# qiskit-community/aqc-research

Measured on AMD Instinct MI355X. Metric: objective+gradient evals/sec, higher is better.
Workload: dtype f64; 1 GPU; 16-qubit, 40-block cx spin ansatz, state-vector objective+gradient; n_qubits=16, num_thetas=208, gate_groups=56, batch_per_gpu=1024, columns=1, transport=none, records_gathered=1024, launcher=none

## Files before the change

### aqc_research_amd/csrc/aqc_kernels3.hip

```cpp
#include <hip/hip_runtime.h>

#include <cstring>

#include <type_traits>

#include "aqc_device.h"
#include "aqc_launch.h"
#include "aqc_math.h"

namespace aqc {

typedef double double4_t __attribute__((ext_vector_type(4)));

__host__ __device__ __forceinline__ unsigned swz3(unsigned l) { return l ^ ((l >> 4) & 15u) ^ ((l >> 8) & 15u); }

__device__ __forceinline__ double4_t mfma(double a, double b, double4_t c) {
    return __builtin_amdgcn_mfma_f64_16x16x4f64(a, b, c, 0, 0, 0);
}

struct Acc3 { double4_t k1, k2, k3; };
__device__ __forceinline__ void u_mfma(const cplx (&v)[4], const double (&u0)[4], const double (&u1)[4], const double (&u2)[4], Acc3& t) {
    t.k1 = double4_t{0.0, 0.0, 0.0, 0.0}; t.k2 = t.k1; t.k3 = t.k1;
#pragma unroll
    for (int s = 0; s < 4; ++s) {
        t.k1 = mfma(v[s].x + v[s].y, u0[s], t.k1);
        t.k2 = mfma(v[s].x, u1[s], t.k2);
        t.k3 = mfma(v[s].y, u2[s], t.k3);
    }
}
__device__ __forceinline__ void u_combine(const Acc3& t, cplx (&o)[4]) {
#pragma unroll
    for (int r = 0; r < 4; ++r) {
        o[r].x = t.k1[r] - t.k3[r];
        o[r].y = t.k1[r] + t.k2[r];
    }
}

#ifdef AQC_TUNING
#define AQC_STAMP(slot) do { if (a.stamps && threadIdx.x == 0 && (slot) < kStampSlots) \
    a.stamps[((size_t)blockIdx.y * gridDim.x + blockIdx.x) * kStampSlots + (slot)] = __builtin_amdgcn_s_memtime(); } while (0)
#ifdef AQC_TUNING_NODBG
#define AQC_DBG_AND(x)
#define AQC_DBG_TEST(x) false
#else
#define AQC_DBG_AND(x) && (x)
#define AQC_DBG_TEST(x) (x)
#endif
#else
#define AQC_STAMP(slot) do { } while (0)
#define AQC_DBG_AND(x)
#define AQC_DBG_TEST(x) false
#endif

__host__ __device__ constexpr bool sweep_scratch_double(int k) { return k >= 12 || k <= 9; }
#ifndef AQC_SWEEP_SPREAD
#define AQC_SWEEP_SPREAD 1
#endif
#ifndef AQC_APPLY_SPREAD
#define AQC_APPLY_SPREAD 1
#endif
#ifndef AQC_EXP_APPLY_SKIP
#define AQC_EXP_APPLY_SKIP 0
#endif
constexpr int kApplySkip = AQC_EXP_APPLY_SKIP;
#ifndef AQC_EXP_SWEEP_SKIP
#define AQC_EXP_SWEEP_SKIP 0
#endif
constexpr int kSweepSkip = AQC_EXP_SWEEP_SKIP;
#ifndef AQC_EXP_UBUILD_SKIP
#define AQC_EXP_UBUILD_SKIP 0
#endif
constexpr int kUbuildSkip = AQC_EXP_UBUILD_SKIP;

constexpr int kSweepSpread = AQC_SWEEP_SPREAD, kApplySpread = AQC_APPLY_SPREAD;
template <int K, bool SWEEP = false> struct TileShape {
    static constexpr int kSweepWaves12 = 4;
    static constexpr int kWaves = (SWEEP && K == 12) ? kSweepWaves12 : (K >= 10 ? 4 : (1 << (K - 8)));
    static constexpr int kGroups = 1 << (K - 8);
    static constexpr int kGpw = kGroups / kWaves;
    static constexpr int kLoads = (1 << (K - 6)) / kWaves;
};

struct SubRegs {
    double u0[4], u1[4], u2[4];
    unsigned lane12;
};

template <int GPW>
__device__ __forceinline__ void fetch_sub(SubRegs& x, const DevSub3* subs, const double* umat, int sub_index, int lane, int wave,
                                          int nwaves) {
    const DevSub3* sub = subs + sub_index;
    const double* up = umat + (size_t)sub_index * 12 * 64;
#pragma unroll
    for (int s = 0; s < 4; ++s) {
        x.u0[s] = up[(0 * 4 + s) * 64 + lane];
        x.u1[s] = up[(1 * 4 + s) * 64 + lane];
        x.u2[s] = up[(2 * 4 + s) * 64 + lane];
    }
    x.lane12 = sub->lane12[lane];
}

template <int GPW>
struct SubAddr {
    unsigned a1, a2;
    unsigned k1[GPW][4], k2[GPW][4];
};
typedef unsigned uint8v_t __attribute__((ext_vector_type(8)));
template <int GPW>
__device__ __forceinline__ void fetch_k(SubAddr<GPW>& x, const DevSub3* subs, int sub_index, int wave, int nwaves) {
#pragma unroll
    for (int j = 0; j < GPW; ++j) {
        const uint8v_t kv = *reinterpret_cast<const __attribute__((address_space(4))) uint8v_t*>(
            (const __attribute__((address_space(4))) void*)(const void*)&subs[sub_index].kk[wave + j * nwaves][0]);
#pragma unroll
        for (int s = 0; s < 4; ++s) { x.k1[j][s] = kv[s]; x.k2[j][s] = kv[4 + s]; }
    }
}
template <int GPW>
__device__ __forceinline__ void sub_addr(SubAddr<GPW>& x, const SubRegs& c, unsigned lds_base) {
    x.a1 = ((c.lane12 & 0xffffu) << 4) + lds_base;
    x.a2 = ((c.lane12 >> 16) << 4) + lds_base;
}
typedef double dbl2_t __attribute__((ext_vector_type(2)));
typedef __attribute__((address_space(3))) dbl2_t* lds_cplx_ptr;
__device__ __forceinline__ cplx lds_get(unsigned addr) {
    const dbl2_t v = *reinterpret_cast<lds_cplx_ptr>(addr);
    return make_double2(v.x, v.y);
}
__device__ __forceinline__ void lds_put(unsigned addr, cplx v) { *reinterpret_cast<lds_cplx_ptr>(addr) = dbl2_t{v.x, v.y}; }
__device__ __forceinline__ unsigned lds_address(const void* p) {
    return (unsigned)reinterpret_cast<size_t>((__attribute__((address_space(3))) const char*)p);
}

__device__ __forceinline__ const void* uniform_ptr(const void* p) {
    const unsigned long long v = (unsigned long long)p;
    const unsigned lo = __builtin_amdgcn_readfirstlane((unsigned)v), hi = __builtin_amdgcn_readfirstlane((unsigned)(v >> 32));
    return (const void*)(((unsigned long long)hi << 32) | lo);
}

template <int K, int NV>
__device__ __forceinline__ void load_tiles3(cplx* t0, cplx* t1, const cplx* s0, const cplx* s1, const DevStage& st, unsigned lo, int wave) {
    constexpr int NL = TileShape<K, NV == 2>::kLoads, NW = TileShape<K, NV == 2>::kWaves;
    cplx v0[NL], v1[NL];
#pragma unroll
    for (int i = 0; i < NL; ++i) {
        const unsigned off = lo + st.dhi[wave + i * NW];
        v0[i] = s0[off];
        if (NV == 2) v1[i] = s1[off];
    }
#pragma unroll
    for (int i = 0; i < NL; ++i) {
        const unsigned slot = swz3((unsigned)((wave + i * NW) << 6) | (threadIdx.x & 63u));
        t0[slot] = v0[i];
        if (NV == 2) t1[slot] = v1[i];
    }
}
template <int K, bool SWEEP>
__device__ __forceinline__ void store_tile3(const cplx* tile, cplx* dst, const DevStage& st, unsigned lo, int wave) {
    constexpr int NL = TileShape<K, SWEEP>::kLoads, NW = TileShape<K, SWEEP>::kWaves;
#pragma unroll
    for (int i = 0; i < NL; ++i) {
        const unsigned slot = swz3((unsigned)((wave + i * NW) << 6) | (threadIdx.x & 63u));
        dst[lo + st.dhi[wave + i * NW]] = tile[slot];
    }
}
__device__ __forceinline__ size_t tile_base3(const DevStage& st, unsigned tile) {
    size_t base = 0;
    for (int i0 = 0; i0 < st.nub; i0 += 4) {
        int ub[4];
#pragma unroll
        for (int u = 0; u < 4; ++u) ub[u] = st.ubits[i0 + u];
#pragma unroll
        for (int u = 0; u < 4; ++u)
            if (i0 + u < st.nub) base |= (size_t)((tile >> (i0 + u)) & 1u) << ub[u];
    }
    return base;
}

__device__ __forceinline__ int uniform_load(const int* p) { return __builtin_amdgcn_readfirstlane(*p); }
struct ItemAt { int bl, tile, slot; };
template <bool LIST>
__device__ __forceinline__ ItemAt item_at(const Stage3Args& a, int wi) {
    if (LIST) {
        const TileItem* it = a.items + wi;
        return ItemAt{uniform_load(&it->lane), uniform_load(&it->tile), uniform_load(&it->slot)};
    }
    const int bl = wi / a.ntiles;
    return ItemAt{bl, wi - bl * a.ntiles, 0};
}
template <int K, bool LIST, bool PAIR = false>
__device__ __forceinline__ void apply_mfma_body(const Stage3Args& a0, const Stage3Args& b0, const int wg, const int nwg) {
    using TS = TileShape<K>;
    static_assert(!PAIR || (LIST && K >= 12), "the pair form walks two lists with persistent workgroups");
    extern __shared__ __attribute__((aligned(16))) char smem[];
    const Stage3Args* ca = &a0;
#define a (*ca)
#define st (ca->stage)
    cplx* tw = reinterpret_cast<cplx*>(smem);
    const unsigned lds_base = lds_address(smem);
    if (lds_base & ((16u << K) - 1)) __builtin_trap();
    const int lane = threadIdx.x & 63;
    const int wave = __builtin_amdgcn_readfirstlane((int)(threadIdx.x >> 6));
    constexpr int NL = TS::kLoads, NW = TS::kWaves;
    constexpr bool kPersist = K >= 12;
    int nwork = LIST ? uniform_load(a.nitems) : a.ntiles * a.batch;
    bool second = false;
    if (PAIR && wg >= nwork) { ca = &b0; second = true; nwork = uniform_load(b0.nitems); }
    unsigned lo = st.dlo[lane];
    unsigned lo16 = lo << 4;
    (void)lo16;
    SubRegs cur, nxt;
    SubAddr<TS::kGpw> ad;
    dbl2_t pw[NL];
    int wi = wg + ((kPersist || LIST) ? 0 : (int)blockIdx.y * a.ntiles);
    if (LIST && wi >= nwork) return;
    ItemAt it = item_at<LIST>(a, wi);
    {
        const int bl = it.bl;
        if (st.nsubs > 0) {
            fetch_sub<TS::kGpw>(cur, a.subs, a.umat + (size_t)bl * a.nsubs_total * 12 * 64, st.sub_begin, lane, wave, NW);
            fetch_k<TS::kGpw>(ad, a.subs, st.sub_begin, wave, NW);
        }
        AQC_STAMP(0);
        if (!(kApplySkip & 64)) load_tiles3<K, 1>(tw, nullptr, a.in0 + (size_t)bl * a.lane_stride + tile_base3(st, it.tile), nullptr, st, lo, wave);
    }
    __builtin_amdgcn_s_waitcnt(0x0F70);
    AQC_STAMP(1);
    for (;;) {
    const int bl = it.bl;
    const size_t lane_off = (size_t)bl * a.lane_stride + tile_base3(st, it.tile);
    const double* umat = a.umat + (size_t)bl * a.nsubs_total * 12 * 64;
    int nwi = wi + nwg;
    bool more = kPersist && st.nsubs > 0 && nwi < nwork;
    const Stage3Args* na = ca;
    int nnwork = nwork;
    if (PAIR && !more && !second) {
        na = &b0; nwi = wg; nnwork = uniform_load(b0.nitems);
        more = nwi < nnwork;
    }
    const bool change = PAIR && na != ca;
    const ItemAt nit = more ? item_at<LIST>(*na, nwi) : ItemAt{0, 0, 0};
    const int nbl = nit.bl;
    const size_t next_off = more ? (size_t)nbl * na->lane_stride + tile_base3(na->stage, nit.tile) : 0;
    const unsigned nlo = change ? na->stage.dlo[lane] : lo;
    const unsigned nlo16 = nlo << 4;
    for (int si = 0; si < st.nsubs; ++si) {
        AQC_STAMP(4 + si);
        if (!(kApplySkip & 512)) __syncthreads();
        if (si + 1 < st.nsubs) fetch_sub<TS::kGpw>(nxt, a.subs, umat, st.sub_begin + si + 1, lane, wave, NW);
        else if (more) fetch_sub<TS::kGpw>(nxt, na->subs, na->umat + (size_t)nbl * na->nsubs_total * 12 * 64, na->stage.sub_begin, lane, wave, NW);
        if (kPersist && more && !(kApplySkip & 64)) {
#pragma unroll
            for (int c = 0; c < 4; ++c) {
                if (si == (c < st.nsubs ? c : st.nsubs - 1)) {
#pragma unroll
                    for (int i = c * (NL / 4); i < (c + 1) * (NL / 4); ++i) {
                        const size_t ub = next_off + na->stage.dhi[wave + i * NW];
                        asm volatile("s_nop 4\n\tglobal_load_dwordx4 %0, %1, %2" : "=a"(pw[i]) : "v"(nlo16), "s"(uniform_ptr(na->in0 + ub)) : "memory");
                    }
                }
            }
        }
        sub_addr(ad, cur, lds_base);
        cplx v[2][4];
        Acc3 acc;
#pragma unroll
        for (int s = 0; s < 4; ++s) v[0][s] = lds_get(ad.a1 ^ ad.k1[0][s]);
#pragma unroll
        for (int j = 0; j <= TS::kGpw; ++j) {
            if (j + 1 < TS::kGpw && !(kApplySkip & 2)) {
#pragma unroll
                for (int s = 0; s < 4; ++s) v[(j + 1) & 1][s] = lds_get((kApplySkip & 32) ? ad.a1 : (ad.a1 ^ ad.k1[j + 1][s]));
            }
            __builtin_amdgcn_sched_barrier(0);
            double sv[4];
            cplx o[4];
            if (j < TS::kGpw) {
#pragma unroll
                for (int s = 0; s < 4; ++s) sv[s] = (kApplySkip & (16 | 128)) ? v[j & 1][s].x : v[j & 1][s].x + v[j & 1][s].y;
            }
            if (j > 0) {
                if (kApplySkip & (16 | 256)) {
#pragma unroll
                    for (int r = 0; r < 4; ++r) o[r] = make_double2(acc.k1[r], acc.k2[r]);
                } else u_combine(acc, o);
            }
            unsigned wa[4];
            if (j < TS::kGpw) {
#pragma unroll
                for (int s = 0; s < 4; ++s) asm volatile("" : "+v"(sv[s]));
            }
            if (j > 0) {
#pragma unroll
                for (int r = 0; r < 4; ++r) { wa[r] = (kApplySkip & 32) ? ad.a2 : (ad.a2 ^ ad.k2[j - 1][r]); asm volatile("" : "+v"(wa[r])); }
            }
            __builtin_amdgcn_sched_barrier(0);
            if (j < TS::kGpw) {
                acc.k1 = double4_t{0.0, 0.0, 0.0, 0.0}; acc.k2 = acc.k1; acc.k3 = acc.k1;
#pragma unroll
                for (int s = 0; s < 4; ++s) {
                    if (kApplySkip & 8) continue;
                    acc.k1 = mfma(sv[s], cur.u0[s], acc.k1);
                    acc.k2 = mfma(v[j & 1][s].x, cur.u1[s], acc.k2);
                    acc.k3 = mfma(v[j & 1][s].y, cur.u2[s], acc.k3);
                }
            }
            if (j > 0 && !(kApplySkip & 1)) {
#pragma unroll
                for (int r = 0; r < 4; ++r) lds_put(wa[r], o[r]);
                if (j < TS::kGpw) {
#pragma unroll
                    for (int i = 0; i < 4; ++i) {
                        __builtin_amdgcn_sched_group_barrier(0x008, kApplySpread, 0);
                        __builtin_amdgcn_sched_group_barrier(0x200, 1, 0);
                    }
                }
            }
            __builtin_amdgcn_sched_barrier(0);
        }
        if (si + 1 < st.nsubs || more) {
            cur = nxt;
            if (si + 1 < st.nsubs) fetch_k<TS::kGpw>(ad, a.subs, st.sub_begin + si + 1, wave, NW);
            else fetch_k<TS::kGpw>(ad, na->subs, na->stage.sub_begin, wave, NW);
        }
    }
    AQC_STAMP(4 + st.nsubs);
    __syncthreads();
    AQC_STAMP(2);
    if (!(kApplySkip & 64)) store_tile3<K, false>(tw, a.out0 + lane_off, st, lo, wave);
    AQC_STAMP(3);
    if (!more) break;
    __syncthreads();
    __builtin_amdgcn_s_waitcnt(0x0F70);
#pragma unroll
    for (int i = 0; i < NL; ++i) {
        const unsigned slot = swz3((unsigned)((wave + i * NW) << 6) | (threadIdx.x & 63u));
        asm volatile("ds_write_b128 %0, %1" : : "v"(lds_base + (slot << 4)), "a"(pw[i]) : "memory");
    }
    __builtin_amdgcn_s_waitcnt(0xC07F);
    wi = nwi;
    it = nit;
    if (PAIR) { ca = na; second = second || change; nwork = nnwork; lo = nlo; lo16 = nlo16; }
    }
#undef a
#undef st
}
template <int K, bool LIST = false>
__global__ __launch_bounds__(TileShape<K>::kWaves * 64, 2) void apply_mfma_kernel(const Stage3Args a) {
    apply_mfma_body<K, LIST>(a, a, (int)blockIdx.x, (int)gridDim.x);
}
#ifndef AQC_PAIR_PLAIN_BOUNDARY
#define AQC_PAIR_PLAIN_BOUNDARY 0
#endif
template <int K>
__global__ __launch_bounds__(TileShape<K>::kWaves * 64, 2) void apply_pair_kernel(const Stage3Args a, const Stage3Args b, const int grid_a) {
    if constexpr (K >= 12 && !AQC_PAIR_PLAIN_BOUNDARY) {
        static_assert(sizeof(Stage3Args) % 8 == 0 && alignof(Stage3Args) == 8, "b follows a in the kernel-argument segment without padding");
        const __attribute__((address_space(4))) char* kp = (const __attribute__((address_space(4))) char*)__builtin_amdgcn_kernarg_segment_ptr();
        const Stage3Args* pa = (const Stage3Args*)(const void*)kp;
        const Stage3Args* pb = (const Stage3Args*)(const void*)(kp + sizeof(Stage3Args));
        apply_mfma_body<K, true, true>(*pa, *pb, (int)blockIdx.x, (int)gridDim.x);
    } else if (K >= 12) {
        apply_mfma_body<K, true>(a, a, (int)blockIdx.x, (int)gridDim.x);
        __syncthreads();
        apply_mfma_body<K, true>(b, b, (int)blockIdx.x, (int)gridDim.x);
    } else if ((int)blockIdx.x < grid_a) {
        apply_mfma_body<K, true>(a, a, (int)blockIdx.x, grid_a);
    } else {
        apply_mfma_body<K, true>(b, b, (int)blockIdx.x - grid_a, (int)gridDim.x - grid_a);
    }
}

template <int N>
__device__ __forceinline__ void wait_prefetched(dbl2_t (&pw)[N], dbl2_t (&pz)[N]) {
    asm volatile("s_waitcnt vmcnt(0)" : : : "memory");
#pragma unroll
    for (int i = 0; i < N; ++i) asm volatile("" : "+a"(pw[i]), "+a"(pz[i]));
}
__device__ __forceinline__ unsigned tile_offset3(const DevStage& st, unsigned local) { return st.dlo[local & 63u] | st.dhi[local >> 6]; }
template <int K> struct SweepShape : TileShape<K, true> {};
__device__ __forceinline__ unsigned elem_bit(const DevStage& st, long long e, unsigned local_pos) {
    const unsigned m = local_pos < 6 ? st.dlo[1u << local_pos] : st.dhi[1u << (local_pos - 6)];
    return ((unsigned long long)e & m) ? 1u : 0u;
}
template <int GPW, int NW>
__device__ __forceinline__ void skip_masks(const DevStage& st, unsigned info, long long e0, long long e1, int wave, unsigned& nzmask, unsigned& kneed) {
    nzmask = 0; kneed = 0;
    const unsigned gfresh = info & 15u, kfresh = (info >> 6) & 3u;
#pragma unroll
    for (int k = 0; k < 2; ++k) {
        const long long e = k ? e1 : e0;
        if (e < 0) continue;
        unsigned gb = 0;
#pragma unroll
        for (int i = 0; i < 4; ++i)
            if (gfresh >> i & 1) gb |= elem_bit(st, e, (info >> (8 + 4 * i)) & 15u) << i;
        unsigned kb = 0;
        if (kfresh & 1) kb |= elem_bit(st, e, (info >> 24) & 15u);
        if (kfresh & 2) kb |= elem_bit(st, e, (info >> 28) & 15u) << 1;
#pragma unroll
        for (int j = 0; j < GPW; ++j)
            if ((((unsigned)(wave + j * NW) ^ gb) & gfresh) == 0) nzmask |= 1u << j;
#pragma unroll
        for (unsigned s2 = 0; s2 < 4; ++s2)
            if (((s2 ^ kb) & kfresh) == 0) kneed |= 1u << s2;
    }
}
template <int K, bool LIST, bool SKIPW, bool RLAST>
__device__ __forceinline__ void sweep_mfma_body(const Stage3Args& a, const int wg, const int nwg) {
    using TS = TileShape<K, true>;
    constexpr int kSlots = TS::kWaves > 4 ? 4 : TS::kWaves;
    constexpr unsigned tsize = 1u << K;
    extern __shared__ __attribute__((aligned(16))) char smem[];
    const DevStage& st = a.stage;
    cplx* tw = reinterpret_cast<cplx*>(smem);
    cplx* tz = tw + tsize;
    cplx* scratch = tz + tsize;
    constexpr bool kDouble = sweep_scratch_double(K);
    const unsigned lds_base = lds_address(smem);
    if (lds_base & ((32u << K) - 1)) __builtin_trap();
    const int lane = threadIdx.x & 63;
    const int wave = __builtin_amdgcn_readfirstlane((int)(threadIdx.x >> 6));
    constexpr bool kPersist = K >= 12;
    constexpr int NL = TS::kLoads, NW = TS::kWaves;
    const int nwork = LIST ? uniform_load(a.nitems) : a.ntiles * a.batch;
    const unsigned lo = st.dlo[lane];
    SubRegs cur, nxt;
    SubAddr<TS::kGpw> ad;
    dbl2_t pw[NL], pz[NL];
    unsigned parity = 0;
    AQC_STAMP(0);
    const int chunk = kPersist ? (LIST ? (nwork + nwg - 1) / nwg : a.chunk) : 0;
    const int wi_first = kPersist ? wg * chunk : wg;
    const int wi_end = kPersist ? (wi_first + chunk < nwork ? wi_first + chunk : nwork) : wi_first + 1;
    int wi = wi_first;
    if (wi >= nwork) return;
    const unsigned e16 = threadIdx.x << 4;
    dbl2_t racc;
    static_assert(!kPersist || NL == 4 * TS::kGpw, "the prefetch registers are the first sub-stage's operands");
    const bool reg_first = kPersist && st.nsubs > 0;
    unsigned flo16 = 0;
    ItemAt it = item_at<LIST>(a, wi);
    size_t item_off = (size_t)it.bl * a.lane_stride + tile_base3(st, it.tile);
    {
        const size_t off0 = item_off;
        if (st.nsubs > 0) {
            fetch_sub<TS::kGpw>(cur, a.subs, a.umat + (size_t)it.bl * a.nsubs_total * 12 * 64, st.sub_begin, lane, wave, NW);
            fetch_k<TS::kGpw>(ad, a.subs, st.sub_begin, wave, NW);
        }
        if (reg_first) {
            flo16 = tile_offset3(st, swz3(cur.lane12 & 0xffffu)) << 4;
#pragma unroll
            for (int i = 0; i < ((kSweepSkip & 64) ? 0 : NL); ++i) {
                const size_t ub = off0 + a.first_hi[wave + (i / 4) * NW][i % 4];
                asm volatile("s_nop 4\n\tglobal_load_dwordx4 %0, %1, %2" : "=a"(pw[i]) : "v"(flo16), "s"(uniform_ptr(a.in0 + ub)) : "memory");
                asm volatile("s_nop 4\n\tglobal_load_dwordx4 %0, %1, %2" : "=a"(pz[i]) : "v"(flo16), "s"(uniform_ptr(a.in1 + ub)) : "memory");
            }
        } else {
            load_tiles3<K, 2>(tw, tz, a.in0 + off0, a.in1 + off0, st, lo, wave);
        }
    }
    __builtin_amdgcn_s_waitcnt(0x0F70);
    if (reg_first) wait_prefetched<NL>(pw, pz);
    __syncthreads();
    AQC_STAMP(1);
    for (;;) {
    const int bl = it.bl, tile = it.tile;
    const size_t lane_off = item_off;
    long long se0 = -1, se1 = -1;
    if (SKIPW) {
        const unsigned long long toff = (unsigned long long)tile_base3(st, tile);
        const long long c0 = a.supp[2 * (size_t)bl], c1 = a.supp[2 * (size_t)bl + 1];
        const unsigned lo0 = __builtin_amdgcn_readfirstlane((unsigned)c0), hi0 = __builtin_amdgcn_readfirstlane((unsigned)(c0 >> 32));
        const unsigned lo1 = __builtin_amdgcn_readfirstlane((unsigned)c1), hi1 = __builtin_amdgcn_readfirstlane((unsigned)(c1 >> 32));
        const long long u0 = (long long)(((unsigned long long)hi0 << 32) | lo0), u1 = (long long)(((unsigned long long)hi1 << 32) | lo1);
        if (u0 >= 0 && (((unsigned long long)u0 ^ toff) & st.fresh_nonlocal) == 0) se0 = u0;
        if (u1 >= 0 && (((unsigned long long)u1 ^ toff) & st.fresh_nonlocal) == 0) se1 = u1;
    }
    const double* umat = a.umat + (size_t)bl * a.nsubs_total * 12 * 64;
    const int part = LIST ? it.slot : (kPersist ? wg - (bl * a.ntiles) / chunk : tile);
    const bool seg_first = LIST || !kPersist || wi == wi_first || tile == 0;
    cplx* rpart = a.rpart + (((size_t)bl * a.nsubs_total + st.sub_begin) * a.nparts + part) * 256;
    const int nwi = wi + 1;
    const bool more = reg_first && nwi < wi_end;
    const ItemAt nit = more ? item_at<LIST>(a, nwi) : ItemAt{0, 0, 0};
    const int nbl = nit.bl;
    const size_t next_off = more ? (size_t)nbl * a.lane_stride + tile_base3(st, nit.tile) : 0;
    constexpr unsigned ZOFF = tsize * 16;
    cplx vw[2][4], vz[2][4];
    constexpr bool kEarly = K >= 11;
    if (reg_first) {
        sub_addr(ad, cur, lds_base);
#pragma unroll
        for (int s = 0; s < 4; ++s) { vw[0][s] = make_double2(pw[s].x, pw[s].y); vz[0][s] = make_double2(pz[s].x, pz[s].y); }
    } else if (kEarly && st.nsubs > 0) {
        sub_addr(ad, cur, lds_base);
#pragma unroll
        for (int s = 0; s < 4; ++s) { vw[0][s] = lds_get(ad.a1 ^ ad.k1[0][s]); vz[0][s] = lds_get((ad.a1 | ZOFF) ^ ad.k1[0][s]); }
    }
    auto prefetch = [&](int c) __attribute__((always_inline)) {
#pragma unroll
        for (int i = 0; i < ((kSweepSkip & 64) ? 0 : NL); ++i)
            if (i / (NL / 4) == c) {
                const size_t ub = next_off + a.first_hi[wave + (i / 4) * NW][i % 4];
                asm volatile("s_nop 4\n\tglobal_load_dwordx4 %0, %1, %2" : "=a"(pw[i]) : "v"(flo16), "s"(uniform_ptr(a.in0 + ub)) : "memory");
                asm volatile("s_nop 4\n\tglobal_load_dwordx4 %0, %1, %2" : "=a"(pz[i]) : "v"(flo16), "s"(uniform_ptr(a.in1 + ub)) : "memory");
            }
    };
    const int nmain = RLAST && a.r_only_last && st.nsubs >= 1 && !(kPersist && st.nsubs == 1) ? st.nsubs - 1 : st.nsubs;
    if (!RLAST) {
        for (int si = 0; si < st.nsubs; ++si) {
#define AQC_SS_FROM_REGS (reg_first && si == 0)
#define AQC_SS_RONLY false
#include "aqc_sweep_substage.inc"
#undef AQC_SS_FROM_REGS
#undef AQC_SS_RONLY
        }
    } else {
        if (nmain > 0) {
            const int si = 0;
#define AQC_SS_FROM_REGS reg_first
#define AQC_SS_RONLY false
#include "aqc_sweep_substage.inc"
#undef AQC_SS_FROM_REGS
#undef AQC_SS_RONLY
        }
        for (int si = 1; si < nmain; ++si) {
#define AQC_SS_FROM_REGS false
#define AQC_SS_RONLY false
#include "aqc_sweep_substage.inc"
#undef AQC_SS_FROM_REGS
#undef AQC_SS_RONLY
        }
        if (nmain < st.nsubs) {
            const int si = nmain;
#define AQC_SS_FROM_REGS false
#define AQC_SS_RONLY true
#include "aqc_sweep_substage.inc"
#undef AQC_SS_FROM_REGS
#undef AQC_SS_RONLY
        }
    }
    AQC_STAMP(kStampSlots - 2);
    if (more) wait_prefetched<NL>(pw, pz);
    if (!(kSweepSkip & 64)) {
        if (a.store_out & 1) store_tile3<K, true>(tw, a.out0 + lane_off, st, lo, wave);
        if (a.store_out & 2) store_tile3<K, true>(tz, a.out1 + lane_off, st, lo, wave);
    }
    AQC_STAMP(kStampSlots - 1);
    if (!more) break;
    AQC_STAMP(kStampSlots - 6);
    __syncthreads();
    AQC_STAMP(kStampSlots - 5);
    wi = nwi;
    it = nit;
    item_off = next_off;
    }
    AQC_STAMP(kStampSlots - 4);
}
template <int K, bool LIST = false, bool SKIPW = false, bool RLAST = false>
__global__ __launch_bounds__(SweepShape<K>::kWaves * 64, K >= 12 ? 1 : 2) void sweep_mfma_kernel(const Stage3Args a) {
    sweep_mfma_body<K, LIST, SKIPW, RLAST>(a, (int)blockIdx.x, (int)gridDim.x);
}
template <int K, bool RLAST_A, bool RLAST_B>
__global__ __launch_bounds__(SweepShape<K>::kWaves * 64, K >= 12 ? 1 : 2) void sweep_pair_kernel(const Stage3Args a, const Stage3Args b, const int grid_a) {
    if (K >= 12) {
        sweep_mfma_body<K, true, false, RLAST_A>(a, (int)blockIdx.x, (int)gridDim.x);
        __syncthreads();
        sweep_mfma_body<K, true, false, RLAST_B>(b, (int)blockIdx.x, (int)gridDim.x);
    } else if ((int)blockIdx.x < grid_a) {
        sweep_mfma_body<K, true, false, RLAST_A>(a, (int)blockIdx.x, grid_a);
    } else {
        sweep_mfma_body<K, true, false, RLAST_B>(b, (int)blockIdx.x - grid_a, (int)gridDim.x - grid_a);
    }
}

constexpr int kGrpChunk = 16;
struct Gm {
    cplx c[4], t[4];
    double ec, es;
    double rc[4], rs[4];
    int type, pc, pt, flags, slot0, jblock, o0, o1;
};
__device__ __forceinline__ void m2_mul(const cplx (&a)[4], const cplx (&b)[4], cplx (&o)[4]) {
#pragma unroll
    for (int i = 0; i < 2; ++i)
#pragma unroll
        for (int j = 0; j < 2; ++j) {
            const cplx x = a[2 * i], y = b[j], u = a[2 * i + 1], v = b[2 + j];
            o[2 * i + j] = make_double2(x.x * y.x - x.y * y.y + u.x * v.x - u.y * v.y, x.x * y.y + x.y * y.x + u.x * v.y + u.y * v.x);
        }
}
__device__ __forceinline__ void m2_ry(double c, double s, cplx (&o)[4]) {
    o[0] = make_double2(c, 0.0); o[1] = make_double2(-s, 0.0); o[2] = make_double2(s, 0.0); o[3] = make_double2(c, 0.0);
}
__device__ __forceinline__ void m2_rz(double c, double s, cplx (&o)[4]) {
    o[0] = make_double2(c, -s); o[1] = make_double2(0.0, 0.0); o[2] = make_double2(0.0, 0.0); o[3] = make_double2(c, s);
}
__device__ __forceinline__ void m2_rx(double c, double s, cplx (&o)[4]) {
    o[0] = make_double2(c, 0.0); o[1] = make_double2(0.0, -s); o[2] = make_double2(0.0, -s); o[3] = make_double2(c, 0.0);
}
template <bool DAG, bool TR>
__device__ __forceinline__ void m2_apply(const cplx (&m)[4], cplx& a0, cplx& a1) {
    const cplx m00 = m[0], m01 = (DAG || TR) ? m[2] : m[1], m10 = (DAG || TR) ? m[1] : m[2], m11 = m[3];
    const double sg = DAG ? -1.0 : 1.0;
    const cplx x = a0, y = a1;
    a0 = make_double2(m00.x * x.x - sg * m00.y * x.y + m01.x * y.x - sg * m01.y * y.y, m00.x * x.y + sg * m00.y * x.x + m01.x * y.y + sg * m01.y * y.x);
    a1 = make_double2(m10.x * x.x - sg * m10.y * x.y + m11.x * y.x - sg * m11.y * y.y, m10.x * x.y + sg * m10.y * x.x + m11.x * y.y + sg * m11.y * y.x);
}
__device__ __forceinline__ void stage_groups(Gm* gm, const DevGrp* grps, int begin, int count, const double* th, int ent, int lane) {
    {
        const int gi = lane >> 2, k = lane & 3;
        if (gi < count) {
            const DevGrp d = grps[begin + gi];
            double c = 1.0, s = 0.0;
            if (k < (d.type == 0 ? 3 : 4)) sincos(0.5 * th[d.theta0 + k], &s, &c);
            gm[gi].rc[k] = c; gm[gi].rs[k] = s;
            if (k == 0) {
                double ec = 1.0, es = 0.0;
                if (ent == 2 && d.type != 0) sincos(th[d.theta0 + 4], &es, &ec);
                gm[gi].ec = ec; gm[gi].es = es;
            }
        }
    }
    __builtin_amdgcn_fence(__ATOMIC_SEQ_CST, "wavefront");
    __builtin_amdgcn_wave_barrier();
    if (lane >= count) return;
    const DevGrp d = grps[begin + lane];
    Gm g;
    g.type = d.type; g.pc = d.pc; g.pt = d.pt; g.flags = d.flags; g.slot0 = d.slot0; g.jblock = d.jblock;
    const int mask = 0xF & ~(1 << d.pc) & ~(1 << d.pt);
    g.o0 = __ffs(mask) - 1; g.o1 = __ffs(mask & (mask - 1)) - 1;
    g.ec = gm[lane].ec; g.es = gm[lane].es;
#pragma unroll
    for (int k = 0; k < 4; ++k) { g.rc[k] = gm[lane].rc[k]; g.rs[k] = gm[lane].rs[k]; }
    cplx a[4], b[4], m[4];
    if (d.type == 0) {
        m2_rz(g.rc[0], g.rs[0], a); m2_ry(g.rc[1], g.rs[1], b); m2_mul(a, b, m);
        m2_rz(g.rc[2], g.rs[2], b); m2_mul(m, b, g.c);
        g.t[0] = make_double2(1.0, 0.0); g.t[1] = make_double2(0.0, 0.0); g.t[2] = g.t[1]; g.t[3] = g.t[0];
    } else {
        m2_rz(g.rc[1], g.rs[1], a); m2_ry(g.rc[0], g.rs[0], b); m2_mul(a, b, g.c);
        if (d.flags & 1) { m2_rz(kR, -kR, b); m2_mul(g.c, b, m); g.c[0] = m[0]; g.c[1] = m[1]; g.c[2] = m[2]; g.c[3] = m[3]; }
        if (ent == 0) m2_rx(g.rc[3], g.rs[3], a); else m2_rz(g.rc[3], g.rs[3], a);
        m2_ry(g.rc[2], g.rs[2], b); m2_mul(a, b, g.t);
        if (d.flags & 2) { m2_rz(kR, kR, a); m2_mul(a, g.t, m); g.t[0] = m[0]; g.t[1] = m[1]; g.t[2] = m[2]; g.t[3] = m[3]; }
    }
    gm[lane] = g;
}
__device__ __forceinline__ int grp_index(const Gm& g, int l, int rest) {
    return ((l >> 1) << g.pc) | ((l & 1) << g.pt) | ((rest & 1) << g.o0) | ((rest >> 1) << g.o1);
}
template <int MODE>
__device__ __forceinline__ void grp_apply(const Gm& g, int ent, cplx (&x)[4]) {
    auto entangle = [&](double es) {
        if (g.type == 0) return;
        if (ent == 0) { const cplx t = x[2]; x[2] = x[3]; x[3] = t; }
        else if (ent == 1) x[3] = make_double2(-x[3].x, -x[3].y);
        else x[3] = cmul(x[3], g.ec, es);
    };
    if (MODE == 0) {
        entangle(g.es);
        m2_apply<false, false>(g.t, x[0], x[1]); m2_apply<false, false>(g.t, x[2], x[3]);
        m2_apply<false, false>(g.c, x[0], x[2]); m2_apply<false, false>(g.c, x[1], x[3]);
    } else {
        m2_apply<MODE == 1, MODE == 2>(g.c, x[0], x[2]); m2_apply<MODE == 1, MODE == 2>(g.c, x[1], x[3]);
        m2_apply<MODE == 1, MODE == 2>(g.t, x[0], x[1]); m2_apply<MODE == 1, MODE == 2>(g.t, x[2], x[3]);
        entangle(MODE == 1 ? -g.es : g.es);
    }
}

__global__ __launch_bounds__(64) void ubuild_kernel(const UJob* jobs, const double* thetas, int T, double* thetas_copy) {
    __shared__ cplx u[256];
    __shared__ Gm gm[kGrpChunk];
    const int lane = threadIdx.x, b = blockIdx.y;
    const UJob job = jobs[blockIdx.x];
    const DevSub3 sub = *job.sub;
    const double* th = thetas + (size_t)b * T;
    if (thetas_copy && blockIdx.x == 0)
        for (int i = lane; i < T; i += 64) thetas_copy[(size_t)b * T + i] = th[i];
#pragma unroll
    for (int m = 0; m < 4; ++m) {
        const int e = lane + 64 * m;
        u[e] = make_double2((e >> 4) == (e & 15) ? 1.0 : 0.0, 0.0);
    }
    const int col = lane & 15, rest = lane >> 4;
    for (int base = 0; base < sub.ngrp; base += kGrpChunk) {
        const int count = min(kGrpChunk, sub.ngrp - base);
        __syncthreads();
        stage_groups(gm, job.grps, sub.grp_begin + base, count, th, job.entangler, lane);
        __syncthreads();
        for (int i = 0; i < count; ++i) {
            const Gm& g = gm[i];
            cplx x[4];
            int idx[4];
#pragma unroll
            for (int l = 0; l < 4; ++l) { idx[l] = grp_index(g, l, rest) * 16 + col; x[l] = u[idx[l]]; }
            if (job.inverse) grp_apply<1>(g, job.entangler, x); else grp_apply<0>(g, job.entangler, x);
#pragma unroll
            for (int l = 0; l < 4; ++l) u[idx[l]] = x[l];
            __syncthreads();
        }
    }
    __syncthreads();
    double* out = job.umat + ((size_t)b * job.nsubs + job.index) * 12 * 64;
    if (kUbuildSkip) {
        double acc = 0.0;
        for (int m = 0; m < 4; ++m) acc += u[lane + 64 * m].x * u[lane + 64 * m].y;
        if (acc == 1.0e300) out[lane] = acc;
    }
    if (kUbuildSkip & 1) return;
#pragma unroll
    for (int s = 0; s < 4; ++s) {
        const cplx v = u[(lane & 15) * 16 + 4 * s + (lane >> 4)];
        out[(0 * 4 + s) * 64 + lane] = v.x;
        out[(1 * 4 + s) * 64 + lane] = v.y - v.x;
        out[(2 * 4 + s) * 64 + lane] = v.x + v.y;
    }
    if (job.umat_mirror && !(kUbuildSkip & 2)) {
        double* om = job.umat_mirror + ((size_t)b * job.mirror_nsubs + job.mirror_index) * 12 * 64;
#pragma unroll
        for (int s = 0; s < 4; ++s) {
            const cplx t = u[(4 * s + (lane >> 4)) * 16 + (lane & 15)];
            const double re = t.x, im = -t.y;
            om[(0 * 4 + s) * 64 + lane] = re;
            om[(1 * 4 + s) * 64 + lane] = im - re;
            om[(2 * 4 + s) * 64 + lane] = re + im;
        }
    }
}

template <int LB>
__device__ __forceinline__ void rho_unapply(cplx (&rho)[16], int kind, double c, double s) {
    constexpr int st = LB == 0 ? 1 : 2, other = LB == 0 ? 2 : 1;
#pragma unroll
    for (int q = 0; q < 2; ++q)
#pragma unroll
        for (int b = 0; b < 4; ++b) {
            const int a0 = q * other;
            if (kind == MOP_RY) ry2(rho[a0 * 4 + b], rho[(a0 + st) * 4 + b], c, -s);
            else if (kind == MOP_RZ) rz2(rho[a0 * 4 + b], rho[(a0 + st) * 4 + b], c, -s);
            else rx2(rho[a0 * 4 + b], rho[(a0 + st) * 4 + b], c, -s);
        }
#pragma unroll
    for (int q = 0; q < 2; ++q)
#pragma unroll
        for (int a = 0; a < 4; ++a) {
            const int b0 = q * other;
            if (kind == MOP_RY) ry2(rho[a * 4 + b0], rho[a * 4 + b0 + st], c, -s);
            else if (kind == MOP_RZ) rz2(rho[a * 4 + b0], rho[a * 4 + b0 + st], c, s);
            else rx2(rho[a * 4 + b0], rho[a * 4 + b0 + st], c, s);
        }
}
template <int LB>
__device__ __forceinline__ cplx rho_dot(const cplx (&rho)[16], int kind) {
    constexpr int st = LB == 0 ? 1 : 2, other = LB == 0 ? 2 : 1;
    double re = 0.0, im = 0.0;
#pragma unroll
    for (int q = 0; q < 2; ++q) {
        const int i0 = q * other, i1 = i0 + st;
        if (kind == MOP_RY) { re += rho[i1 * 4 + i0].x - rho[i0 * 4 + i1].x; im += rho[i1 * 4 + i0].y - rho[i0 * 4 + i1].y; }
        else if (kind == MOP_RZ) { re += rho[i0 * 4 + i0].x - rho[i1 * 4 + i1].x; im += rho[i0 * 4 + i0].y - rho[i1 * 4 + i1].y; }
        else { re += rho[i0 * 4 + i1].x + rho[i1 * 4 + i0].x; im += rho[i0 * 4 + i1].y + rho[i1 * 4 + i0].y; }
    }
    return kind == MOP_RY ? make_double2(0.5 * re, 0.5 * im) : make_double2(-0.5 * im, 0.5 * re);
}

#ifdef AQC_TUNING
__device__ unsigned long long g_rgrad_stamps[32 * 8];
#define RG_STAMP(slot) do { if (blockIdx.y == 0 && blockIdx.x < 32 && threadIdx.x == 0) g_rgrad_stamps[blockIdx.x * 8 + (slot)] = __builtin_amdgcn_s_memtime(); } while (0)
#else
#define RG_STAMP(slot) do { } while (0)
#endif
template <int WAVES>
__global__ __launch_bounds__(64 * WAVES) void rgrad_kernel(const DevSub3* subs, const DevGrp* grps, int ent, const double* thetas, int T,
                                                           const cplx* rpart, int ntiles, int nsubs_total, cplx* partial, int nslots,
                                                           int from, int to, int front, const int* slot_theta, cplx* grads, cplx* mirror,
                                                           const GatherJob gj, int tiles_per_lane, int chunk, int sparse_subs,
                                                           const int* lane_parts, int conj_sub, const double* umat, int nsubs_run,
                                                           const RgradSecond second) {
    if ((int)blockIdx.x == nsubs_run + second.count) {
        const cplx* src = static_cast<const cplx*>(gj.buf) + (size_t)blockIdx.y * gj.lane_stride;
        for (int i = threadIdx.x; i < gj.count; i += 64 * WAVES) {
            const cplx v = src[(size_t)gj.elem[i]];
            static_cast<cplx*>(gj.out)[(size_t)blockIdx.y * gj.count + i] = v;
            if (gj.mirror) static_cast<cplx*>(gj.mirror)[(size_t)blockIdx.y * gj.count + i] = v;
        }
        return;
    }
    __shared__ cplx R[16 * 17];
    __shared__ Gm gm[kGrpChunk];
    __shared__ cplx rho_s[kGrpChunk][16];
    __shared__ cplx psum[WAVES > 1 ? WAVES - 1 : 1][WAVES > 1 ? 256 : 1];
    const int lane = threadIdx.x & 63, wave = threadIdx.x >> 6, b = blockIdx.y;
    int si = blockIdx.x;
    if (si >= nsubs_run) {
        si -= nsubs_run;
        subs = second.subs; grps = second.grps; rpart = second.rpart; ntiles = second.nparts; nsubs_total = second.nsubs_total;
        tiles_per_lane = second.nparts; chunk = 0; sparse_subs = second.nsubs_total; lane_parts = second.lane_parts; conj_sub = -1; umat = second.umat;
    }
    RG_STAMP(0);
    const DevSub3 sub = subs[si];
    const double* th = thetas + (size_t)b * T;
    const int nparts_stride = ntiles;
    if (chunk > 0) ntiles = ((b + 1) * tiles_per_lane - 1) / chunk - (b * tiles_per_lane) / chunk + 1;
    if (si < sparse_subs) ntiles = lane_parts[b];
    const cplx* rp = rpart + ((size_t)b * nsubs_total + si) * nparts_stride * 256;
    {
        cplx acc[4] = {make_double2(0.0, 0.0), make_double2(0.0, 0.0), make_double2(0.0, 0.0), make_double2(0.0, 0.0)};
        constexpr int TB = 8;
        for (int t0 = wave; t0 < ntiles; t0 += TB * WAVES) {
            cplx v[TB][4];
#pragma unroll
            for (int u = 0; u < TB; ++u)
#pragma unroll
                for (int r = 0; r < 4; ++r)
                    v[u][r] = t0 + u * WAVES < ntiles ? rp[(size_t)(t0 + u * WAVES) * 256 + 64 * r + lane] : make_double2(0.0, 0.0);
            if (WAVES > 1 && t0 == wave && wave == 0 && sub.ngrp > 0)
                stage_groups(gm, grps, sub.grp_begin + max(0, sub.ngrp - kGrpChunk), min(sub.ngrp, kGrpChunk), th, ent, lane);
#pragma unroll
            for (int u = 0; u < TB; ++u)
#pragma unroll
                for (int r = 0; r < 4; ++r) { acc[r].x += v[u][r].x; acc[r].y += v[u][r].y; }
        }
        if (WAVES > 1) {
            if (wave > 0) {
#pragma unroll
                for (int r = 0; r < 4; ++r) psum[wave - 1][64 * r + lane] = acc[r];
            }
            __syncthreads();
            if (wave > 0) return;
#pragma unroll
            for (int w = 0; w < WAVES - 1; ++w)
#pragma unroll
                for (int r = 0; r < 4; ++r) { const cplx p = psum[w][64 * r + lane]; acc[r].x += p.x; acc[r].y += p.y; }
        }
#pragma unroll
        for (int r = 0; r < 4; ++r)
            R[(4 * r + (lane >> 4)) * 17 + (lane & 15)] = acc[r];
    }
    if (si == conj_sub) {
        cplx* const Us = &rho_s[0][0];
        const double* up = umat + ((size_t)b * nsubs_total + si) * 12 * 64;
        __syncthreads();
#pragma unroll
        for (int s2 = 0; s2 < 4; ++s2) {
            const double re = up[(0 * 4 + s2) * 64 + lane], im = up[(1 * 4 + s2) * 64 + lane] + re;
            Us[(lane & 15) * 16 + 4 * s2 + (lane >> 4)] = make_double2(re, im);
        }
        __syncthreads();
        const int i0 = lane & 15, j0 = lane >> 4;
        cplx acc[4];
#pragma unroll
        for (int m = 0; m < 4; ++m) {
            const int j = j0 + 4 * m;
            double re = 0.0, im = 0.0;
            for (int k = 0; k < 16; ++k) {
                const cplx u = Us[j * 16 + k], r = R[k * 17 + i0];
                re += u.x * r.x - u.y * r.y; im += u.x * r.y + u.y * r.x;
            }
            acc[m] = make_double2(re, im);
        }
        __syncthreads();
#pragma unroll
        for (int m = 0; m < 4; ++m) R[(j0 + 4 * m) * 17 + i0] = acc[m];
        __syncthreads();
#pragma unroll
        for (int m = 0; m < 4; ++m) {
            const int j = j0 + 4 * m;
            double re = 0.0, im = 0.0;
            for (int k = 0; k < 16; ++k) {
                const cplx t = R[j * 17 + k], u = Us[i0 * 16 + k];
                re += t.x * u.x + t.y * u.y; im += t.y * u.x - t.x * u.y;
            }
            acc[m] = make_double2(re, im);
        }
        __syncthreads();
#pragma unroll
        for (int m = 0; m < 4; ++m) R[(j0 + 4 * m) * 17 + i0] = acc[m];
        __syncthreads();
    }
    RG_STAMP(1);
    cplx* out = partial + (size_t)b * nslots;
    auto put = [&](int slot, cplx v) {
        out[slot] = v;
        if (slot_theta) {
            const int t = slot_theta[slot];
            if (t >= 0) {
                grads[(size_t)b * T + t] = v;
                if (mirror) mirror[(size_t)b * T + t] = v;
            }
        }
    };
    const int lo = lane & 15, hi = lane >> 4;
    for (int top = sub.ngrp; top > 0; top -= kGrpChunk) {
        const int base = max(0, top - kGrpChunk), count = top - base;
        __syncthreads();
        if (WAVES == 1 || top != sub.ngrp) stage_groups(gm, grps, sub.grp_begin + base, count, th, ent, lane);
        __syncthreads();
        RG_STAMP(2);
        for (int i = count - 1; i >= 0; --i) {
            const Gm& g = gm[i];
            {
                const int a = lane >> 4, bb = (lane >> 2) & 3, o = lane & 3;
                cplx v = R[grp_index(g, a, o) * 17 + grp_index(g, bb, o)];
                v.x += dpp_mov<0xB1, 0xf>(v.x); v.y += dpp_mov<0xB1, 0xf>(v.y);
                v.x += dpp_mov<0x4E, 0xf>(v.x); v.y += dpp_mov<0x4E, 0xf>(v.y);
                if (o == 0) rho_s[i][a * 4 + bb] = v;
            }
            cplx x[4];
            int idx[4];
#pragma unroll
            for (int l = 0; l < 4; ++l) { idx[l] = grp_index(g, l, hi) * 17 + lo; x[l] = R[idx[l]]; }
            grp_apply<1>(g, ent, x);
#pragma unroll
            for (int l = 0; l < 4; ++l) R[idx[l]] = x[l];
            __syncthreads();
#pragma unroll
            for (int l = 0; l < 4; ++l) { idx[l] = lo * 17 + grp_index(g, l, hi); x[l] = R[idx[l]]; }
            grp_apply<2>(g, ent, x);
#pragma unroll
            for (int l = 0; l < 4; ++l) R[idx[l]] = x[l];
            __syncthreads();
        }
        RG_STAMP(3);
        if (lane < count) {
            const Gm& g = gm[lane];
            const bool on = g.jblock < 0 ? (front != 0) : (g.jblock >= from && g.jblock < to);
            if (on && g.slot0 >= 0) {
                cplx rho[16];
#pragma unroll
                for (int e = 0; e < 16; ++e) rho[e] = rho_s[lane][e];
                if (g.type == 0) {
                    put(g.slot0 + 2, rho_dot<1>(rho, MOP_RZ));
                    rho_unapply<1>(rho, MOP_RZ, g.rc[0], g.rs[0]);
                    put(g.slot0 + 1, rho_dot<1>(rho, MOP_RY));
                    rho_unapply<1>(rho, MOP_RY, g.rc[1], g.rs[1]);
                    put(g.slot0 + 0, rho_dot<1>(rho, MOP_RZ));
                } else {
                    const int ks = ent == 0 ? MOP_RX : MOP_RZ;
                    if (g.flags & 2) rho_unapply<0>(rho, MOP_RZ, kR, kR);
                    put(g.slot0 + 3, rho_dot<0>(rho, ks));
                    rho_unapply<0>(rho, ks, g.rc[3], g.rs[3]);
                    put(g.slot0 + 2, rho_dot<0>(rho, MOP_RY));
                    put(g.slot0 + 1, rho_dot<1>(rho, MOP_RZ));
                    rho_unapply<1>(rho, MOP_RZ, g.rc[1], g.rs[1]);
                    put(g.slot0 + 0, rho_dot<1>(rho, MOP_RY));
                    if (ent == 2) {
                        rho_unapply<0>(rho, MOP_RY, g.rc[2], g.rs[2]);
                        rho_unapply<1>(rho, MOP_RY, g.rc[0], g.rs[0]);
                        put(g.slot0 + 4, make_double2(rho[15].y, -rho[15].x));
                    }
                }
            } else if (slot_theta && g.slot0 >= 0) {
                for (int k = 0; k < 5; ++k) put(g.slot0 + k, make_double2(0.0, 0.0));
            }
        }
        RG_STAMP(4);
    }
}
#ifdef AQC_TUNING
void rgrad_print_stamps(int nsubs) {
    unsigned long long h[32 * 8];
    if (hipMemcpyFromSymbol(h, HIP_SYMBOL(g_rgrad_stamps), sizeof h) != hipSuccess) return;
    double a = 0, b = 0, c = 0, d = 0;
    const int n = nsubs < 32 ? nsubs : 32;
    for (int i = 0; i < n; ++i) { a += h[i * 8 + 1] - h[i * 8]; b += h[i * 8 + 2] - h[i * 8 + 1]; c += h[i * 8 + 3] - h[i * 8 + 2]; d += h[i * 8 + 4] - h[i * 8 + 3]; }
    fprintf(stderr, "aqc_hip stamps: gradient walk (lane 0, %d sub-stages): tile sum %.0f + group decode %.0f + R walk %.0f + rho walk %.0f cycles\n", n, a / n, b / n, c / n, d / n);
}
#endif

void stage3_first_offsets(Stage3Args& a, const DevSub3& first_sub) {
    for (int g = 0; g < 16; ++g)
        for (int s = 0; s < 4; ++s) {
            const unsigned local = swz3(first_sub.kk[g][s] >> 4);
            a.first_hi[g][s] = a.stage.dlo[local & 63u] | a.stage.dhi[local >> 6];
        }
}

int mfma_threads(int k, bool sweep) { return (sweep && k == 12) ? 64 * SweepShape<12>::kWaves : 64 * std::min(4, 1 << std::max(0, k - 8)); }
size_t apply3_lds_bytes(int k) { return (size_t)16 << k; }
size_t sweep3_lds_bytes(int k) {
    return ((size_t)32 << k) + (size_t)(sweep_scratch_double(k) ? 2 : 1) * std::min(4, mfma_threads(k, true) / 64) * 256 * sizeof(cplx);
}

template <typename F>
static hipError_t with_tile_size(int k, F&& f) {
    switch (k) {
        case 8: return f(std::integral_constant<int, 8>{});
        case 9: return f(std::integral_constant<int, 9>{});
        case 10: return f(std::integral_constant<int, 10>{});
        case 11: return f(std::integral_constant<int, 11>{});
        case 12: return f(std::integral_constant<int, 12>{});
        default: return hipErrorInvalidValue;
    }
}
using Stage3Kernel = void (*)(Stage3Args);
using Pair3Kernel = void (*)(Stage3Args, Stage3Args, int);
template <int K> static Stage3Kernel apply_variant(bool list) { return list ? apply_mfma_kernel<K, true> : apply_mfma_kernel<K, false>; }
template <int K> static Stage3Kernel sweep_variant(bool list, bool skipw, bool rlast) {
    if (list) return rlast ? sweep_mfma_kernel<K, true, false, true> : sweep_mfma_kernel<K, true, false, false>;
    if (skipw) return sweep_mfma_kernel<K, false, true, false>;
    return rlast ? sweep_mfma_kernel<K, false, false, true> : sweep_mfma_kernel<K, false, false, false>;
}
template <int K> static Pair3Kernel apply_pair_variant() { return apply_pair_kernel<K>; }
template <int K> static Pair3Kernel sweep_pair_variant(bool rlast_a) { return rlast_a ? sweep_pair_kernel<K, true, false> : sweep_pair_kernel<K, false, false>; }

template <typename F>
static hipError_t big_lds(F kernel) {
    return hipFuncSetAttribute(reinterpret_cast<const void*>(kernel), hipFuncAttributeMaxDynamicSharedMemorySize, 160 * 1024);
}
hipError_t init_kernels3() {
    hipError_t e = hipSuccess;
    for (int k = 8; k <= 12 && e == hipSuccess; ++k)
        e = with_tile_size(k, [](auto kk) {
            constexpr int K = decltype(kk)::value;
            hipError_t e = big_lds(apply_pair_variant<K>());
            for (int f = 0; f < 2 && e == hipSuccess; ++f) e = big_lds(apply_variant<K>(f));
            for (int f = 0; f < 2 && e == hipSuccess; ++f) e = big_lds(sweep_pair_variant<K>(f));
            for (int f = 0; f < 8 && e == hipSuccess; ++f) e = big_lds(sweep_variant<K>(f & 1, f & 2, f & 4));
            return e;
        });
    return e;
}
template <typename... Args>
static hipError_t launch3(void (*kernel)(Args...), dim3 grid, int k, bool sweep, hipStream_t s, const Args&... args) {
    kernel<<<grid, mfma_threads(k, sweep), sweep ? sweep3_lds_bytes(k) : apply3_lds_bytes(k), s>>>(args...);
    return hipGetLastError();
}
int mfma_occupancy(int k, bool sweep) {
    int n = 0;
    const hipError_t e = with_tile_size(k, [&](auto kk) {
        constexpr int K = decltype(kk)::value;
        return sweep ? hipOccupancyMaxActiveBlocksPerMultiprocessor(&n, sweep_variant<K>(false, false, false), mfma_threads(k, true), sweep3_lds_bytes(k))
                     : hipOccupancyMaxActiveBlocksPerMultiprocessor(&n, apply_variant<K>(false), mfma_threads(k, false), apply3_lds_bytes(k));
    });
    return e == hipSuccess ? n : -1;
}
static long persistent_sweep_grid(long sweep_grid) {
    if (sweep_grid > 0) return sweep_grid;
    static int cus[64] = {0};
    int dev = 0;
    if (hipGetDevice(&dev) != hipSuccess || dev < 0 || dev >= 64) return 256;
    if (cus[dev] == 0) {
        int n = 0;
        cus[dev] = (hipDeviceGetAttribute(&n, hipDeviceAttributeMultiprocessorCount, dev) == hipSuccess && n > 0) ? n : 256;
    }
    return cus[dev];
}
static bool stage3_launchable(int k, const Stage3Args& a, bool need_list, bool need_subs) {
    if (a.items ? (!a.nitems || a.max_items < 1) : need_list) return false;
    if (k < 12) return true;
    if (need_subs && a.stage.nsubs <= 0) return false;
    for (int l = 0; l < 64; ++l)
        if (a.stage.dlo[l] >= (1u << 28)) return false;
    return true;
}
hipError_t launch_apply3(int k, hipStream_t s, const Stage3Args& a, const Switches& sw) {
    const bool list = a.items != nullptr;
    const long persist = sw.apply_persist;
    if (!stage3_launchable(k, a, false, list) || (list && k >= 12 && persist <= 0)) return hipErrorInvalidValue;
    const long nwork = list ? (long)a.max_items : (long)a.ntiles * a.batch;
    const dim3 grid = (k >= 12 && persist > 0 && a.stage.nsubs > 0) ? dim3((unsigned)std::min<long>(nwork, persist * persistent_sweep_grid(sw.sweep_grid)))
                                                                     : ((k >= 12 || list) ? dim3((unsigned)nwork) : dim3(a.ntiles, a.batch));
    return with_tile_size(k, [&](auto kk) { return launch3(apply_variant<decltype(kk)::value>(list), grid, k, false, s, a); });
}
static_assert(2 * sizeof(Stage3Args) + 16 <= 3840, "two argument blocks must fit the kernel-argument segment");
hipError_t launch_apply3_pair(int k, hipStream_t s, const Stage3Args& a, const Stage3Args& b, const Switches& sw) {
    const long persist = sw.apply_persist;
    if (!stage3_launchable(k, a, true, true) || !stage3_launchable(k, b, true, true) || (k >= 12 && persist <= 0)) return hipErrorInvalidValue;
    const long longer = std::max(a.max_items, b.max_items);
    const dim3 grid((unsigned)(k >= 12 ? std::min<long>(longer, persist * persistent_sweep_grid(sw.sweep_grid)) : (long)a.max_items + b.max_items));
    return with_tile_size(k, [&](auto kk) { return launch3(apply_pair_variant<decltype(kk)::value>(), grid, k, false, s, a, b, a.max_items); });
}
int sweep3_chunk(int ntiles, int batch, int k, long sweep_grid) {
    if (k < 12) return 0;
    const long nwork = (long)ntiles * batch, g = std::min<long>(nwork, persistent_sweep_grid(sweep_grid));
    return (int)((nwork + g - 1) / g);
}
int sweep3_nparts(int ntiles, int batch, int k, long sweep_grid) {
    const int chunk = sweep3_chunk(ntiles, batch, k, sweep_grid);
    return chunk > 0 ? std::min(ntiles, (ntiles + chunk - 1) / chunk + 1) : ntiles;
}
hipError_t launch_sweep3(int k, hipStream_t s, const Stage3Args& a, const Switches& sw) {
    const bool list = a.items != nullptr;
    if (!stage3_launchable(k, a, false, true)) return hipErrorInvalidValue;
    if (a.nparts < 1 || (!list && (a.nparts != sweep3_nparts(a.ntiles, a.batch, k, sw.sweep_grid) || a.chunk != sweep3_chunk(a.ntiles, a.batch, k, sw.sweep_grid)))) return hipErrorInvalidValue;
    const long nwork = list ? (long)a.max_items : (long)a.ntiles * a.batch;
    const dim3 grid((unsigned)(k >= 12 ? (list ? std::min<long>(nwork, persistent_sweep_grid(sw.sweep_grid)) : (nwork + a.chunk - 1) / a.chunk) : nwork));
    const bool skipw = !list && a.supp != nullptr;
    const bool rlast = !skipw && a.r_only_last != 0;
    return with_tile_size(k, [&](auto kk) { return launch3(sweep_variant<decltype(kk)::value>(list, skipw, rlast), grid, k, true, s, a); });
}

hipError_t launch_sweep3_pair(int k, hipStream_t s, const Stage3Args& a, const Stage3Args& b, const Switches& sw) {
    if (!stage3_launchable(k, a, true, true) || !stage3_launchable(k, b, true, true)) return hipErrorInvalidValue;
    if (a.nparts < 1 || b.nparts < 1 || a.supp || b.supp || b.r_only_last) return hipErrorInvalidValue;
    const long longer = std::max(a.max_items, b.max_items);
    const dim3 grid((unsigned)(k >= 12 ? std::min<long>(longer, persistent_sweep_grid(sw.sweep_grid)) : (long)a.max_items + b.max_items));
    return with_tile_size(k, [&](auto kk) { return launch3(sweep_pair_variant<decltype(kk)::value>(a.r_only_last != 0), grid, k, true, s, a, b, a.max_items); });
}

__device__ __forceinline__ int tile_of_elem(const DevStage& st, long long e) {
    int t = 0;
    for (int i = 0; i < st.nub; ++i) t |= (int)((e >> st.ubits[i]) & 1) << i;
    return t;
}
__device__ __forceinline__ int lane_tiles(const DevStage& st, const long long* supp, int per_lane, const long long* extra, int nextra, int b,
                                          int (&tiles)[kMaxTileCands]) {
    int n = 0;
    auto add = [&](long long e) {
        if (e < 0) return;
        const int t = tile_of_elem(st, e);
        for (int i = 0; i < n; ++i)
            if (tiles[i] == t) return;
        tiles[n++] = t;
    };
    for (int k = 0; supp && k < per_lane; ++k) add(supp[(size_t)b * per_lane + k]);
    for (int k = 0; extra && k < nextra; ++k) add(extra[k]);
    return n;
}
__global__ __launch_bounds__(1024) void tile_items_kernel(const DevStage st, const long long* supp, int per_lane, const long long* extra, int nextra,
                                                          int batch, TileItem* items, int* nitems, int* lane_parts, int* prev_tiles,
                                                          TileItem* clear_items, int* nclear) {
    __shared__ int scan_a[1024], scan_b[1024];
    const int tid = threadIdx.x, per = (batch + 1023) / 1024;
    const int b0 = tid * per, b1 = min(batch, b0 + per);
    int tiles[kMaxTileCands];
    int mine = 0, mine_clear = 0;
    for (int b = b0; b < b1; ++b) {
        const int n = lane_tiles(st, supp, per_lane, extra, nextra, b, tiles);
        mine += n;
        if (prev_tiles)
            for (int k = 0; k < 2; ++k) {
                const int pt = prev_tiles[2 * b + k];
                bool stale = pt >= 0;
                for (int i = 0; i < n; ++i) stale = stale && tiles[i] != pt;
                mine_clear += stale ? 1 : 0;
            }
    }
    scan_a[tid] = mine; scan_b[tid] = mine_clear;
    __syncthreads();
    for (int d = 1; d < 1024; d <<= 1) {
        const int va = tid >= d ? scan_a[tid - d] : 0, vb = tid >= d ? scan_b[tid - d] : 0;
        __syncthreads();
        scan_a[tid] += va; scan_b[tid] += vb;
        __syncthreads();
    }
    int at = scan_a[tid] - mine, at_clear = scan_b[tid] - mine_clear;
    if (tid == 1023) { *nitems = scan_a[tid]; if (nclear) *nclear = scan_b[tid]; }
    for (int b = b0; b < b1; ++b) {
        const int n = lane_tiles(st, supp, per_lane, extra, nextra, b, tiles);
        if (lane_parts) lane_parts[b] = n;
        if (prev_tiles) {
            for (int k = 0; k < 2; ++k) {
                const int pt = prev_tiles[2 * b + k];
                bool stale = pt >= 0;
                for (int i = 0; i < n; ++i) stale = stale && tiles[i] != pt;
                if (stale) clear_items[at_clear++] = TileItem{b, pt, 0, 0};
            }
            prev_tiles[2 * b] = n > 0 ? tiles[0] : -1;
            prev_tiles[2 * b + 1] = n > 1 ? tiles[1] : -1;
        }
        for (int i = 0; i < n; ++i) items[at++] = TileItem{b, tiles[i], i, 0};
    }
}
hipError_t launch_tile_items(const DevStage& stage, const long long* supp, int per_lane, const long long* extra, int nextra, int batch,
                             TileItem* items, int* nitems, int* lane_parts, int* prev_tiles, TileItem* clear_items, int* nclear, hipStream_t s) {
    if ((supp ? per_lane : 0) + (extra ? nextra : 0) > kMaxTileCands || batch < 1) return hipErrorInvalidValue;
    if (prev_tiles && ((supp ? per_lane : 0) > 2 || (extra && nextra > 0) || !clear_items || !nclear)) return hipErrorInvalidValue;
    tile_items_kernel<<<1, 1024, 0, s>>>(stage, supp, per_lane, extra, nextra, batch, items, nitems, lane_parts, prev_tiles, clear_items, nclear);
    return hipGetLastError();
}
__global__ __launch_bounds__(256) void clear_tiles_kernel(const DevStage st, cplx* buf, size_t lane_stride, const TileItem* clear_items, const int* nclear) {
    if ((int)blockIdx.x >= *nclear) return;
    const TileItem it = clear_items[blockIdx.x];
    cplx* dst = buf + (size_t)it.lane * lane_stride + tile_base3(st, (unsigned)it.tile);
    for (unsigned l = threadIdx.x; l < (1u << st.k); l += 256) dst[tile_offset3(st, l)] = make_double2(0.0, 0.0);
}
hipError_t launch_clear_tiles(const DevStage& stage, void* buf, size_t lane_stride, const TileItem* clear_items, const int* nclear, int max_items,
                              hipStream_t s) {
    if (max_items < 1) return hipSuccess;
    clear_tiles_kernel<<<max_items, 256, 0, s>>>(stage, static_cast<cplx*>(buf), lane_stride, clear_items, nclear);
    return hipGetLastError();
}
hipError_t launch_ubuild(const UJob* jobs, int njobs, const double* thetas, int T, int batch, hipStream_t s, double* thetas_copy) {
    if (njobs < 1) return hipSuccess;
    ubuild_kernel<<<dim3(njobs, batch), 64, 0, s>>>(jobs, thetas, T, thetas_copy);
    return hipGetLastError();
}
hipError_t launch_rgrad(const DevSub3* subs, const DevGrp* grps, int entangler, const double* thetas, int T, const void* rpart,
                        int ntiles, int nsubs_total, void* partial, int nslots, int from, int to, int front, int batch, hipStream_t s,
                        const int* slot_theta, void* grads, void* mirror, GatherJob gather, int nparts, int chunk, int sparse_subs,
                        const int* lane_parts, int conj_sub, const double* umat, int nsubs_run, const RgradSecond* second_plan) {
    if (nsubs_total < 1) return hipSuccess;
    if (nsubs_run < 0 || nsubs_run > nsubs_total) nsubs_run = nsubs_total;
    RgradSecond second;
    memset(&second, 0, sizeof second);
    if (second_plan) second = *second_plan;
    const int extra = (gather.count > 0 && gather.buf ? 1 : 0) + second.count;
    if (nsubs_run + extra < 1) return hipSuccess;
    const int tiles_per_lane = ntiles;
    if (nparts <= 0) nparts = ntiles;
    ntiles = nparts;
    if (nparts >= 32 && second.count == 0)
        rgrad_kernel<4><<<dim3(nsubs_run + extra, batch), 256, 0, s>>>(subs, grps, entangler, thetas, T, static_cast<const cplx*>(rpart), ntiles,
                                                                  nsubs_total, static_cast<cplx*>(partial), nslots, from, to, front, slot_theta,
                                                                  static_cast<cplx*>(grads), static_cast<cplx*>(mirror), gather, tiles_per_lane, chunk, sparse_subs, lane_parts, conj_sub, umat, nsubs_run, second);
    else
        rgrad_kernel<1><<<dim3(nsubs_run + extra, batch), 64, 0, s>>>(subs, grps, entangler, thetas, T, static_cast<const cplx*>(rpart), ntiles,
                                                                 nsubs_total, static_cast<cplx*>(partial), nslots, from, to, front, slot_theta,
                                                                 static_cast<cplx*>(grads), static_cast<cplx*>(mirror), gather, tiles_per_lane, chunk, sparse_subs, lane_parts, conj_sub, umat, nsubs_run, second);
    return hipGetLastError();
}

}
```

### aqc_research_amd/csrc/aqc_launch.h

```cpp
#pragma once
#include <string>
#include <hip/hip_runtime.h>

#include <algorithm>
#include <cstddef>

#include "aqc_device.h"
#include "aqc_mps_walk.h"
#include "aqc_switches.h"

namespace aqc {

struct StageArgs {
    const DevStage* stage;
    const DevOp* ops;
    const DevSub* subs;
    const DevMop* mops;
    const double* coef;
    int ncoef;
    const double2* in0;
    const double2* in1;
    double2* out0;
    double2* out1;
    size_t lane_stride;
    double2* partial;
    int nslots, ntiles_max;
    int from, to, front;
    int final_stage;
    int debug;
};

size_t apply_lds_bytes(int k);
size_t sweep_lds_bytes(int k, int threads);
hipError_t init_kernels();
hipError_t launch_apply(int ent, bool inverse, int ntiles, int batch, int threads, int k, hipStream_t s, const StageArgs& a);
hipError_t launch_sweep(int ent, int ntiles, int batch, int threads, int k, hipStream_t s, const StageArgs& a);
hipError_t launch_coef(const double* thetas, double* coef, int n, int nblocks, int tpb, int tail, int batch, hipStream_t s);
hipError_t launch_finalize(const void* partial, const int* theta_slots, const int* slot_ntiles, void* grads, int T,
                           int nslots, int ntiles_max, int n, int tpb, int from, int to, int front, int batch,
                           hipStream_t s, void* mirror = nullptr);
hipError_t launch_scatter_one(void* buf, size_t lane_stride, int batch, const long long* elem, hipStream_t s);
hipError_t launch_scatter_two(void* buf, size_t lane_stride, int batch, const long long* elem, const void* coef, long long* prev, hipStream_t s);
hipError_t launch_set_identity(void* buf, size_t lane_stride, int dim, int pitch, int batch, hipStream_t s);
hipError_t launch_gather(const void* buf, size_t lane_stride, const long long* elem, int count, int batch, void* out,
                         hipStream_t s, void* mirror = nullptr);
hipError_t launch_vdot(const void* a, const void* b, size_t lane_stride, size_t count, int batch, void* part, int nparts,
                       void* out, hipStream_t s);

hipError_t init_kernels2();
hipError_t launch_apply2(int ent, int ntiles, int batch, int k, hipStream_t s, const StageArgs& a);
hipError_t launch_sweep2(int ent, int ntiles, int batch, int k, int reg_bits, hipStream_t s, const StageArgs& a);

struct TileItem { int lane, tile, slot, pad; };
struct Stage3Args {
    DevStage stage;
    const DevSub3* subs;
    const double* umat;
    int nsubs_total;
    const double2* in0;
    const double2* in1;
    double2* out0;
    double2* out1;
    size_t lane_stride;
    double2* rpart;
    int ntiles;
    int batch;
    int chunk, nparts;
    int store_out;
    int r_only_last;
    const long long* supp;
    const TileItem* items;
    const int* nitems;
    int max_items;
    unsigned first_hi[16][4];
    int debug;
    unsigned long long* stamps;
};
constexpr int kStampSlots = 40;
void stage3_first_offsets(Stage3Args& a, const DevSub3& first_sub);
hipError_t init_kernels3();
int mfma_threads(int k, bool sweep);
int mfma_occupancy(int k, bool sweep);
hipError_t launch_apply3(int k, hipStream_t s, const Stage3Args& a, const Switches& sw);
hipError_t launch_sweep3(int k, hipStream_t s, const Stage3Args& a, const Switches& sw);
hipError_t launch_apply3_pair(int k, hipStream_t s, const Stage3Args& a, const Stage3Args& b, const Switches& sw);
hipError_t launch_sweep3_pair(int k, hipStream_t s, const Stage3Args& a, const Stage3Args& b, const Switches& sw);
void rgrad_print_stamps(int nsubs);
int sweep3_chunk(int ntiles, int batch, int k, long sweep_grid);
int sweep3_nparts(int ntiles, int batch, int k, long sweep_grid);
struct ProjMap { const unsigned* tab; int shift; };
struct ProjArgs {
    const double2* y;
    const double2* s;
    double2* out;
    int s_virtual, out_virtual;
    int staged;
    int keep_bits, k_bits, cb;
    ProjMap y_keep, y_k, s_k, s_c, o_keep, o_c;
    size_t lane_stride;
    const TileItem* items;
    const int* nitems;
    const int* lane_parts;
    int nub0, ubits0[32];
    unsigned ff_mask, cb_mask, tf_mask;
    int nvp;
    const unsigned* off_t;
    const unsigned* off_cb;
    const unsigned* it_of_c;
    const unsigned* off_us;
    int us_bits;
    size_t part_stride;
    double2* cpart;
    int cpart_shares;
    int t, ntiles_v;
    double2* vm;
    TileItem* vitems;
    int* vcount;
    int* vlane_parts;
    int batch;
};
hipError_t launch_project_init(const ProjArgs& a, hipStream_t s);
hipError_t launch_project_fused(const ProjArgs& a, const void* mend, void* ctile, void* yout, hipStream_t s, int qb);
hipError_t launch_project_amps(const ProjArgs& a, const long long* gather, int ngather, const long long* supp, void* small, const void* vy, const void* z,
                               hipStream_t s);
hipError_t launch_project(const ProjArgs& a, hipStream_t s);
struct UJob {
    const DevSub3* sub;
    const DevGrp* grps;
    double* umat;
    int index, nsubs;
    int inverse, entangler;
    double* umat_mirror;
    int mirror_index, mirror_nsubs;
};
hipError_t launch_ubuild(const UJob* jobs, int njobs, const double* thetas, int T, int batch, hipStream_t s, double* thetas_copy = nullptr);
struct GatherJob {
    const void* buf; size_t lane_stride; const long long* elem; int count; void* out; void* mirror;
};
struct RgradSecond {
    const DevSub3* subs;
    const DevGrp* grps;
    const double2* rpart;
    const int* lane_parts;
    const double* umat;
    int nparts, nsubs_total, count;
};
hipError_t launch_rgrad(const DevSub3* subs, const DevGrp* grps, int entangler, const double* thetas, int T, const void* rpart,
                        int ntiles, int nsubs_total, void* partial, int nslots, int from, int to, int front, int batch, hipStream_t s,
                        const int* slot_theta = nullptr, void* grads = nullptr, void* mirror = nullptr,
                        GatherJob gather = GatherJob{nullptr, 0, nullptr, 0, nullptr, nullptr},
                        int nparts = 0, int chunk = 0,
                        int sparse_subs = 0, const int* lane_parts = nullptr,
                        int conj_sub = -1, const double* umat = nullptr,
                        int nsubs_run = -1,
                        const RgradSecond* second_plan = nullptr);
constexpr int kMaxTileCands = 72;
hipError_t launch_tile_items(const DevStage& stage, const long long* supp, int per_lane, const long long* extra, int nextra, int batch,
                             TileItem* items, int* nitems, int* lane_parts, int* prev_tiles, TileItem* clear_items, int* nclear, hipStream_t s);
hipError_t launch_clear_tiles(const DevStage& stage, void* buf, size_t lane_stride, const TileItem* clear_items, const int* nclear, int max_items,
                              hipStream_t s);

struct LbState {
    int B, T, S, memory;
    double *x, *g, *f;
    double *d, *slope, *step;
    double *x_new;
    double *Smem, *Ymem, *rho;
    int *active, *done;
    long long* nit;
    double *weight, *fidelity;
    int* max_no;
    double2 *cur_hs, *cur_g0;
    double2 *acc_hs, *acc_g0;
};
hipError_t lb_prepare(const LbState& st, const void* hs, int update, double* f_out, void* raw_hs, void* x2, size_t lane_stride,
                      const long long* index, long long* prev, hipStream_t s);
hipError_t lb_take(const LbState& st, const void* grads, double* g_out, void* raw_g, hipStream_t s);
hipError_t lb_probe(const LbState& st, const void* hs, int* flags, hipStream_t s);
hipError_t lb_commit0(const LbState& st, const void* hs, const void* raw_g, double* f_out, double* g_out, hipStream_t s);
hipError_t lb_active(const LbState& st, double gtol, double fid_thr, int* flags, hipStream_t s);
hipError_t lb_direction(const LbState& st, int count, hipStream_t s);
hipError_t lb_trial(const LbState& st, double* thetas, hipStream_t s);
hipError_t lb_armijo(const LbState& st, double c1, const double* thetas, const double* ft, const void* raw_hs_t, const void* raw_g0_t,
                     int* flags, hipStream_t s);
hipError_t lb_copy_raw(const LbState& st, hipStream_t s);
hipError_t lb_history(const LbState& st, int count, double ftol, const double* f_acc, const double* g_acc, hipStream_t s);
struct LbMat {
    int k;
    double gtol, fobj_thr, fid_thr;
    double *gmax;
    double *ft, *gt, *gmax_t, *fid_t;
    double *f_acc, *g_acc, *gmax_acc, *fid_acc;
    int* status;
    int* flags;
};
enum { kLbNotDone = 1, kLbAnyActive = 2 };
enum { kLbNonFinite = 1 };
hipError_t lb_mat_value(const LbState& st, const LbMat& m, const void* trace, const void* grads, int init, hipStream_t s);
hipError_t lb_mat_direction(const LbState& st, const LbMat& m, int count, hipStream_t s);
hipError_t lb_mat_armijo(const LbState& st, const LbMat& m, double c1, const double* thetas, hipStream_t s);
hipError_t lb_mat_history(const LbState& st, const LbMat& m, int count, double ftol, int last, hipStream_t s);

hipError_t launch_mps_scale(void* g, const double* lam, int rows, int cols, hipStream_t s);
hipError_t launch_zgemm(bool conj_t, bool accum, int M, int N, int K, const void* A, int lda, const void* B, int ldb,
                        void* C, int ldc, hipStream_t s);
hipError_t launch_zgemm_bh(bool conj_t, bool accum, int M, int N, int K, const void* A, int lda, const void* B, int ldb,
                           void* C, int ldc, hipStream_t s);
hipError_t launch_mps_env_dot(const void* e, const void* rc, size_t count, void* out, hipStream_t s);
hipError_t launch_zgemm_batched(bool conj_t, bool accum, int M, int N, int K, const void* A, int lda, const void* B, int ldb,
                                void* C, int ldc, size_t stride_a, size_t stride_b, size_t stride_c, int nbatch, hipStream_t s);
hipError_t launch_zgemm_tables(int M, int N, int K, const void* const* a_tab, int lda, const void* const* b_tab, int ldb, void* const* c_tab, int ldc,
                               size_t stride_a, size_t stride_b, size_t stride_c, int outer, int inner, hipStream_t s, int b_transposed = 0);
hipError_t launch_zgemm_tables_op(bool conj_t, bool accum, int M, int N, int K, const void* const* a_tab, int lda, const void* const* b_tab, int ldb,
                                  void* const* c_tab, int ldc, size_t stride_a, size_t stride_b, size_t stride_c, int outer, int inner, hipStream_t s);
hipError_t launch_mps_product(const void* const* t_tab, void* const* out_tab, int n, int count, hipStream_t s);
struct MpsSites {
    int n;
    size_t total;
    size_t offset[65];
    int lam_offset[64];
    int cols[64];
};
hipError_t launch_mps_scale_all(void* t, const double* lam, const MpsSites& sites, hipStream_t s);

struct CdSegHost { int32_t ha, hb, ent, nrot, kind[4], on_b[4], tindex[4]; };
size_t cd_persistent_lds_bytes(int nbits, int T);
struct CdRule {
    int* status;
    int* nit;
    double* best_f;
    double* best_thetas;
    double* profile;
    double fobj_thr, dtheta_thr;
    int maxiter;
};
hipError_t launch_cd_persistent(const void* prog, int nsegs, int nbits, int col_bits, const void* target, size_t lane_stride, double* thetas,
                                int T, double* fobj, int nsweeps, int max_steps, int batch, hipStream_t s, const CdRule* rule = nullptr);
struct CdWide {
    void* w; void* z;
    size_t lane_stride;
    int ngroups, nparts;
    int ha, hb, ent;
    int kind, on_b, tindex;
    int next_kind, next_on_b;
    int T;
    const double* theta_in;
    double* theta_out;
    double* dmax;
    const int* status;
    const double* part_in;
    double* part_out;
    double inv_d2n;
};
int cd_wide_parts(size_t lane_elems);
hipError_t launch_cd_wide_open(const CdWide& a, int batch, hipStream_t s);
hipError_t launch_cd_wide_step(const CdWide& a, int batch, hipStream_t s);
struct CdClose {
    CdRule rule;
    const double2* trace;
    double* dmax;
    double* theta_own;
    const double* theta_cur;
    int T;
    double inv_d2n;
};
hipError_t launch_cd_close(const CdClose& a, int batch, hipStream_t s);
hipError_t launch_cd_count(int* status, int batch, int mark, int* running, hipStream_t s);


hipError_t launch_gate1q(const void* src, void* dst, int n, size_t ncols, int q, const double* g, hipStream_t s);
hipError_t launch_gate2q(const void* src, void* dst, int n, size_t ncols, int qc, int qt, const double* g, hipStream_t s);
int gate_dot_parts(int n, size_t ncols, int kind);
hipError_t launch_gate_dot(const void* w, const void* z, int n, size_t ncols, int kind, int q0, int q1, void* partial, void* out,
                           hipStream_t s);

constexpr int kXxzThreads = 256, kXxzTileBits = 11;
struct XxzArgs {
    int n, tile_bits, lanes;
    double delta;
    const double2* cur;
    size_t cur_stride;
    const double2* prev;
    size_t prev_stride;
    double2* next;
    double2* out;
    const double2* coef;
    const double2* coef0;
    double scale;
    int first;
    double* partial;
};
int xxz_tile_bits(int n);
hipError_t launch_xxz_mul(const XxzArgs& a, hipStream_t s);
hipError_t launch_xxz_step(const XxzArgs& a, hipStream_t s);
hipError_t launch_xxz_energy(const XxzArgs& a, double* energy , hipStream_t s);

constexpr int kObsThreads = 256, kObsSubsetCap = 16, kObsGridCap = 512;
struct ObsArgs {
    int n, tile_bits, lanes, nsub;
    int ksplit;
    uint32_t bits;
    uint16_t subsets[kObsSubsetCap];
    const double2* src;
    double* partial;
};
int obs_ksplit(int nsub);
unsigned obs_grid_x(int n, int tile_bits);
hipError_t launch_obs_pass(const ObsArgs& a, hipStream_t s);
hipError_t launch_obs_final(const double* partial, unsigned nblocks, int nsub, int lanes, double2* rho, size_t lane_stride, hipStream_t s);

struct MpsObsFusedArgs {
    int n;
    const double2* const* sites;
    const int* dims;
    const size_t* env_off;
    double2* env_l;
    double2* env_r;
    const int* chain_start;
    const int* chain_last;
    const int* emit_of;
    double2* sums;
};
hipError_t launch_mps_obs_env(const MpsObsFusedArgs& a, hipStream_t s);
hipError_t launch_mps_obs_fused(const MpsObsFusedArgs& a, int nchains, hipStream_t s);
hipError_t launch_mps_obs_sums(const void* e_base, const int* slots, const int* emits, int count, size_t slot_stride, const void* k_base, size_t k_stride,
                               int chi, void* sums, hipStream_t s);

int set_error(const std::string& msg);

hipError_t launch_svd_identity(void* V, int cols, hipStream_t s);
hipError_t launch_jacobi_round(void* W, int rows, void* V, int cols, const void* pairs, int npairs, double tol, const double* fro2, int* rotations,
                               hipStream_t s);
hipError_t launch_svd_fro2(const void* W, size_t n, double* out, hipStream_t s);
hipError_t launch_svd_load(const void* a, int m, int n, int mode, void* work, hipStream_t s);
hipError_t launch_svd_assemble(const void* W, const void* V, const int* ord, const double* sigma, int m, int n, int k, int mode, void* u, void* vh,
                               double* s_sorted, hipStream_t s);
bool svd_fits_small(int rows, int cols);
hipError_t launch_jacobi_small(void* W, int rows, void* V, int cols, double tol, int max_sweeps, int* sweeps_out, double* sigma_out,
                               hipStream_t s);
bool svd_fits_block(int rows, int cols);
int svd_block_size();
hipError_t launch_jacobi_block(void* W, int rows, void* V, int cols, const void* bpairs, int rounds, int per_round, double tol, int max_sweeps,
                               const double* fro2, int* rot, unsigned* bar, int* status, hipStream_t s, int debug = 0);
hipError_t launch_svd_norms(const void* W, int rows, int cols, double* sigma, hipStream_t s);
hipError_t launch_mps_theta(const void* theta0, const double* lam_left, int chil, int chir, const double* g16, int mode, void* work, hipStream_t s);
size_t svd_batch_work_elems(int count, int m, int n);
size_t svd_batch_v_elems(int count, int m, int n);
hipError_t launch_svd_batch(int count, int m, int n, const int* d_rows, const int* d_cols, const void* d_a, void* d_u, double* d_s, void* d_vh,
                            int* d_sweeps, int* d_status, void* work, void* vmat, hipStream_t s);
constexpr int kLaneCap = 32;
constexpr int kLaneSite = 2 * kLaneCap * kLaneCap;
constexpr int kLaneEnv = kLaneCap * kLaneCap;
constexpr int kLaneNoConv = 1, kLaneOverflow = 2, kLaneZero = 4, kLaneLdsShort = 8;
struct LaneMps { void* T; double* lam; int* dims; double* discarded; int n, pad; };
hipError_t launch_lanes_gate1(const LaneMps& a, const LaneMps* b, const LaneOp1* ops, int nops, const LaneOp1& one, const double* thetas, int T, int lanes,
                              int bond_hint, hipStream_t s);
hipError_t launch_lanes_gate2(const LaneMps& m, const LaneMps* m2, const LaneOp2* ops, int nops, const LaneOp2& one, const double* thetas, int T,
                              double trunc_thr, int max_bond, int* status, int* peak, int lanes, int bond_hint, hipStream_t s,
                              unsigned long long* jstats = nullptr);
hipError_t launch_lanes_env_left(const LaneMps& w, const LaneMps& z, int p, const void* in, size_t in_stride, void* out, size_t out_stride,
                                 const double* gh8, int lanes, hipStream_t s);
hipError_t launch_lanes_env_right(const LaneMps& w, const LaneMps& z, int p, const void* in, size_t in_stride, void* out, size_t out_stride, int lanes,
                                  hipStream_t s);
hipError_t launch_lanes_env_dot(const LaneMps& w, const LaneMps& z, int hi, const void* e, size_t e_stride, const void* rc, size_t rc_stride, void* vals,
                                int nvals, int slot, int lanes, hipStream_t s);
struct LaneSteps { LaneGate1 g[3]; double gh[3][8]; int count, pad; };
hipError_t launch_lanes_grad_step(const LaneMps& w, const LaneMps& z, int q, const LaneSteps& steps, const double* thetas, int T, const void* env_l,
                                  size_t l_stride, const void* env_r, size_t r_stride, void* scratch, void* vals, int nvals, int slot, int lanes, hipStream_t s);
hipError_t launch_lanes_basis(const LaneMps& m, const unsigned char* bits , int lanes, hipStream_t s);
hipError_t launch_lanes_bank_dot(const LaneMps& bank, int count, const LaneMps& vh, int lanes, void* vals, int nvals, int slot0, int* status,
                                 int bond_hint, hipStream_t s);
hipError_t launch_lanes_env_init(void* env_l, size_t l_stride, void* env_r_last, size_t r_stride, int lanes, hipStream_t s);
bool mps_env_fits_small(int xa, int ua, int yb, int vb);
hipError_t launch_mps_env_left(const void* in, const void* A, const void* B, int xa, int ua, int yb, int vb, const double* gh8, void* out, hipStream_t s);
hipError_t launch_mps_env_right(const void* rc, const void* A, const void* B, int xa, int ua, int yb, int vb, void* out, hipStream_t s);
hipError_t launch_mps_theta_fused(const void* tq, const void* tq1, const double* lam_left, int chil, int chim, int chir, const double* g16, int mode,
                                  void* work, hipStream_t s);
hipError_t launch_mps_split(const void* W, const void* V, const int* ord, const double* sigma, const double* lam_left, int chil, int chir,
                            int k, int mode, double rescale, void* tq, void* tq1, const double* lam_new, double* lam_dst, hipStream_t s);
hipError_t launch_mps_colscale(void* t, const double* lam, size_t rows, int cols, int mul, hipStream_t s);

int sk_qr_slabs(int d);
hipError_t launch_sk_qr(void* a, void* scratch, size_t lane_stride, int lda, int d, int k, int batch, double abs_floor, void* partial, void* rinv, int* status,
                        hipStream_t s);
hipError_t launch_sk_alt(void* x, void* y, size_t lane_stride, int pitch, int d, int k, const void* u, size_t u_stride, const int* idx, int batch,
                         hipStream_t s);
hipError_t launch_sk_omega(void* out, size_t lane_stride, int pitch, int d, int k, unsigned long long seed, unsigned long long stream,
                           unsigned long long iteration, int normal, int batch, hipStream_t s);
hipError_t launch_sk_sub(void* a, const void* b, size_t lane_stride, int pitch, int d, int k, int batch, hipStream_t s);
struct SkAdam {
    int B, T, k, profile_stride;
    double* thetas;
    const double2* trace;
    const double2* grads;
    double *m, *v, *best_x;
    double *best_f, *profile;
    const double* lr;
    int *t, *nit, *flag;
    double beta1, beta2, eps, tol;
};
hipError_t launch_sk_adam(const SkAdam& st, int col, int do_update, hipStream_t s);

}
```

### aqc_research_amd/csrc/aqc_sweep_substage.inc

```
{
        constexpr bool kROnly = AQC_SS_RONLY;
        const bool from_regs = AQC_SS_FROM_REGS;
        unsigned nzmask = ~0u, kneed = 15u;
        if (SKIPW) {
            const unsigned info = *reinterpret_cast<const __attribute__((address_space(4))) unsigned*>(
                (const __attribute__((address_space(4))) void*)(const void*)&a.subs[st.sub_begin + si].skipinfo);
            skip_masks<TS::kGpw, NW>(st, info, se0, se1, wave, nzmask, kneed);
        }
        AQC_STAMP(2 + 4 * si);
        if (si + 1 < st.nsubs) fetch_sub<TS::kGpw>(nxt, a.subs, umat, st.sub_begin + si + 1, lane, wave, NW);
        else if (more) fetch_sub<TS::kGpw>(nxt, a.subs, a.umat + (size_t)nbl * a.nsubs_total * 12 * 64, st.sub_begin, lane, wave, NW);
        if (kPersist && more && si > 0) {
#pragma unroll
            for (int c = 0; c < 4; ++c)
                if (si == (1 + c < st.nsubs ? 1 + c : st.nsubs - 1)) prefetch(c);
        }
        if (kPersist && !seg_first)
            asm volatile("s_nop 4\n\tglobal_load_dwordx4 %0, %1, %2 sc0 sc1" : "=a"(racc) : "v"(e16), "s"(uniform_ptr(rpart + (size_t)si * a.nparts * 256)) : "memory");
        double4_t t1 = {0.0, 0.0, 0.0, 0.0}, t2 = t1, t3 = t1;
        if (!kEarly) {
            sub_addr(ad, cur, lds_base);
#pragma unroll
            for (int s = 0; s < 4; ++s) { vw[0][s] = lds_get(ad.a1 ^ ad.k1[0][s]); vz[0][s] = lds_get((ad.a1 | ZOFF) ^ ad.k1[0][s]); }
        }
        const unsigned a1z = ad.a1 | ZOFF, a2z = ad.a2 | ZOFF;
        auto group_loop = [&]() __attribute__((always_inline)) {
        constexpr bool SK = SKIPW;
        const bool from_regs_here = from_regs;
        Acc3 aw, az;
#pragma unroll
        for (int j = 0; j <= TS::kGpw; ++j) {
            if (j + 1 < TS::kGpw AQC_DBG_AND(!(a.debug & 2))) {
                if (kPersist && from_regs_here) {
#pragma unroll
                    for (int s = 0; s < 4; ++s) {
                        vw[(j + 1) & 1][s] = make_double2(pw[4 * (j + 1) + s].x, pw[4 * (j + 1) + s].y);
                        vz[(j + 1) & 1][s] = make_double2(pz[4 * (j + 1) + s].x, pz[4 * (j + 1) + s].y);
                    }
                } else {
#pragma unroll
                    for (int s = 0; s < 4; ++s) {
                        vw[(j + 1) & 1][s] = lds_get(ad.a1 ^ ad.k1[j + 1][s]);
                        vz[(j + 1) & 1][s] = lds_get(a1z ^ ad.k1[j + 1][s]);
                    }
                }
            }
            __builtin_amdgcn_sched_barrier(0);
            double sw[4], sz[4], zs[4], wd[4];
            cplx ow[4], oz[4];
            if (j < TS::kGpw) {
#pragma unroll
                for (int s = 0; s < 4; ++s) { sw[s] = vw[j & 1][s].x + vw[j & 1][s].y; sz[s] = vz[j & 1][s].x + vz[j & 1][s].y; }
            }
            if (j > 0) {
                u_combine(aw, ow);
                u_combine(az, oz);
#pragma unroll
                for (int r = 0; r < 4; ++r) { zs[r] = oz[r].x + oz[r].y; wd[r] = ow[r].x - ow[r].y; }
            }
            if (j < TS::kGpw) {
#pragma unroll
                for (int s = 0; s < 4; ++s) { asm volatile("" : "+v"(sw[s])); asm volatile("" : "+v"(sz[s])); }
            }
            if (j > 0) {
#pragma unroll
                for (int r = 0; r < 4; ++r) { asm volatile("" : "+v"(zs[r])); asm volatile("" : "+v"(wd[r])); }
            }
            unsigned wa[4], za[4];
            if (j > 0) {
#pragma unroll
                for (int r = 0; r < 4; ++r) {
                    wa[r] = ad.a2 ^ ad.k2[j - 1][r]; za[r] = a2z ^ ad.k2[j - 1][r];
                    asm volatile("" : "+v"(wa[r])); asm volatile("" : "+v"(za[r]));
                }
            }
            __builtin_amdgcn_sched_barrier(0);
            if (j < TS::kGpw) {
                aw.k1 = double4_t{0.0, 0.0, 0.0, 0.0}; aw.k2 = aw.k1; aw.k3 = aw.k1; az.k1 = aw.k1; az.k2 = aw.k1; az.k3 = aw.k1;
                if (!SK) {
#pragma unroll
                    for (int s = 0; s < (AQC_DBG_TEST(a.debug & 8) ? 0 : 4); ++s) {
                        aw.k1 = mfma(sw[s], cur.u0[s], aw.k1);
                        aw.k2 = mfma(vw[j & 1][s].x, cur.u1[s], aw.k2);
                        aw.k3 = mfma(vw[j & 1][s].y, cur.u2[s], aw.k3);
                        az.k1 = mfma(sz[s], cur.u0[s], az.k1);
                        az.k2 = mfma(vz[j & 1][s].x, cur.u1[s], az.k2);
                        az.k3 = mfma(vz[j & 1][s].y, cur.u2[s], az.k3);
                    }
                } else {
#pragma unroll
                    for (int s = 0; s < 4; ++s) {
                        az.k1 = mfma(sz[s], cur.u0[s], az.k1);
                        az.k2 = mfma(vz[j & 1][s].x, cur.u1[s], az.k2);
                        az.k3 = mfma(vz[j & 1][s].y, cur.u2[s], az.k3);
                    }
                }
            }
            if (!SK && j > 0 AQC_DBG_AND(!(a.debug & 4))) {
#pragma unroll
                for (int r = 0; r < 4; ++r) {
                    t1 = mfma(oz[r].x, ow[r].x, t1);
                    t2 = mfma(oz[r].y, ow[r].y, t2);
                    t3 = mfma(zs[r], wd[r], t3);
                }
            }
            if (j > 0 && !(SK && j == TS::kGpw) AQC_DBG_AND(!(a.debug & 1))) {
#pragma unroll
                for (int r = 0; r < 4; ++r) { lds_put(wa[r], ow[r]); lds_put(za[r], oz[r]); }
#pragma unroll
                for (int i = 0; i < 8; ++i) {
                    __builtin_amdgcn_sched_group_barrier(0x008, kSweepSpread, 0);
                    __builtin_amdgcn_sched_group_barrier(0x200, 1, 0);
                }
            }
            __builtin_amdgcn_sched_barrier(0);
            if (SK && j == TS::kGpw) {
                if (nzmask >> (j - 1) & 1u) {
#pragma unroll
                    for (int r = 0; r < 4; ++r) {
                        t1 = mfma(oz[r].x, ow[r].x, t1);
                        t2 = mfma(oz[r].y, ow[r].y, t2);
                        t3 = mfma(zs[r], wd[r], t3);
                    }
#pragma unroll
                    for (int r = 0; r < 4; ++r) { lds_put(wa[r], ow[r]); lds_put(za[r], oz[r]); }
#pragma unroll
                    for (int i = 0; i < 8; ++i) {
                        __builtin_amdgcn_sched_group_barrier(0x008, kSweepSpread, 0);
                        __builtin_amdgcn_sched_group_barrier(0x200, 1, 0);
                    }
                } else {
#pragma unroll
                    for (int r = 0; r < 4; ++r) { lds_put(wa[r], ow[r]); lds_put(za[r], oz[r]); }
                }
                __builtin_amdgcn_sched_barrier(0);
            } else
            if (SK) {
                if (j < TS::kGpw && (nzmask >> j & 1u)) {
#pragma unroll
                    for (int s = 0; s < 4; ++s)
                        if (kneed >> s & 1u) {
                            aw.k1 = mfma(sw[s], cur.u0[s], aw.k1);
                            aw.k2 = mfma(vw[j & 1][s].x, cur.u1[s], aw.k2);
                            aw.k3 = mfma(vw[j & 1][s].y, cur.u2[s], aw.k3);
                        }
                }
                if (j > 0 && (nzmask >> (j - 1) & 1u)) {
#pragma unroll
                    for (int r = 0; r < 4; ++r) {
                        t1 = mfma(oz[r].x, ow[r].x, t1);
                        t2 = mfma(oz[r].y, ow[r].y, t2);
                        t3 = mfma(zs[r], wd[r], t3);
                    }
                }
                __builtin_amdgcn_sched_barrier(0);
            }
        }
        };
        if (kROnly) {
            cplx rw[2][4], rz[2][4];
#pragma unroll
            for (int r = 0; r < 4; ++r) { rw[0][r] = lds_get(ad.a2 ^ ad.k2[0][r]); rz[0][r] = lds_get(a2z ^ ad.k2[0][r]); }
#pragma unroll
            for (int j = 0; j < TS::kGpw; ++j) {
                if (j + 1 < TS::kGpw) {
#pragma unroll
                    for (int r = 0; r < 4; ++r) { rw[(j + 1) & 1][r] = lds_get(ad.a2 ^ ad.k2[j + 1][r]); rz[(j + 1) & 1][r] = lds_get(a2z ^ ad.k2[j + 1][r]); }
                }
                __builtin_amdgcn_sched_barrier(0);
                double zs2[4], wd2[4];
#pragma unroll
                for (int r = 0; r < 4; ++r) { zs2[r] = rz[j & 1][r].x + rz[j & 1][r].y; wd2[r] = rw[j & 1][r].x - rw[j & 1][r].y; }
#pragma unroll
                for (int r = 0; r < 4; ++r) { asm volatile("" : "+v"(zs2[r])); asm volatile("" : "+v"(wd2[r])); }
                __builtin_amdgcn_sched_barrier(0);
#pragma unroll
                for (int r = 0; r < 4; ++r) {
                    t1 = mfma(rz[j & 1][r].x, rw[j & 1][r].x, t1);
                    t2 = mfma(rz[j & 1][r].y, rw[j & 1][r].y, t2);
                    t3 = mfma(zs2[r], wd2[r], t3);
                }
                __builtin_amdgcn_sched_barrier(0);
            }
        } else {
            group_loop();
        }
        AQC_STAMP(3 + 4 * si);
        if (kPersist && more && st.nsubs == 1) {
#pragma unroll
            for (int c = 0; c < 4; ++c) prefetch(c);
        }
        if (si + 1 < st.nsubs || more) fetch_k<TS::kGpw>(ad, a.subs, si + 1 < st.nsubs ? st.sub_begin + si + 1 : st.sub_begin, wave, NW);
        cplx rr[4];
#pragma unroll
        for (int r = 0; r < 4; ++r) rr[r] = make_double2(t1[r] + t2[r], t3[r] - t1[r] + t2[r]);
        cplx* scr = scratch + (kDouble ? parity * (kSlots * 256) : 0);
        parity ^= 1u;
        if (TS::kWaves > 4) {
            if (wave >= 4) {
#pragma unroll
                for (int r = 0; r < 4; ++r) scr[((wave - 4) * 4 + r) * 64 + lane] = rr[r];
            }
            __syncthreads();
            if (wave < 4) {
#pragma unroll
                for (int r = 0; r < 4; ++r) {
                    const cplx p = scr[(wave * 4 + r) * 64 + lane];
                    scr[(wave * 4 + r) * 64 + lane] = make_double2(rr[r].x + p.x, rr[r].y + p.y);
                }
            }
        } else {
#pragma unroll
            for (int r = 0; r < 4; ++r) scr[(wave * 4 + r) * 64 + lane] = rr[r];
        }
        __syncthreads();
        AQC_STAMP(4 + 4 * si);
        const bool go_on = si + 1 < st.nsubs;
        if (kEarly) {
            cplx p[kSlots];
#pragma unroll
            for (int w = 0; w < kSlots; ++w) p[w] = scr[w * 256 + threadIdx.x];
            __builtin_amdgcn_sched_barrier(0);
            if (go_on) {
                cur = nxt;
                sub_addr(ad, cur, lds_base);
#pragma unroll
                for (int s = 0; s < 4; ++s) { vw[0][s] = lds_get(ad.a1 ^ ad.k1[0][s]); vz[0][s] = lds_get((ad.a1 | ZOFF) ^ ad.k1[0][s]); }
            }
            __builtin_amdgcn_sched_barrier(0);
            double re = p[0].x, im = p[0].y;
#pragma unroll
            for (int w = 1; w < kSlots; ++w) { re += p[w].x; im += p[w].y; }
            if (kPersist && !seg_first) {
                asm volatile("s_waitcnt vmcnt(0)" : "+a"(racc) : : "memory");
                re += racc.x; im += racc.y;
            }
            rpart[(size_t)si * a.nparts * 256 + threadIdx.x] = make_double2(re, im);
            if (!kDouble) __syncthreads();
        } else {
            for (int e = threadIdx.x; e < 256; e += TS::kWaves * 64) {
                cplx p[kSlots];
#pragma unroll
                for (int w = 0; w < kSlots; ++w) p[w] = scr[w * 256 + e];
                double re = p[0].x, im = p[0].y;
#pragma unroll
                for (int w = 1; w < kSlots; ++w) { re += p[w].x; im += p[w].y; }
                rpart[(size_t)si * a.nparts * 256 + e] = make_double2(re, im);
            }
            if (!kDouble) __syncthreads();
            if (go_on) cur = nxt;
        }
        AQC_STAMP(5 + 4 * si);
        if (!go_on && more) cur = nxt;
}
```

### aqc_research_amd/csrc/aqc_ws.h

```cpp
#pragma once
#include <hip/hip_runtime_api.h>

#include <cmath>
#include <cstdarg>
#include <cstdio>
#include <cstdlib>
#include <cstring>
#include <functional>
#include <initializer_list>
#include <map>
#include <memory>
#include <mutex>
#include <string>
#include <type_traits>
#include <vector>

#include "../../include/aqc_hip.h"
#include "aqc_devbuf.h"
#include "aqc_device.h"
#include "aqc_launch.h"
#include "aqc_plan.h"

namespace aqc {

int fail(const char* fmt, ...) __attribute__((format(printf, 1, 2)));

#define HIP_OK(expr)                                                                              \
    do {                                                                                          \
        hipError_t e_ = (expr);                                                                   \
        if (e_ != hipSuccess) return ::aqc::fail("%s failed: %s (%s:%d)", #expr, hipGetErrorString(e_), __FILE__, __LINE__); \
    } while (0)

inline int ceil_log2(int v) {
    int b = 0;
    while ((1 << b) < v) ++b;
    return b;
}

enum ULevel { kUNone = 0, kURoute = 1, kUAll = 2 };

struct HostPlan {
    Plan plan;
    std::vector<DevStage> h_stages;
    std::vector<DevOp> h_ops;
    std::vector<DevSub> h_subs;
    std::vector<DevMop> h_mops;
    int k = 0, ntiles = 0, reg_bits = 0;
    bool v2 = false;
    bool v3 = false;
    std::vector<DevSub3> h_subs3;
    std::vector<DevGrp> h_grps;
    int family() const { return v3 ? 3 : (v2 ? 2 : 1); }
};
static_assert(std::is_copy_constructible<HostPlan>::value && std::is_copy_assignable<HostPlan>::value,
              "a cached plan is copied out of the cache: it owns no device memory (a buffer member would make it move-only)");

struct DevPlan : HostPlan {
    DevBuf<DevStage> d_stages;
    DevBuf<DevOp> d_ops;
    DevBuf<DevSub> d_subs;
    DevBuf<DevMop> d_mops;
    DevBuf<DevSub3> d_subs3;
    DevBuf<DevGrp> d_grps;
    DevBuf<double> d_umat;
    DevBuf<double2> d_rpart;
    int u_level = kUNone;
    DevPlan& operator=(const HostPlan& host) { HostPlan::operator=(host); return *this; }
};

struct ListKey {
    static constexpr int kUnknown = -2, kGatherOnly = -1;
    int buf = kUnknown;
    unsigned long long supp = 0, gather = 0;
    bool operator==(const ListKey& o) const { return buf != kUnknown && buf == o.buf && supp == o.supp && gather == o.gather; }
};

struct EvalRoute {
    int x_buf = AQC_BUF_X;
    bool vdag = false;
    bool new_thetas = false;
    bool gather = false;
    bool gather_rides = false;
    bool grads = false;
    bool support_in_gather_set = false;
    bool sparse = false;
    enum VdagKind { kStages, kRestricted, kProjected } vdag_kind = kStages;
    bool skip_zero_w = false;
    int key_bits() const {
        static_assert(AQC_NUM_BUFS <= 8, "x_buf takes the low three bits");
        return x_buf | (vdag ? 8 : 0) | (gather ? 16 : 0) | (gather_rides ? 32 : 0) | (grads ? 64 : 0) | (sparse ? 128 : 0) |
               (support_in_gather_set ? 256 : 0) | (skip_zero_w ? 512 : 0) | ((int)vdag_kind << 10);
    }
};

struct ProjRoute {
    bool ok = false;
    int t = 0, cb = 0, us = 0, nv = 0, nvp = 0, kv = 0, ntiles_v = 0;
    int first_subs = 0;
    Program vprog;
    std::vector<int> rest;
    DevPlan vsw;
    DevPlan vinv;
    DevBuf<double2> vm;
    DevBuf<double2> vy;
    DevBuf<double2> vme;
    DevBuf<double2> cpart;
    int cpart_shares = 0;
    int vy_copies = 1;
    unsigned l0_mask = 0;
    DevBuf<unsigned> d_tab;
    std::vector<unsigned> h_tab;
    unsigned ff_mask = 0, cb_mask = 0, tf_mask = 0;
    DevBuf<TileItem> d_items;
    DevBuf<int> d_count;
    DevBuf<int> d_lane_parts;
    ListKey init_key;
};

void lower_plan(const Program& prog, const Plan& plan, HostPlan& out, int reg_bits, bool with_dots, bool mfma = false, bool presplit = false, int beam_width = 64);
int upload_plan(DevPlan& p);
Plan mirror_plan(const Plan& plan);

}

using aqc::DevBuf; using aqc::DevPlan; using aqc::HostPlan; using aqc::PinBuf; using aqc::Program; using aqc::UJob;

struct aqc_ctx {
    Program prog;
    std::recursive_mutex mu;
    std::map<std::vector<int>, HostPlan> plan_cache;
    std::map<int, aqc_ws*> oneshot;
};

struct aqc_ws {
    aqc_ctx* ctx = nullptr;
    aqc::Switches sw;
    int device = 0, batch = 1, ncols = 1, pitch = 1, col_bits = 0, nbits = 0, threads = 256;
    size_t lane_elems = 0;
    hipStream_t stream = nullptr;
    DevPlan fwd, inv, sweep;
    double* d_thetas = nullptr;
    DevBuf<double> d_thetas_own;
    DevBuf<double> d_theta_bank;
    int bank_sets = 0, gather_count = 0;
    DevBuf<double> d_coef;
    DevBuf<double2> bufs[AQC_NUM_BUFS];
    PinBuf<double> h_pin;
    size_t pin_thetas = 0, pin_grads = 0, pin_small = 0;
    DevBuf<double2> d_partial;
    DevBuf<double2> d_grads;
    double* mirror_grads = nullptr;
    double* mirror_small = nullptr;
    DevBuf<double2> d_small;
    DevBuf<double2> d_vdot_part;
    DevBuf<double2> d_vdot_out;
    DevBuf<long long> d_index;
    DevBuf<long long> d_tmp_index;
    DevBuf<double2> d_tmp_small;
    DevBuf<long long> d_basis_index;
    DevBuf<long long> d_combo_prev[AQC_NUM_BUFS];
    bool combo_valid[AQC_NUM_BUFS] = {false, false, false, false, false, false};
    std::vector<long long> combo_last_elem[AQC_NUM_BUFS];
    std::vector<double> combo_last_coef[AQC_NUM_BUFS];
    DevBuf<char> d_sur;
    PinBuf<char> h_sur;
    int sur_states = 0;
    DevBuf<double> d_sur_real;
    DevBuf<long long> d_combo_index;
    DevBuf<double2> d_combo_coef;
    DevBuf<int> d_theta_slots;
    DevBuf<int> d_slot_theta;
    bool grads_direct = false;
    DevBuf<int> d_slot_ntiles;
    int nslots = 0, vdot_parts = 0;
    bool coef_valid = false;
    bool need_coef = false;
    std::map<std::vector<long long>, hipGraphExec_t> graphs;
    bool capturing = false;
    DevBuf<UJob> d_ujobs;
    bool ujobs_mirror = false;
    DevBuf<UJob> d_ujobs_route;
    int n_ujobs_route = 0;
    struct MpsSlot {
        std::vector<int> dims;
        std::vector<size_t> offset;
        DevBuf<double2> d_t;
    } mps[AQC_MPS_SLOTS];
    DevBuf<double> d_mps_lam;
    DevBuf<double2> d_mps_scratch;
    struct MpsTabs { std::vector<const void*> host; DevBuf<const void*> dev; unsigned long long tick = 0; };
    DevBuf<aqc::CdSegHost> d_cd_prog;
    int cd_nsteps = 0;
    DevBuf<double> d_cd_thetas;
    DevBuf<double> d_cd_fobj;
    DevBuf<double> d_cd_best;
    DevBuf<double> d_cd_real;
    DevBuf<int> d_cd_int;
    DevBuf<double> d_cd_profile;
    DevBuf<double> d_cd_part;
    MpsTabs mps_tabs[32];
    unsigned long long mps_tabs_tick = 0;
    hipEvent_t ev0 = nullptr, ev1 = nullptr, pev0 = nullptr, pev1 = nullptr;
    hipStream_t copy_stream = nullptr;
    hipEvent_t ev_ready = nullptr, ev_copied = nullptr;
    hipStream_t mps_stream = nullptr;
    hipEvent_t ev_mps_fork = nullptr, ev_mps_join = nullptr;
    bool copy_pending = false;
    const double* theta_host = nullptr;
    bool inv_mirrored = false;
    bool ckpt_valid = false;
    bool w_clean = true;
    unsigned long long supp_version[AQC_NUM_BUFS] = {0, 0, 0, 0, 0, 0};
    DevBuf<aqc::TileItem> d_sw_items;
    DevBuf<aqc::TileItem> d_sw_clear;
    DevBuf<int> d_sw_counts;
    DevBuf<int> d_sw_lane_parts;
    DevBuf<int> d_sw_prev_tiles;
    int sw_lists_built = 0;
    aqc::ListKey sw_items_key;
    DevBuf<double2> w2;
    DevBuf<double2> zw2;
    bool z_full = true;
    DevBuf<aqc::TileItem> d_vd_items;
    unsigned long long gather_gen = 0;
    aqc::ListKey vd_key;
    aqc::ListKey z_key;
    aqc::ProjRoute proj;
    bool proj_y0_ready = false;
    bool z_from_y = false;
    std::vector<long long> h_gather;
    aqc::ListKey projb_key;
    bool projb_ok = false;
    struct Sketch {
        DevBuf<double2> target;
        bool shared = false;
        DevBuf<double2> qr_part;
        DevBuf<double2> qr_rinv;
        DevBuf<double2> tmp;
        DevBuf<int> status;
        DevBuf<int> idx;
        DevBuf<double> adam;
        DevBuf<int> adam_i;
        DevBuf<double> profile;
        bool adam_started = false;
    } sk;
    bool profile = false;
    int64_t prof_count[AQC_NUM_KINDS] = {};
    double prof_ms[AQC_NUM_KINDS] = {};
    std::vector<std::pair<int, float>> prof_log;
};

namespace aqc {

struct ProfScope {
    aqc_ws* ws;
    int kind;
    ProfScope(aqc_ws* w, int k) : ws(w), kind(k) {
        if (ws->profile) (void)hipEventRecord(ws->pev0, ws->stream);
    }
    ~ProfScope() {
        if (!ws->profile) return;
        float ms = 0.f;
        if (hipEventRecord(ws->pev1, ws->stream) == hipSuccess && hipEventSynchronize(ws->pev1) == hipSuccess &&
            hipEventElapsedTime(&ms, ws->pev0, ws->pev1) == hipSuccess) {
            ws->prof_count[kind] += 1;
            ws->prof_ms[kind] += ms;
            if (ws->prof_log.size() < 100000) ws->prof_log.emplace_back(kind, ms);
        }
    }
};

inline int wait_result_copies(aqc_ws* ws) {
    if (!ws->copy_pending) return 0;
    HIP_OK(hipStreamSynchronize(ws->copy_stream));
    ws->copy_pending = false;
    return 0;
}
struct MirrorScope {
    aqc_ws* w;
    MirrorScope(aqc_ws* w_, double* grads, double* small) : w(w_) { w->mirror_grads = grads; w->mirror_small = small; }
    ~MirrorScope() { w->mirror_grads = nullptr; w->mirror_small = nullptr; w->theta_host = nullptr; }
};
inline bool direct_thetas(const aqc_ws* ws, bool zero_copy) {
    return zero_copy && ws->fwd.v3 && ws->inv.v3 && ws->sweep.v3 && !ws->need_coef;
}

int check_buf(const aqc_ws* ws, int buf);
int check_block_range(const aqc_ws* ws, int block_from, int block_to);
int ensure_coef(aqc_ws* ws);
int copy_in(aqc_ws* ws, double2* dst, const double* src, size_t rows);
int copy_out(aqc_ws* ws, double* dst, const double2* src, size_t rows);
int results_guard(aqc_ws* ws);
int before_read(aqc_ws* ws, int buf);
int before_gather(aqc_ws* ws, int buf);
int before_write(aqc_ws* ws, int buf, bool some_lanes = false);
void lhs_support_changed(aqc_ws* ws, int buf, std::vector<long long> elem = {}, std::vector<double> coef = {});
int run_coef(aqc_ws* ws, double* d_thetas);
void thetas_changed(aqc_ws* ws, double* d_thetas);
ListKey key_of(const aqc_ws* ws, int lhs_buf, bool gather);
bool built_for(const aqc_ws* ws, const ListKey& slot, const ListKey& key);
void record_key(const aqc_ws* ws, ListKey& slot, const ListKey& key);
void replay_state_after(aqc_ws* ws);
int eval_route(aqc_ws* ws, EvalRoute& route);
int enqueue_vdag(aqc_ws* ws, const EvalRoute& route);
int enqueue_gather(aqc_ws* ws, const EvalRoute& route);
void route_state_after(aqc_ws* ws, const EvalRoute& route);
int run_graph(aqc_ws* ws, const EvalRoute& route, std::initializer_list<long long> call, const std::function<int()>& enqueue);
void vdag_projected_state_after(aqc_ws* ws, int x_buf);
int grad_from_impl(aqc_ws* ws, const EvalRoute& route, int block_from, int block_to, int front_layer);
int sweep_r_only_sub(const aqc_ws* ws);
int ensure_umat(aqc_ws* ws, DevPlan& p, int need = kUAll);
int run_apply(aqc_ws* ws, bool inverse, int src_buf, int dst_buf);
Stage3Args stage3_args(aqc_ws* ws, const DevPlan& p, size_t s);
void stage3_first_list(const aqc_ws* ws, Stage3Args& a);
void stage3_sweep_fields(Stage3Args& a, const DevPlan& p, int nparts, int chunk);
void drop_graphs(aqc_ws* ws);
void proj_plan(aqc_ws* ws, int low_bits);
int proj_alloc(aqc_ws* ws);
bool list_launches_allowed(const aqc_ws* ws);
bool sweep_route_projected(const aqc_ws* ws, bool sparse);
bool projected_pairs(const aqc_ws* ws);
Stage3Args virtual_stage3_args(aqc_ws* ws, const DevPlan& v, size_t s);
Stage3Args projected_sweep_stage(aqc_ws* ws, size_t s);
int run_projected_stages(aqc_ws* ws);
aqc::RgradSecond projected_rgrad_plan(aqc_ws* ws);
bool vdag_route_projected(aqc_ws* ws, int x_buf);
int run_vdag_projected(aqc_ws* ws, int x_buf);
int proj_fix_amplitudes(aqc_ws* ws, int x_buf);
int ensure_sweep_items(aqc_ws* ws, int x_buf);

}
```

### aqc_research_amd/csrc/aqc_ws_project.cpp

```cpp
#include "aqc_ws.h"

#include <algorithm>

using namespace aqc;

namespace aqc {

namespace {
int popc(uint64_t v) { return __builtin_popcountll(v); }
unsigned deposit_bits(unsigned v, const std::vector<int>& bits) {
    unsigned o = 0;
    for (size_t j = 0; j < bits.size(); ++j)
        if (v >> j & 1) o |= 1u << bits[j];
    return o;
}
}

void proj_plan(aqc_ws* ws, int low_bits) {
    ProjRoute& pr = ws->proj;
    pr.ok = false;
    const Program& prog = ws->ctx->prog;
    const DevPlan& p = ws->sweep;
    if (!ws->sw.projected || !ws->sw.sparse_sweep || !ws->inv_mirrored || !p.v3 || ws->col_bits != 0 || ws->ncols != 1 ||
        p.plan.stages.size() < 2 || prog.n > 30 || !list_launches_allowed(ws))
        return;
    const int n = prog.n;
    uint64_t L0 = 0, T = 0;
    for (int b : p.plan.stages[0].bits) L0 |= 1ull << b;
    pr.rest.clear();
    for (size_t s = 1; s < p.plan.stages.size(); ++s)
        for (int gi : p.plan.stages[s].ops) {
            const GateGroup& g = prog.groups[gi];
            pr.rest.push_back(gi);
            T |= 1ull << g.q0;
            if (g.q1 >= 0) T |= 1ull << g.q1;
        }
    if (pr.rest.empty()) return;
    const uint64_t all = (1ull << n) - 1, F = all & ~L0, Cb = T & L0, Us = L0 & ~T;
    pr.t = popc(T); pr.cb = popc(Cb); pr.us = popc(Us);
    pr.nv = pr.t + pr.cb;
    if ((Us & 15) != 15 || pr.t < 4 || pr.cb > 6 || pr.nv + 2 > n || pr.nv > 20) return;
    pr.nvp = std::max(pr.nv, 8);
    pr.kv = std::min(pr.nvp, p.k);
    pr.ntiles_v = 1 << (pr.nvp - pr.kv);
    pr.first_subs = p.h_stages[0].nsubs;
    std::vector<int> tbits, cbits, usbits;
    std::vector<int> vq(n, -1);
    for (int b = 0; b < n; ++b) {
        if (T >> b & 1) { vq[b] = (int)tbits.size(); tbits.push_back(b); }
        if (Cb >> b & 1) cbits.push_back(b);
        if (Us >> b & 1) usbits.push_back(b);
    }
    pr.vprog = prog;
    for (int gi : pr.rest) {
        GateGroup& g = pr.vprog.groups[gi];
        g.q0 = vq[g.q0];
        if (g.q1 >= 0) g.q1 = vq[g.q1];
    }
    Plan best;
    for (int lb = std::max(low_bits, 2); lb >= 2; --lb) {
        Plan cand = make_plan(pr.vprog, 0, pr.kv, lb, false, &pr.rest, pr.nvp);
        if (best.stages.empty() || cand.stages.size() < best.stages.size()) best = cand;
    }
    lower_plan(pr.vprog, best, pr.vsw, 4, true, true, false, (int)ws->sw.projected_beam);
    if (!pr.vsw.v3 || !check_plan(pr.vprog, pr.vsw.plan, &pr.rest).empty()) return;
    lower_plan(pr.vprog, mirror_plan(pr.vsw.plan), pr.vinv, 4, false, true, true);
    if (!pr.vinv.v3 || pr.vinv.h_subs3.size() != pr.vsw.h_subs3.size()) return;
    for (DevPlan* q : {&pr.vsw, &pr.vinv})
        for (DevStage& ds : q->h_stages) {
            if (ds.nub >= 32) return;
            ds.ubits[ds.nub++] = pr.nvp;
            ds.ntiles *= 2;
        }
    pr.l0_mask = (unsigned)L0;
    pr.ff_mask = (unsigned)(F & ~T);
    pr.cb_mask = (unsigned)Cb;
    pr.tf_mask = (unsigned)(T & F);
    pr.h_tab.clear();
    for (unsigned i = 0; i < (1u << pr.t); ++i) pr.h_tab.push_back(deposit_bits(i, tbits));
    for (unsigned k = 0; k < (1u << pr.us); ++k) pr.h_tab.push_back(deposit_bits(k, usbits));
    for (unsigned c = 0; c < (1u << pr.cb); ++c) pr.h_tab.push_back(deposit_bits(c, cbits));
    for (unsigned c = 0; c < (1u << pr.cb); ++c) {
        const unsigned addr = deposit_bits(c, cbits);
        unsigned it = 0;
        for (size_t j = 0; j < tbits.size(); ++j)
            if (addr >> tbits[j] & 1) it |= 1u << j;
        pr.h_tab.push_back(it);
    }
    pr.ok = true;
    if (ws->sw.verbose)
        fprintf(stderr, "aqc_hip: projected route: the sweep's stages after the first run on %d virtual qubits (%d touched, %d shared with the first "
                "stage) instead of %d: %zu stage(s) of 2^%d tiles, %zu sub-stages\n", pr.nv, pr.t, pr.cb, n, pr.vsw.h_stages.size(), pr.kv,
                pr.vsw.h_subs3.size());
}

int proj_alloc(aqc_ws* ws) {
    ProjRoute& pr = ws->proj;
    if (!pr.ok) return 0;
    const size_t B = (size_t)ws->batch;
    if (upload_plan(pr.vsw) || upload_plan(pr.vinv)) return 1;
    const size_t nsubs = std::max<size_t>(pr.vsw.h_subs3.size(), 1);
    if (pr.vsw.d_umat.alloc(B * nsubs * 12 * 64) || pr.vinv.d_umat.alloc(B * nsubs * 12 * 64)) return 1;
    if (pr.vsw.d_rpart.alloc(B * nsubs * (2 * (size_t)pr.ntiles_v) * 256)) return 1;
    const size_t velems = B * (2ull << pr.nvp), vbytes = sizeof(double2) * velems;
    pr.vy_copies = pr.us > 8 && pr.us <= 10 && pr.cb <= 4 ? 1 << (pr.us - 8) : 1;
    if (pr.vm.alloc(velems) || pr.vy.alloc(velems * pr.vy_copies)) return 1;
    HIP_OK(hipMemsetAsync(pr.vm, 0, vbytes, ws->stream));
    HIP_OK(hipMemsetAsync(pr.vy, 0, vbytes * pr.vy_copies, ws->stream));
    pr.cpart_shares = 0;
    const long want_wgs = ws->sw.projected_fused_wgs;
    if (pr.us <= 10 && pr.cb <= 4 && (long)B < want_wgs) {
        int shares = 1;
        const long cap = ws->sw.projected_fused_max_shares;
        while ((long)B * pr.vy_copies * shares < want_wgs && 2 * shares <= (1 << (pr.t - 4)) && 2 * shares <= cap) shares *= 2;
        if (shares > 1) {
            if (pr.cpart.alloc((size_t)shares * 2 * B * (16ull << pr.us))) return 1;
            pr.cpart_shares = shares;
        }
    }
    if (pr.vme.alloc(velems)) return 1;
    HIP_OK(hipMemsetAsync(pr.vme, 0, vbytes, ws->stream));
    if (pr.d_tab.upload(pr.h_tab) || pr.d_items.alloc(2 * B * pr.ntiles_v) || pr.d_count.alloc(1) || pr.d_lane_parts.alloc(B)) return 1;
    HIP_OK(hipMemsetAsync(pr.d_count, 0, sizeof(int), ws->stream));
    HIP_OK(hipMemsetAsync(pr.d_lane_parts, 0, sizeof(int) * B, ws->stream));
    return 0;
}

bool list_launches_allowed(const aqc_ws* ws) { return ws->sweep.k < 12 || ws->sw.apply_persist > 0; }
bool sweep_route_projected(const aqc_ws* ws, bool sparse) { return sparse && ws->proj.ok; }

static ProjArgs proj_args(aqc_ws* ws);
static int ensure_pattern(aqc_ws* ws, const ProjArgs& a) {
    ProjRoute& pr = ws->proj;
    if (pr.vsw.h_stages.size() == 1 && built_for(ws, pr.init_key, ws->sw_items_key)) return 0;
    ProfScope ps(ws, AQC_K_MISC);
    HIP_OK(launch_project_init(a, ws->stream));
    record_key(ws, pr.init_key, ws->sw_items_key);
    return 0;
}

static ProjArgs proj_args(aqc_ws* ws) {
    ProjRoute& pr = ws->proj;
    ProjArgs a;
    memset(&a, 0, sizeof a);
    a.lane_stride = ws->lane_elems;
    a.items = ws->d_sw_items;
    a.nitems = ws->d_sw_counts;
    a.lane_parts = ws->d_sw_lane_parts;
    const DevStage& s0 = ws->sweep.h_stages[0];
    a.nub0 = s0.nub;
    for (int i = 0; i < s0.nub; ++i) a.ubits0[i] = s0.ubits[i];
    a.ff_mask = pr.ff_mask; a.cb_mask = pr.cb_mask; a.tf_mask = pr.tf_mask;
    a.nvp = pr.nvp;
    a.off_t = pr.d_tab;
    a.off_cb = pr.d_tab + (1u << pr.t) + (1u << pr.us);
    a.it_of_c = a.off_cb + (1u << pr.cb);
    a.off_us = pr.d_tab + (1u << pr.t);
    a.us_bits = pr.us;
    a.t = pr.t; a.cb = pr.cb; a.ntiles_v = pr.ntiles_v;
    a.vm = pr.vm;
    a.vitems = pr.d_items; a.vcount = pr.d_count; a.vlane_parts = pr.d_lane_parts;
    a.batch = ws->batch;
    return a;
}

static ProjArgs y_product(aqc_ws* ws, ProjArgs a, const double2* y) {
    const ProjRoute& pr = ws->proj;
    a.y = y;
    a.s = ws->bufs[AQC_BUF_W];
    a.out = pr.vy;
    a.s_virtual = 0; a.out_virtual = 1;
    a.staged = 1;
    a.keep_bits = pr.t; a.k_bits = pr.us;
    a.y_keep = ProjMap{a.off_t, 0};
    a.y_k = ProjMap{a.off_us, 0};
    a.s_k = ProjMap{a.off_us, 0};
    a.s_c = ProjMap{a.off_cb, 0};
    a.o_keep = ProjMap{nullptr, 0};
    a.o_c = ProjMap{nullptr, pr.t};
    return a;
}

int run_projected_stages(aqc_ws* ws) {
    ProjRoute& pr = ws->proj;
    if (!ws->proj_y0_ready) {
        const ProjArgs a = proj_args(ws);
        if (ensure_pattern(ws, a)) return 1;
        ProfScope ps(ws, AQC_K_PROJECT);
        HIP_OK(launch_project(y_product(ws, a, ws->bufs[AQC_BUF_ZW]), ws->stream));
    }
    for (size_t s = 0; s < pr.vsw.h_stages.size(); ++s) {
        const Stage3Args a = projected_sweep_stage(ws, s);
        ProfScope ps(ws, AQC_K_SWEEP_VIRTUAL);
        HIP_OK(launch_sweep3(pr.kv, ws->stream, a, ws->sw));
    }
    return 0;
}

Stage3Args virtual_stage3_args(aqc_ws* ws, const DevPlan& v, size_t s) {
    const ProjRoute& pr = ws->proj;
    Stage3Args a = stage3_args(ws, v, s);
    a.lane_stride = 2ull << pr.nvp;
    a.ntiles = 2 * pr.ntiles_v;
    a.items = pr.d_items; a.nitems = pr.d_count; a.max_items = 2 * ws->batch * pr.ntiles_v;
    return a;
}
Stage3Args projected_sweep_stage(aqc_ws* ws, size_t s) {
    const ProjRoute& pr = ws->proj;
    Stage3Args a = virtual_stage3_args(ws, pr.vsw, s);
    a.in0 = pr.vm; a.in1 = pr.vy; a.out0 = pr.vm; a.out1 = pr.vy;
    a.store_out = s + 1 < pr.vsw.h_stages.size() ? 3 : 0;
    stage3_sweep_fields(a, pr.vsw, a.ntiles, 0);
    return a;
}

bool projected_pairs(const aqc_ws* ws) {
    const ProjRoute& pr = ws->proj;
    return pr.ok && ws->sw.projected_pairs && !ws->capturing && pr.vsw.h_stages.size() == 1 && pr.vinv.h_stages.size() == 1 &&
           ws->sweep.k == pr.kv && ws->inv.k == pr.kv;
}

RgradSecond projected_rgrad_plan(aqc_ws* ws) {
    ProjRoute& pr = ws->proj;
    DevPlan& v = pr.vsw;
    RgradSecond r;
    memset(&r, 0, sizeof r);
    r.subs = v.d_subs3; r.grps = v.d_grps; r.rpart = v.d_rpart; r.lane_parts = pr.d_lane_parts; r.umat = v.d_umat;
    r.nparts = 2 * pr.ntiles_v;
    r.nsubs_total = r.count = (int)v.h_subs3.size();
    return r;
}

bool vdag_route_projected(aqc_ws* ws, int x_buf) {
    ProjRoute& pr = ws->proj;
    if (!pr.ok || !ws->sw.projected_vdag || ws->capturing || (long long)ws->lane_elems * ws->batch < ws->sw.projected_vdag_min_elems) return false;
    const ListKey key = key_of(ws, x_buf, true);
    if (ws->projb_key == key) return ws->projb_ok;
    ws->projb_key = key;
    ws->projb_ok = false;
    const std::vector<long long>& el = ws->combo_last_elem[x_buf];
    const std::vector<double>& cf = ws->combo_last_coef[x_buf];
    const size_t B = (size_t)ws->batch;
    if (el.size() != 2 * B || cf.size() != 4 * B || (ws->gather_count > 0 && ws->h_gather.size() != (size_t)ws->gather_count)) return false;
    const unsigned fmask = ~pr.l0_mask & (unsigned)((1ull << ws->ctx->prog.n) - 1);
    for (size_t b = 0; b < B; ++b) {
        if (el[2 * b] < 0 || el[2 * b + 1] >= 0 || cf[4 * b] != 1.0 || cf[4 * b + 1] != 0.0) return false;
        const unsigned e = (unsigned)el[2 * b];
        for (long long gl : ws->h_gather) {
            const unsigned d = e ^ (unsigned)gl;
            if ((d & fmask) == 0) continue;
            if ((d & pr.l0_mask) != 0 || (d & pr.ff_mask) != 0) return false;
        }
    }
    ws->projb_ok = true;
    return true;
}

struct VirtualRun { const DevPlan& plan; const double2* src; double2* dst; };
static Stage3Args virtual_apply_stage(aqc_ws* ws, const VirtualRun& v, size_t s) {
    Stage3Args a = virtual_stage3_args(ws, v.plan, s);
    a.in0 = s == 0 ? v.src : v.dst;
    a.out0 = v.dst;
    return a;
}
static int enqueue_couple(aqc_ws* ws, int k, const Stage3Args* real, const VirtualRun* v) {
    if (real && v) {
        ProfScope ps(ws, AQC_K_APPLY_VIRTUAL);
        HIP_OK(launch_apply3_pair(k, ws->stream, *real, virtual_apply_stage(ws, *v, 0), ws->sw));
    } else if (real) {
        ProfScope ps(ws, AQC_K_APPLY_LIST);
        HIP_OK(launch_apply3(k, ws->stream, *real, ws->sw));
    } else {
        for (size_t s = 0; s < v->plan.h_stages.size(); ++s) {
            ProfScope ps(ws, AQC_K_APPLY_VIRTUAL);
            HIP_OK(launch_apply3(ws->proj.kv, ws->stream, virtual_apply_stage(ws, *v, s), ws->sw));
        }
    }
    return 0;
}

int run_vdag_projected(aqc_ws* ws, int x_buf) {
    ProjRoute& pr = ws->proj;
    const DevPlan& p = ws->sweep;
    const DevPlan& iv = ws->inv;
    if (ensure_umat(ws, ws->inv, kURoute)) return 1;
    if (!ws->d_sw_items || !ws->w_clean) return fail("objective by projection without the sparse route's preparation");
    if (ensure_sweep_items(ws, x_buf)) return 1;
    Stage3Args psi = stage3_args(ws, p, 0);
    psi.in0 = ws->bufs[x_buf];
    psi.out0 = ws->bufs[AQC_BUF_W];
    stage3_first_list(ws, psi);
    Stage3Args last = stage3_args(ws, iv, iv.h_stages.size() - 1);
    last.in0 = ws->bufs[AQC_BUF_ZW];
    last.out0 = ws->bufs[AQC_BUF_Z];
    stage3_first_list(ws, last);
    const VirtualRun mend{pr.vsw, pr.vm, pr.vme};
    const VirtualRun y0{pr.vinv, pr.vy, pr.vy};
    const ProjArgs a = proj_args(ws);
    const bool pairs = projected_pairs(ws);

    if (!pairs && enqueue_couple(ws, p.k, &psi, nullptr)) return 1;
    if (ensure_pattern(ws, a)) return 1;
    if (enqueue_couple(ws, p.k, pairs ? &psi : nullptr, &mend)) return 1;
    if (ws->sw.projected_fused && pr.us <= 10 && pr.cb <= 4 && (pr.us <= 8 || pr.vy_copies == 1 << (pr.us - 8))) {
        ProjArgs q = a;
        q.part_stride = (size_t)ws->batch * (2ull << pr.nvp);
        q.cpart = pr.cpart; q.cpart_shares = pr.cpart_shares;
        q.y = ws->bufs[AQC_BUF_Y]; q.s = ws->bufs[AQC_BUF_W];
        ProfScope ps(ws, AQC_K_PROJECT);
        HIP_OK(launch_project_fused(q, pr.vme, ws->bufs[AQC_BUF_ZW], pr.vy, ws->stream, ws->sw.projected_fused_qb == 4 ? 4 : 2));
    } else {
        {
            ProfScope ps(ws, AQC_K_PROJECT);
            HIP_OK(launch_project(y_product(ws, a, ws->bufs[AQC_BUF_Y]), ws->stream));
        }
        ProjArgs q = a;
        q.y = ws->bufs[AQC_BUF_Y]; q.s = pr.vme; q.out = ws->bufs[AQC_BUF_ZW];
        q.s_virtual = 1; q.out_virtual = 0; q.staged = 0;
        q.keep_bits = pr.us; q.k_bits = pr.t;
        q.y_keep = ProjMap{a.off_us, 0}; q.y_k = ProjMap{a.off_t, 0};
        q.s_k = ProjMap{nullptr, 0}; q.s_c = ProjMap{nullptr, pr.t};
        q.o_keep = ProjMap{a.off_us, 0}; q.o_c = ProjMap{a.off_cb, 0};
        ProfScope ps(ws, AQC_K_PROJECT);
        HIP_OK(launch_project(q, ws->stream));
    }
    if (!pairs && enqueue_couple(ws, iv.k, nullptr, &y0)) return 1;
    if (enqueue_couple(ws, iv.k, &last, pairs ? &y0 : nullptr)) return 1;
    vdag_projected_state_after(ws, x_buf);
    return 0;
}

int proj_fix_amplitudes(aqc_ws* ws, int x_buf) {
    ProjRoute& pr = ws->proj;
    if (results_guard(ws)) return 1;
    ProfScope ps(ws, AQC_K_MISC);
    ProjArgs a = proj_args(ws);
    HIP_OK(launch_project_amps(a, ws->d_index, ws->gather_count, ws->d_combo_prev[x_buf], ws->d_small, pr.vy, ws->bufs[AQC_BUF_Z], ws->stream));
    return 0;
}

}
```

### aqc_research_amd/csrc/aqc_ws_sweep.cpp

```cpp
#include "aqc_ws.h"

#include <algorithm>

using namespace aqc;

namespace aqc {


void thetas_changed(aqc_ws* ws, double* d_thetas) {
    ws->d_thetas = d_thetas;
    ws->coef_valid = true;
    ws->fwd.u_level = ws->inv.u_level = ws->sweep.u_level = kUNone;
    ws->ckpt_valid = false;
    ws->z_from_y = false;
    ws->proj_y0_ready = false;
}

static void umat_state_after(aqc_ws* ws, const DevPlan& p, int level = kUAll) {
    if (!p.v3) return;
    if (&p == &ws->fwd) ws->fwd.u_level = kUAll;
    else ws->inv.u_level = ws->sweep.u_level = std::max(ws->sweep.u_level, level);
}
static int route_level(const aqc_ws* ws) { return ws->d_ujobs_route ? kURoute : kUAll; }

static int ensure_z_full(aqc_ws* ws, bool reader);

static void touch_buf(aqc_ws* ws, int buf) {
    ws->combo_valid[buf] = false;
    if (buf == AQC_BUF_Z || buf == AQC_BUF_ZW) ws->ckpt_valid = false;
    if (buf == AQC_BUF_Y || buf == AQC_BUF_Z) ws->z_from_y = false;
    ws->proj_y0_ready = false;
    if (buf == AQC_BUF_Z) ws->z_full = true;
    if (buf == AQC_BUF_W) ws->w_clean = false;
}

int before_read(aqc_ws* ws, int buf) { return buf == AQC_BUF_Z ? ensure_z_full(ws, true) : 0; }

int before_gather(aqc_ws* ws, int buf) {
    return buf == AQC_BUF_Z && !ws->z_full && ws->z_key.gather != ws->gather_gen ? ensure_z_full(ws, true) : 0;
}

int before_write(aqc_ws* ws, int buf, bool some_lanes) {
    if (buf == AQC_BUF_ZW && ensure_z_full(ws, false)) return 1;
    if (buf == AQC_BUF_Z && some_lanes && ws->batch > 1 && ensure_z_full(ws, true)) return 1;
    touch_buf(ws, buf);
    return 0;
}

void lhs_support_changed(aqc_ws* ws, int buf, std::vector<long long> elem, std::vector<double> coef) {
    touch_buf(ws, buf);
    ws->combo_valid[buf] = true;
    ++ws->supp_version[buf];
    ws->combo_last_elem[buf].swap(elem);
    ws->combo_last_coef[buf].swap(coef);
}

ListKey key_of(const aqc_ws* ws, int lhs_buf, bool gather) {
    return ListKey{lhs_buf, lhs_buf >= 0 ? ws->supp_version[lhs_buf] : 0, gather ? ws->gather_gen : 0};
}
bool built_for(const aqc_ws* ws, const ListKey& slot, const ListKey& key) { return !ws->capturing && slot == key; }
void record_key(const aqc_ws* ws, ListKey& slot, const ListKey& key) { slot = ws->capturing ? ListKey{} : key; }

void replay_state_after(aqc_ws* ws) { ws->sw_items_key = ws->vd_key = ws->proj.init_key = ListKey{}; }

int ensure_umat(aqc_ws* ws, DevPlan& p, int need) {
    if (!p.v3) return 0;
    if (&p != &ws->fwd && need == kURoute) need = route_level(ws);
    if (p.u_level >= need) return 0;
    const int T = ws->ctx->prog.num_thetas();
    const int ninv = ws->inv.v3 && !ws->ujobs_mirror ? (int)ws->inv.h_subs3.size() : 0;
    int nsw = ws->sweep.v3 ? (int)ws->sweep.h_subs3.size() : 0;
    const int nfwd = ws->fwd.v3 ? (int)ws->fwd.h_subs3.size() : 0;
    const int nvs = ws->proj.ok ? (int)ws->proj.vsw.h_subs3.size() : 0;
    nsw += nvs;
    ProfScope ps(ws, AQC_K_COEF);
    if (&p == &ws->fwd) {
        HIP_OK(launch_ubuild(ws->d_ujobs + ninv + nsw, nfwd, ws->d_thetas, T, ws->batch, ws->stream));
    } else {
        const bool subset = need == kURoute;
        HIP_OK(launch_ubuild(subset ? ws->d_ujobs_route : ws->d_ujobs, subset ? ws->n_ujobs_route : ninv + nsw,
                             ws->theta_host ? ws->theta_host : ws->d_thetas, T, ws->batch, ws->stream, ws->theta_host ? ws->d_thetas : nullptr));
        ws->theta_host = nullptr;
    }
    umat_state_after(ws, p, need);
    return 0;
}

int run_coef(aqc_ws* ws, double* d_thetas) {
    const Program& prog = ws->ctx->prog;
    thetas_changed(ws, d_thetas);
    if (ws->fwd.v3 && ws->inv.v3 && ws->sweep.v3 && !ws->need_coef) return 0;
    ProfScope ps(ws, AQC_K_COEF);
    HIP_OK(launch_coef(ws->d_thetas, ws->d_coef, prog.n, prog.num_blocks, prog.tpb, prog.tail_blocks, ws->batch, ws->stream));
    return 0;
}

#ifdef AQC_TUNING
namespace {
unsigned long long* g_stamps = nullptr;
int stamps_begin(aqc_ws* ws, Stage3Args& a, size_t nwg) {
    if (!ws->sw.stamps || nwg > 65536) return 0;
    if (!g_stamps) HIP_OK(hipMalloc((void**)&g_stamps, sizeof(unsigned long long) * 65536 * kStampSlots));
    HIP_OK(hipMemsetAsync(g_stamps, 0, sizeof(unsigned long long) * nwg * kStampSlots, ws->stream));
    a.stamps = g_stamps;
    return 0;
}
int stamps_apply(aqc_ws* ws, const Stage3Args& a, size_t s, size_t nwg) {
    if (!a.stamps) return 0;
    std::vector<unsigned long long> h(nwg * kStampSlots);
    HIP_OK(hipStreamSynchronize(ws->stream));
    HIP_OK(hipMemcpy(h.data(), g_stamps, sizeof(unsigned long long) * h.size(), hipMemcpyDeviceToHost));
    double load = 0, loop = 0, store = 0, bar = 0;
    const int ns = a.stage.nsubs;
    for (size_t w = 0; w < nwg; ++w) {
        const unsigned long long* t = h.data() + w * kStampSlots;
        load += (double)(t[1] - t[0]); loop += (double)(t[2] - t[1]); store += (double)(t[3] - t[2]);
        for (int i = 0; i < ns && 5 + i < kStampSlots; ++i) bar += (double)(t[5 + i] - t[4 + i]);
    }
    fprintf(stderr, "aqc_hip stamps: V/V^H stage %zu (%d sub-stages, %zu workgroups): load %.0f + sub-stage loop %.0f (%.0f per sub-stage, of which "
            "waiting at its barrier %.0f) + store %.0f cycles per workgroup\n", s, ns, nwg, load / nwg, loop / nwg, loop / nwg / std::max(ns, 1),
            bar / nwg / std::max(ns, 1), store / nwg);
    return 0;
}
int stamps_sweep(aqc_ws* ws, const Stage3Args& a, size_t s, size_t nwg) {
    if (!a.stamps) return 0;
    std::vector<unsigned long long> h(nwg * kStampSlots);
    HIP_OK(hipStreamSynchronize(ws->stream));
    HIP_OK(hipMemcpy(h.data(), g_stamps, sizeof(unsigned long long) * h.size(), hipMemcpyDeviceToHost));
    const int ns = a.stage.nsubs;
    double load = 0, store = 0, total = 0, mf = 0, bar = 0, red = 0, top = 0, turn = 0;
    size_t live = 0;
    unsigned long long first_start = ~0ull, last_start = 0, first_end = ~0ull, last_end = 0, wg_min = ~0ull, wg_max = 0;
    for (size_t w = 0; w < nwg; ++w) {
        const unsigned long long* t = h.data() + w * kStampSlots;
        if (t[kStampSlots - 4] == 0) continue;
        ++live;
        first_start = std::min(first_start, t[0]); last_start = std::max(last_start, t[0]);
        first_end = std::min(first_end, t[kStampSlots - 4]); last_end = std::max(last_end, t[kStampSlots - 4]);
        wg_min = std::min(wg_min, t[kStampSlots - 4] - t[0]); wg_max = std::max(wg_max, t[kStampSlots - 4] - t[0]);
        load += (double)(t[1] - t[0]);
        store += (double)(t[kStampSlots - 1] - t[kStampSlots - 2]);
        total += (double)(t[kStampSlots - 4] - t[0]);
        if (t[kStampSlots - 5]) turn += (double)(t[kStampSlots - 5] - t[kStampSlots - 6]);
        for (int i = 0; i < ns && 5 + 4 * i < kStampSlots - 6; ++i) {
            if (i) top += (double)(t[2 + 4 * i] - t[5 + 4 * (i - 1)]);
            mf += (double)(t[3 + 4 * i] - t[2 + 4 * i]);
            bar += (double)(t[4 + 4 * i] - t[3 + 4 * i]);
            red += (double)(t[5 + 4 * i] - t[4 + 4 * i]);
        }
    }
    const double n = (double)std::max<size_t>(live, 1), items = (double)nwg / n;
    fprintf(stderr, "aqc_hip stamps: stage %zu (%d sub-stages, %zu workgroups x %.1f items): total %.0f cycles per item = first load %.0f/items + "
            "per sub-stage [top %.0f + mfma loop %.0f + scratch/barrier %.0f + reduce %.0f] + store %.0f + hand-over %.0f\n", s, ns, live, items,
            total / n / items, load / n, top / n / std::max(ns - 1, 1), mf / n / ns, bar / n / ns, red / n / ns, store / n, turn / n);
    fprintf(stderr, "aqc_hip stamps: stage %zu workgroup lifetimes (s_memtime ticks): min %llu max %llu; starts spread over %llu, ends over %llu; "
            "first start -> last end %llu\n", s, wg_min, wg_max, last_start - first_start, last_end - first_end, last_end - first_start);
    return 0;
}
}
#endif

Stage3Args stage3_args(aqc_ws* ws, const DevPlan& p, size_t s) {
    Stage3Args a;
    memset(&a, 0, sizeof a);
    a.stage = p.h_stages[s];
    a.subs = p.d_subs3;
    a.umat = p.d_umat;
    a.nsubs_total = (int)p.h_subs3.size();
    a.lane_stride = ws->lane_elems;
    a.ntiles = p.ntiles;
    a.batch = ws->batch;
    return a;
}
void stage3_first_list(const aqc_ws* ws, Stage3Args& a) {
    a.items = ws->d_sw_items; a.nitems = ws->d_sw_counts; a.max_items = 2 * ws->batch;
}
void stage3_sweep_fields(Stage3Args& a, const DevPlan& p, int nparts, int chunk) {
    a.rpart = p.d_rpart;
    a.nparts = nparts;
    a.chunk = chunk;
    if (a.stage.nsubs > 0) stage3_first_offsets(a, p.h_subs3[a.stage.sub_begin]);
}

static StageArgs stage_args(const aqc_ws* ws, const DevPlan& p, size_t s) {
    const Program& prog = ws->ctx->prog;
    StageArgs a;
    memset(&a, 0, sizeof a);
    a.stage = p.d_stages + s; a.ops = p.d_ops; a.subs = p.d_subs; a.mops = p.d_mops;
    a.coef = ws->d_coef; a.ncoef = prog.n + prog.num_blocks + 1;
    a.lane_stride = ws->lane_elems;
    return a;
}

static bool keeps_checkpoint(const aqc_ws* ws, bool inverse, int src_buf, int dst_buf) {
    return inverse && ws->inv_mirrored && ws->inv.v3 && dst_buf == AQC_BUF_Z && src_buf != AQC_BUF_ZW && ws->inv.h_stages.size() >= 2;
}
static void apply_state_after(aqc_ws* ws, bool inverse, int src_buf, int dst_buf, int level = kUAll) {
    umat_state_after(ws, inverse ? ws->inv : ws->fwd, level);
    touch_buf(ws, dst_buf);
    if (keeps_checkpoint(ws, inverse, src_buf, dst_buf)) { touch_buf(ws, AQC_BUF_ZW); ws->ckpt_valid = true; }
}

int run_apply(aqc_ws* ws, bool inverse, int src_buf, int dst_buf) {
    DevPlan& p = inverse ? ws->inv : ws->fwd;
    const Program& prog = ws->ctx->prog;
    if (before_read(ws, src_buf) || before_write(ws, dst_buf)) return 1;
    if (p.v3) {
        if (ensure_umat(ws, p)) return 1;
        const bool keep = keeps_checkpoint(ws, inverse, src_buf, dst_buf);
        const size_t m = p.h_stages.size();
        for (size_t s = 0; s < m; ++s) {
            Stage3Args a = stage3_args(ws, p, s);
            const int mid = keep ? AQC_BUF_ZW : dst_buf;
            a.in0 = s == 0 ? ws->bufs[src_buf] : ws->bufs[mid];
            a.out0 = s + 1 == m ? ws->bufs[dst_buf] : ws->bufs[mid];
#ifdef AQC_TUNING
            const size_t nwg = (size_t)p.ntiles * ws->batch;
            if (stamps_begin(ws, a, nwg)) return 1;
#endif
            {
                ProfScope ps(ws, AQC_K_APPLY);
                HIP_OK(launch_apply3(p.k, ws->stream, a, ws->sw));
            }
#ifdef AQC_TUNING
            if (stamps_apply(ws, a, s, nwg)) return 1;
#endif
        }
        apply_state_after(ws, inverse, src_buf, dst_buf);
        return 0;
    }
    for (size_t s = 0; s < p.h_stages.size(); ++s) {
        StageArgs a = stage_args(ws, p, s);
        a.in0 = s == 0 ? ws->bufs[src_buf] : ws->bufs[dst_buf];
        a.out0 = ws->bufs[dst_buf];
        a.final_stage = (s + 1 == p.h_stages.size()) ? 1 : 0;
        ProfScope ps(ws, AQC_K_APPLY);
        if (p.v2) HIP_OK(launch_apply2(prog.entangler, p.ntiles, ws->batch, p.k, ws->stream, a));
        else HIP_OK(launch_apply(prog.entangler, inverse, p.ntiles, ws->batch, ws->threads, p.k, ws->stream, a));
    }
    apply_state_after(ws, inverse, src_buf, dst_buf);
    return 0;
}

static bool vdag_route_restricted(const aqc_ws* ws) {
    return ws->sw.lazy_z && 2 + ws->gather_count <= kMaxTileCands;
}
static Stage3Args last_vdag_stage(aqc_ws* ws) {
    DevPlan& p = ws->inv;
    Stage3Args a = stage3_args(ws, p, p.h_stages.size() - 1);
    a.in0 = ws->bufs[AQC_BUF_ZW];
    a.out0 = ws->bufs[AQC_BUF_Z];
    return a;
}
static void vdag_restricted_state_after(aqc_ws* ws, int x_buf, int level = kUAll) {
    apply_state_after(ws, true, AQC_BUF_Y, AQC_BUF_Z, level);
    ws->z_full = false;
    ws->z_key = key_of(ws, x_buf, true);
}
void vdag_projected_state_after(aqc_ws* ws, int x_buf) {
    vdag_restricted_state_after(ws, x_buf, route_level(ws));
    ws->z_key.gather = 0;
    ws->ckpt_valid = false;
    ws->z_from_y = true;
    ws->proj_y0_ready = true;
}
static int run_vdag_restricted(aqc_ws* ws, int x_buf, bool support_in_gather_set) {
    DevPlan& p = ws->inv;
    if (ensure_umat(ws, p)) return 1;
    const size_t m = p.h_stages.size();
    const size_t per_lane = 2 + (size_t)ws->gather_count;
    if (ws->d_vd_items.capacity() < per_lane * ws->batch) return fail("objective V^H inside a captured graph without its preparation");
    for (size_t s = 0; s + 1 < m; ++s) {
        Stage3Args a = stage3_args(ws, p, s);
        a.in0 = s == 0 ? ws->bufs[AQC_BUF_Y] : ws->bufs[AQC_BUF_ZW];
        a.out0 = ws->bufs[AQC_BUF_ZW];
        ProfScope ps(ws, AQC_K_APPLY);
        HIP_OK(launch_apply3(p.k, ws->stream, a, ws->sw));
    }
    const bool gather_only = support_in_gather_set && ws->gather_count > 0;
    const ListKey key = key_of(ws, gather_only ? ListKey::kGatherOnly : x_buf, true);
    if (!built_for(ws, ws->vd_key, key)) {
        ProfScope ps(ws, AQC_K_MISC);
        HIP_OK(launch_tile_items(p.h_stages[m - 1], gather_only ? nullptr : ws->d_combo_prev[x_buf], 2, ws->gather_count > 0 ? ws->d_index : nullptr,
                                 ws->gather_count, ws->batch, ws->d_vd_items, ws->d_sw_counts + 2, nullptr, nullptr, nullptr, nullptr, ws->stream));
        record_key(ws, ws->vd_key, key);
    }
    Stage3Args a = last_vdag_stage(ws);
    a.items = ws->d_vd_items;
    a.nitems = ws->d_sw_counts + 2;
    a.max_items = (int)(per_lane * ws->batch);
    ws->sw_lists_built |= 2;
    {
        ProfScope ps(ws, AQC_K_APPLY_LIST);
        HIP_OK(launch_apply3(p.k, ws->stream, a, ws->sw));
    }
    vdag_restricted_state_after(ws, x_buf);
    return 0;
}
static int ensure_z_full(aqc_ws* ws, bool reader) {
    if (ws->z_full) return 0;
    if (ws->capturing) return fail("BUF_Z is partial inside a captured graph");
    if (ws->ckpt_valid && ws->inv.u_level != kUNone) {
        if (ensure_umat(ws, ws->inv)) return 1;
        Stage3Args a = last_vdag_stage(ws);
        ProfScope ps(ws, AQC_K_APPLY);
        HIP_OK(launch_apply3(ws->inv.k, ws->stream, a, ws->sw));
        ws->z_full = true;
        return 0;
    }
    if (!reader) return 0;
    if (ws->z_from_y && ws->inv.u_level != kUNone) {
        ws->z_full = true;
        return run_apply(ws, true, AQC_BUF_Y, AQC_BUF_Z);
    }
    return fail("BUF_Z holds V^H y only on the tiles the last one-call evaluation read, and the thetas (or ZW) have changed since: "
                "run aqc_ws_apply(inverse) for the whole vector");
}

void drop_graphs(aqc_ws* ws) {
    for (auto& kv : ws->graphs) (void)hipGraphExecDestroy(kv.second);
    ws->graphs.clear();
}

static bool sweep_route_sparse(const aqc_ws* ws, int x_buf, bool will_vdag) {
    const DevPlan& p = ws->sweep;
    if (!ws->sw.sparse_sweep || !p.v3 || !ws->inv_mirrored || p.h_stages.size() < 2) return false;
    if (!list_launches_allowed(ws)) return false;
    if (!ws->combo_valid[x_buf] || !ws->d_combo_prev[x_buf]) return false;
    if (!(will_vdag ? keeps_checkpoint(ws, true, AQC_BUF_Y, AQC_BUF_Z) : (ws->ckpt_valid || ws->proj_y0_ready))) return false;
    return (long)p.ntiles * ws->batch >= ws->sw.sparse_min_items;
}
int sweep_r_only_sub(const aqc_ws* ws) {
    const DevPlan& p = ws->sweep;
    if (!p.v3 || !ws->sw.r_only_last || p.h_stages.empty()) return -1;
    const DevStage& last = p.h_stages.back();
    if (last.nsubs < 1 || last.nsubs > ws->sw.r_only_max_subs || (p.k >= 12 && last.nsubs == 1)) return -1;
    return last.sub_begin + last.nsubs - 1;
}
static bool sweep_skips_zero_w(const aqc_ws* ws, int x_buf) {
    return ws->sw.skip_zero_w && ws->sweep.v3 && ws->combo_valid[x_buf] && ws->d_combo_prev[x_buf] != nullptr;
}
static int sweep_sparse_prepare(aqc_ws* ws) {
    const DevPlan& p = ws->sweep;
    const int B = ws->batch;
    if (!ws->d_sw_items) {
        if (ws->d_sw_items.alloc(2 * (size_t)B) || ws->d_sw_clear.alloc(2 * (size_t)B) || ws->d_sw_counts.alloc(4)) return 1;
        HIP_OK(hipMemsetAsync(ws->d_sw_counts, 0, sizeof(int) * 4, ws->stream));
        if (ws->d_sw_lane_parts.alloc(B) || ws->d_sw_prev_tiles.alloc(2 * (size_t)B)) return 1;
        ws->w_clean = false;
    }
    if (p.h_stages.size() >= 3 && !ws->w2 && !ws->proj.ok) {
        if (ws->w2.alloc((size_t)B * ws->lane_elems) || ws->zw2.alloc((size_t)B * ws->lane_elems)) return 1;
    }
    const size_t vd_need = (2 + (size_t)ws->gather_count) * B;
    if (ws->sw.lazy_z && ws->d_vd_items.capacity() < vd_need) {
        HIP_OK(hipStreamSynchronize(ws->stream));
        if (ws->d_vd_items.reserve(vd_need)) return 1;
        ws->vd_key = ListKey{};
    }
    if (!ws->w_clean) {
        HIP_OK(hipMemsetAsync(ws->bufs[AQC_BUF_W], 0, sizeof(double2) * (size_t)B * ws->lane_elems, ws->stream));
        HIP_OK(hipMemsetAsync(ws->d_sw_prev_tiles, 0xff, sizeof(int) * 2 * B, ws->stream));
        ws->w_clean = true;
        ws->sw_items_key = ListKey{};
    }
    return 0;
}
static void sweep_state_after(aqc_ws* ws, bool sparse) {
    umat_state_after(ws, ws->sweep, sweep_route_projected(ws, sparse) ? route_level(ws) : kUAll);
    ws->proj_y0_ready = false;
    if (!sparse) {
        ws->w_clean = false;
        ws->ckpt_valid = false;
    }
}

int eval_route(aqc_ws* ws, EvalRoute& r) {
    r.sparse = r.grads && (r.vdag || !r.new_thetas) && sweep_route_sparse(ws, r.x_buf, r.vdag);
    r.skip_zero_w = r.grads && sweep_skips_zero_w(ws, r.x_buf);
    r.vdag_kind = EvalRoute::kStages;
    if (r.sparse && sweep_sparse_prepare(ws)) return 1;
    if (!(r.sparse && r.vdag && vdag_route_restricted(ws))) return 0;
    const bool projected = !r.gather_rides && !r.support_in_gather_set && vdag_route_projected(ws, r.x_buf);
    r.vdag_kind = projected ? EvalRoute::kProjected : EvalRoute::kRestricted;
    return 0;
}
int enqueue_vdag(aqc_ws* ws, const EvalRoute& r) {
    if (r.vdag_kind == EvalRoute::kProjected) return run_vdag_projected(ws, r.x_buf);
    if (r.vdag_kind == EvalRoute::kRestricted) return run_vdag_restricted(ws, r.x_buf, r.support_in_gather_set);
    return run_apply(ws, true, AQC_BUF_Y, AQC_BUF_Z);
}
int enqueue_gather(aqc_ws* ws, const EvalRoute& r) {
    return r.vdag_kind == EvalRoute::kProjected ? proj_fix_amplitudes(ws, r.x_buf) : aqc_ws_gather_launch(ws, AQC_BUF_Z);
}
void route_state_after(aqc_ws* ws, const EvalRoute& r) {
    if (r.vdag && r.vdag_kind == EvalRoute::kProjected) vdag_projected_state_after(ws, r.x_buf);
    else if (r.vdag && r.vdag_kind == EvalRoute::kRestricted) vdag_restricted_state_after(ws, r.x_buf);
    else if (r.vdag) apply_state_after(ws, true, AQC_BUF_Y, AQC_BUF_Z);
    if (r.support_in_gather_set) lhs_support_changed(ws, r.x_buf);
    if (r.grads) sweep_state_after(ws, r.sparse);
}
static std::vector<long long> graph_key(const aqc_ws* ws, const EvalRoute& r, std::initializer_list<long long> call) {
    std::vector<long long> key;
    key.reserve(call.size() + 5);
    key.insert(key.end(), call.begin(), call.end());
    key.push_back(r.key_bits());
    for (const void* addr : {(const void*)ws->d_small, (const void*)ws->h_pin, (const void*)ws->d_combo_prev[r.x_buf], (const void*)ws->d_vd_items})
        key.push_back((long long)(size_t)addr);
    return key;
}

int run_graph(aqc_ws* ws, const EvalRoute& route, std::initializer_list<long long> call, const std::function<int()>& enqueue) {
    const std::vector<long long> key = graph_key(ws, route, call);
    auto it = ws->graphs.find(key);
    if (it == ws->graphs.end()) {
        hipGraph_t graph = nullptr;
        hipGraphExec_t exec = nullptr;
        HIP_OK(hipStreamSynchronize(ws->stream));
        HIP_OK(hipStreamBeginCapture(ws->stream, hipStreamCaptureModeThreadLocal));
        ws->capturing = true;
        const int rc = enqueue();
        ws->capturing = false;
        const hipError_t e = hipStreamEndCapture(ws->stream, &graph);
        if (rc != 0) { if (graph) (void)hipGraphDestroy(graph); return 1; }
        if (e != hipSuccess || !graph) return fail("hipStreamEndCapture failed: %s", hipGetErrorString(e));
        const hipError_t ei = hipGraphInstantiate(&exec, graph, nullptr, nullptr, 0);
        (void)hipGraphDestroy(graph);
        if (ei != hipSuccess) return fail("hipGraphInstantiate failed: %s", hipGetErrorString(ei));
        if (ws->graphs.size() >= 16) drop_graphs(ws);
        it = ws->graphs.emplace(key, exec).first;
    }
    thetas_changed(ws, ws->d_thetas_own);
    route_state_after(ws, route);
    replay_state_after(ws);
    HIP_OK(hipGraphLaunch(it->second, ws->stream));
    return 0;
}

int ensure_sweep_items(aqc_ws* ws, int x_buf) {
    const DevPlan& p = ws->sweep;
    const ListKey key = key_of(ws, x_buf, false);
    if (!built_for(ws, ws->sw_items_key, key)) {
        ProfScope ps(ws, AQC_K_MISC);
        HIP_OK(launch_tile_items(p.h_stages[0], ws->d_combo_prev[x_buf], 2, nullptr, 0, ws->batch, ws->d_sw_items, ws->d_sw_counts,
                                 ws->d_sw_lane_parts, ws->d_sw_prev_tiles, ws->d_sw_clear, ws->d_sw_counts + 1, ws->stream));
        HIP_OK(launch_clear_tiles(p.h_stages[0], ws->bufs[AQC_BUF_W], ws->lane_elems, ws->d_sw_clear, ws->d_sw_counts + 1, 2 * ws->batch, ws->stream));
        record_key(ws, ws->sw_items_key, key);
        ws->sw_lists_built |= 1;
    }
    return 0;
}

static int sweep_mfma(aqc_ws* ws, const EvalRoute& route, int block_from, int block_to, int front_layer) {
    const Program& prog = ws->ctx->prog;
    DevPlan& p = ws->sweep;
    const int x_buf = route.x_buf;
    const int nsubs = (int)p.h_subs3.size();
    const size_t m = p.h_stages.size();
    const int nparts = sweep3_nparts(p.ntiles, ws->batch, p.k, ws->sw.sweep_grid), chunk = sweep3_chunk(p.ntiles, ws->batch, p.k, ws->sw.sweep_grid);
    const bool sparse = route.sparse, skipw = route.skip_zero_w;
    const bool projected = sweep_route_projected(ws, sparse);
    if (ensure_umat(ws, p, projected ? kURoute : kUAll)) return 1;
    int r_only_sub = skipw || projected ? -1 : sweep_r_only_sub(ws);
    const bool first_stage_r_only = projected && ws->proj_y0_ready && ws->sw.r_only_last && p.h_stages[0].nsubs >= 2 &&
                                    p.h_stages[0].nsubs <= ws->sw.r_only_max_subs;
    if (first_stage_r_only) r_only_sub = p.h_stages[0].sub_begin + p.h_stages[0].nsubs - 1;
    bool pair_virtual = projected && ws->proj_y0_ready && projected_pairs(ws);
#ifdef AQC_TUNING
    if (ws->sw.stamps) pair_virtual = false;
#endif
    if (!ws->z_full && !(sparse && ((route.support_in_gather_set && ws->z_key.gather == ws->gather_gen) ||
                                    (ws->z_key.buf == x_buf && ws->z_key.supp == ws->supp_version[x_buf]))) && ensure_z_full(ws, true))
        return 1;
    if (sparse) {
        if (!ws->d_sw_items || !ws->w_clean || (m >= 3 && !ws->w2 && !projected)) return fail("sparse sweep inside a captured graph without its preparation");
        if (ensure_sweep_items(ws, x_buf)) return 1;
    }
    for (size_t s = 0; s < (projected ? 1 : m); ++s) {
        Stage3Args a = stage3_args(ws, p, s);
        if (sparse) {
            double2* w2 = m >= 3 ? ws->w2 : nullptr;
            double2* z2 = m >= 3 ? ws->zw2 : nullptr;
            a.in0 = s == 0 ? ws->bufs[x_buf] : (s == 1 ? ws->bufs[AQC_BUF_W] : w2);
            a.in1 = s == 0 ? ws->bufs[AQC_BUF_Z] : (s == 1 ? ws->bufs[AQC_BUF_ZW] : z2);
            a.out0 = s == 0 ? ws->bufs[AQC_BUF_W] : w2;
            a.out1 = s == 0 ? nullptr : z2;
            a.store_out = s + 1 < m ? (s == 0 ? 1 : 3) : 0;
            if (s == 0) stage3_first_list(ws, a);
            if (s == 0 && first_stage_r_only) { a.r_only_last = 1; a.store_out = 0; }
        } else {
            a.in0 = s == 0 ? ws->bufs[x_buf] : ws->bufs[AQC_BUF_W];
            a.in1 = s == 0 ? ws->bufs[AQC_BUF_Z] : ws->bufs[AQC_BUF_ZW];
            a.out0 = ws->bufs[AQC_BUF_W];
            a.out1 = ws->bufs[AQC_BUF_ZW];
            a.store_out = s + 1 < m ? 3 : 0;
        }
        if (skipw && !a.items) a.supp = ws->d_combo_prev[x_buf];
        if (s + 1 == m && r_only_sub >= 0) a.r_only_last = 1;
        stage3_sweep_fields(a, p, nparts, chunk);
#ifdef AQC_TUNING
        const size_t nwg = (size_t)p.ntiles * ws->batch;
        a.debug = (int)ws->sw.debug_skip;
        if (stamps_begin(ws, a, nwg)) return 1;
#endif
        if (pair_virtual) {
            const Stage3Args b = projected_sweep_stage(ws, 0);
            ProfScope ps(ws, AQC_K_SWEEP_LIST);
            HIP_OK(launch_sweep3_pair(p.k, ws->stream, a, b, ws->sw));
        } else {
            ProfScope ps(ws, a.items ? AQC_K_SWEEP_LIST : AQC_K_SWEEP);
            HIP_OK(launch_sweep3(p.k, ws->stream, a, ws->sw));
        }
#ifdef AQC_TUNING
        if (stamps_sweep(ws, a, s, nwg)) return 1;
#endif
    }
    if (projected && !pair_virtual && run_projected_stages(ws)) return 1;
    sweep_state_after(ws, sparse);
    ProfScope ps(ws, AQC_K_FINALIZE);
    RgradSecond vwalk;
    if (projected) vwalk = projected_rgrad_plan(ws);
    HIP_OK(launch_rgrad(p.d_subs3, p.d_grps, prog.entangler, ws->d_thetas, prog.num_thetas(), p.d_rpart, p.ntiles, nsubs, ws->d_partial,
                        ws->nslots, block_from, block_to, front_layer ? 1 : 0, ws->batch, ws->stream,
                        ws->grads_direct ? ws->d_slot_theta : nullptr, ws->d_grads, ws->mirror_grads,
                        route.gather_rides ? GatherJob{ws->bufs[AQC_BUF_Z], ws->lane_elems, ws->d_index, ws->gather_count, ws->d_small, ws->mirror_small}
                                         : GatherJob{nullptr, 0, nullptr, 0, nullptr, nullptr},
                        nparts, chunk,
                        sparse ? p.h_stages[0].nsubs : 0, sparse ? ws->d_sw_lane_parts : nullptr, r_only_sub, p.d_umat,
                        projected ? p.h_stages[0].nsubs : -1, projected ? &vwalk : nullptr));
#ifdef AQC_TUNING
    if (ws->sw.stamps) { HIP_OK(hipStreamSynchronize(ws->stream)); rgrad_print_stamps(nsubs); }
#endif
    if (!ws->grads_direct)
        HIP_OK(launch_finalize(ws->d_partial, ws->d_theta_slots, ws->d_slot_ntiles, ws->d_grads, prog.num_thetas(), ws->nslots,
                               1, prog.n, prog.tpb, block_from, block_to, front_layer ? 1 : 0, ws->batch, ws->stream, ws->mirror_grads));
    return 0;
}

static int sweep_valu(aqc_ws* ws, int x_buf, int block_from, int block_to, int front_layer) {
    const Program& prog = ws->ctx->prog;
    DevPlan& p = ws->sweep;
    if (before_read(ws, AQC_BUF_Z)) return 1;
    for (size_t s = 0; s < p.h_stages.size(); ++s) {
        StageArgs a = stage_args(ws, p, s);
        a.in0 = s == 0 ? ws->bufs[x_buf] : ws->bufs[AQC_BUF_W];
        a.in1 = s == 0 ? ws->bufs[AQC_BUF_Z] : ws->bufs[AQC_BUF_ZW];
        a.out0 = ws->bufs[AQC_BUF_W];
        a.out1 = ws->bufs[AQC_BUF_ZW];
        a.partial = ws->d_partial; a.nslots = ws->nslots; a.ntiles_max = p.ntiles;
#ifdef AQC_TUNING
        a.debug = (int)ws->sw.debug_skip;
#endif
        a.from = block_from; a.to = block_to; a.front = front_layer ? 1 : 0;
        ProfScope ps(ws, AQC_K_SWEEP);
        if (p.v2) HIP_OK(launch_sweep2(prog.entangler, p.ntiles, ws->batch, p.k, p.reg_bits, ws->stream, a));
        else HIP_OK(launch_sweep(prog.entangler, p.ntiles, ws->batch, ws->threads, p.k, ws->stream, a));
    }
    sweep_state_after(ws, false);
    ProfScope ps(ws, AQC_K_FINALIZE);
    HIP_OK(launch_finalize(ws->d_partial, ws->d_theta_slots, ws->d_slot_ntiles, ws->d_grads, prog.num_thetas(), ws->nslots,
                           p.ntiles, prog.n, prog.tpb, block_from, block_to, front_layer ? 1 : 0, ws->batch, ws->stream, ws->mirror_grads));
    return 0;
}

static int sweep_refused(aqc_ws* ws, int x_buf, int block_from, int block_to) {
    if (check_buf(ws, x_buf)) return 1;
    if (x_buf == AQC_BUF_W || x_buf == AQC_BUF_ZW || x_buf == AQC_BUF_Z) return fail("lhs buffer must not be Z, W or ZW");
    return ensure_coef(ws) || check_block_range(ws, block_from, block_to);
}

int grad_from_impl(aqc_ws* ws, const EvalRoute& route, int block_from, int block_to, int front_layer) {
    const int x_buf = route.x_buf;
    if (sweep_refused(ws, x_buf, block_from, block_to) || results_guard(ws)) return 1;
    if (block_from < 0) { block_from = 0; block_to = ws->ctx->prog.num_blocks; }
    HIP_OK(hipSetDevice(ws->device));
    return ws->sweep.v3 ? sweep_mfma(ws, route, block_from, block_to, front_layer) : sweep_valu(ws, x_buf, block_from, block_to, front_layer);
}

}

extern "C" {

int aqc_ws_apply(aqc_ws* ws, int inverse, int src_buf, int dst_buf) {
    if (check_buf(ws, src_buf) || check_buf(ws, dst_buf)) return 1;
    if (ensure_coef(ws)) return 1;
    HIP_OK(hipSetDevice(ws->device));
    return run_apply(ws, inverse != 0, src_buf, dst_buf);
}

int aqc_ws_sweep_r_only_sub(aqc_ws* ws) { return ws ? sweep_r_only_sub(ws) : -1; }

int aqc_ws_grad(aqc_ws* ws, int block_from, int block_to, int front_layer) {
    return aqc_ws_grad_from(ws, AQC_BUF_X, block_from, block_to, front_layer);
}

int aqc_ws_grad_from(aqc_ws* ws, int x_buf, int block_from, int block_to, int front_layer) {
    if (sweep_refused(ws, x_buf, block_from, block_to)) return 1;
    HIP_OK(hipSetDevice(ws->device));
    EvalRoute route;
    route.x_buf = x_buf; route.grads = true;
    if (eval_route(ws, route)) return 1;
    return grad_from_impl(ws, route, block_from, block_to, front_layer);
}

int aqc_ws_objective_launch(aqc_ws* ws, int x_buf, int block_from, int block_to, int front_layer) {
    if (check_buf(ws, x_buf)) return 1;
    if (x_buf == AQC_BUF_W || x_buf == AQC_BUF_ZW || x_buf == AQC_BUF_Z || x_buf == AQC_BUF_Y) return fail("lhs buffer must be X or X2");
    if (check_block_range(ws, block_from, block_to)) return 1;
    if (ensure_coef(ws)) return 1;
    HIP_OK(hipSetDevice(ws->device));
    EvalRoute route;
    route.x_buf = x_buf; route.vdag = route.grads = true; route.gather = ws->gather_count > 0;
    if (eval_route(ws, route)) return 1;
    if (enqueue_vdag(ws, route)) return 1;
    if (route.gather && enqueue_gather(ws, route)) return 1;
    return grad_from_impl(ws, route, block_from, block_to, front_layer);
}

int aqc_ws_eval(aqc_ws* ws, const double* thetas, int do_vdag, double* gathered, int x_buf, int block_from, int block_to,
                int front_layer, double* grads) {
    if (!ws) return fail("null workspace");
    HIP_OK(hipSetDevice(ws->device));
    if (wait_result_copies(ws)) return 1;
    const Program& prog = ws->ctx->prog;
    const size_t nth = (size_t)ws->batch * prog.num_thetas();
    double* pin_th = ws->h_pin;
    double* pin_gr = ws->h_pin + ws->pin_thetas;
    double* pin_sm = pin_gr + ws->pin_grads;
    size_t nsm = 0;
    if (gathered) {
        if (ws->gather_count < 1) return fail("aqc_ws_gather_setup has not been called");
        nsm = (size_t)ws->batch * ws->gather_count;
        if (2 * nsm > ws->pin_small) return fail("too many gathered amplitudes for the staging buffer");
    }
    if (check_buf(ws, x_buf)) return 1;
    if (grads && check_block_range(ws, block_from, block_to)) return 1;
    if (!thetas && (do_vdag || grads) && ensure_coef(ws)) return 1;
    const bool zero_copy = sizeof(double2) * (nth + nsm) <= 65536;
    MirrorScope mirror_scope(ws, zero_copy ? pin_gr : nullptr, zero_copy ? pin_sm : nullptr);
    if (!do_vdag && (gathered || grads) && before_read(ws, AQC_BUF_Z)) return 1;
    EvalRoute route;
    route.x_buf = x_buf; route.vdag = do_vdag != 0; route.new_thetas = thetas != nullptr;
    route.gather = gathered != nullptr; route.grads = grads != nullptr;
    route.gather_rides = gathered && grads && zero_copy && ws->sweep.v3;
    if (eval_route(ws, route)) return 1;
    auto enqueue = [&]() -> int {
        if (thetas) {
            const bool direct = (do_vdag || grads) && direct_thetas(ws, zero_copy);
            if (!direct) HIP_OK(hipMemcpyAsync(ws->d_thetas_own, pin_th, sizeof(double) * nth, hipMemcpyHostToDevice, ws->stream));
            if (run_coef(ws, ws->d_thetas_own)) return 1;
            ws->theta_host = direct ? pin_th : nullptr;
        }
        if (route.vdag && enqueue_vdag(ws, route)) return 1;
        if (route.gather && !route.gather_rides) {
            if (enqueue_gather(ws, route)) return 1;
            if (!zero_copy) HIP_OK(hipMemcpyAsync(pin_sm, ws->d_small, sizeof(double2) * nsm, hipMemcpyDeviceToHost, ws->stream));
        }
        if (grads) {
            if (grad_from_impl(ws, route, block_from, block_to, front_layer)) return 1;
            if (!zero_copy) HIP_OK(hipMemcpyAsync(pin_gr, ws->d_grads, sizeof(double2) * nth, hipMemcpyDeviceToHost, ws->stream));
        }
        ws->theta_host = nullptr;
        return 0;
    };
    if (thetas) memcpy(pin_th, thetas, sizeof(double) * nth);
    if (thetas && ws->sw.graph && !ws->profile) {
        if (run_graph(ws, route, {0, block_from, block_to, front_layer, (long long)ws->gather_count}, enqueue)) return 1;
    } else if (enqueue()) {
        return 1;
    }
    HIP_OK(hipStreamSynchronize(ws->stream));
    if (gathered) memcpy(gathered, pin_sm, sizeof(double2) * nsm);
    if (grads) memcpy(grads, pin_gr, sizeof(double2) * nth);
    return 0;
}

}
```

Measured before the change: 1.180 million evals/s.

## Fuse last inverse stage into gradient sweep via backward walk

```diff
diff --git a/aqc_research_amd/csrc/aqc_backwalk.h b/aqc_research_amd/csrc/aqc_backwalk.h
--- /dev/null
+++ b/aqc_research_amd/csrc/aqc_backwalk.h
@@ -0,0 +1,17 @@
+#pragma once
+
+#if defined(__HIPCC__) || defined(__CUDACC__)
+#define AQC_BW_HD __host__ __device__
+#else
+#define AQC_BW_HD
+#endif
+
+namespace aqc {
+
+AQC_BW_HD constexpr int backwalk_r_slot(int nsubs_total, int mirrored_sub) { return nsubs_total - 1 - mirrored_sub; }
+
+AQC_BW_HD constexpr int backwalk_conj_sub(int nsubs_total, int mirrored_sub_begin) { return backwalk_r_slot(nsubs_total, mirrored_sub_begin); }
+
+AQC_BW_HD constexpr bool backwalk_tile(int k) { return k >= 8 && k <= 12 && k != 11; }
+
+}
diff --git a/aqc_research_amd/csrc/aqc_kernels3.hip b/aqc_research_amd/csrc/aqc_kernels3.hip
--- a/aqc_research_amd/csrc/aqc_kernels3.hip
+++ b/aqc_research_amd/csrc/aqc_kernels3.hip
@@ -4,6 +4,7 @@
 
 #include <type_traits>
 
+#include "aqc_backwalk.h"
 #include "aqc_device.h"
 #include "aqc_launch.h"
 #include "aqc_math.h"
@@ -406,9 +407,10 @@
             if (((s2 ^ kb) & kfresh) == 0) kneed |= 1u << s2;
     }
 }
-template <int K, bool LIST, bool SKIPW, bool RLAST>
+template <int K, bool LIST, bool SKIPW, bool RLAST, bool BACK = false>
 __device__ __forceinline__ void sweep_mfma_body(const Stage3Args& a, const int wg, const int nwg) {
     using TS = TileShape<K, true>;
+    static_assert(!BACK || (LIST && !SKIPW && !RLAST), "the backward walk is a list launch with a form of its own");
     constexpr int kSlots = TS::kWaves > 4 ? 4 : TS::kWaves;
     constexpr unsigned tsize = 1u << K;
     extern __shared__ __attribute__((aligned(16))) char smem[];
@@ -480,7 +482,7 @@
     const double* umat = a.umat + (size_t)bl * a.nsubs_total * 12 * 64;
     const int part = LIST ? it.slot : (kPersist ? wg - (bl * a.ntiles) / chunk : tile);
     const bool seg_first = LIST || !kPersist || wi == wi_first || tile == 0;
-    cplx* rpart = a.rpart + (((size_t)bl * a.nsubs_total + st.sub_begin) * a.nparts + part) * 256;
+    cplx* rpart = a.rpart + (((size_t)bl * a.nsubs_total + (BACK ? 0 : st.sub_begin)) * a.nparts + part) * 256;
     const int nwi = wi + 1;
     const bool more = reg_first && nwi < wi_end;
     const ItemAt nit = more ? item_at<LIST>(a, nwi) : ItemAt{0, 0, 0};
@@ -508,37 +510,75 @@
             }
     };
     const int nmain = RLAST && a.r_only_last && st.nsubs >= 1 && !(kPersist && st.nsubs == 1) ? st.nsubs - 1 : st.nsubs;
-    if (!RLAST) {
+    if constexpr (BACK) {
+        {
+            const int si = 0;
+#define AQC_SS_FROM_REGS reg_first
+#define AQC_SS_RONLY false
+#define AQC_SS_BACK 0
+#include "aqc_sweep_substage.inc"
+#undef AQC_SS_FROM_REGS
+#undef AQC_SS_RONLY
+#undef AQC_SS_BACK
+        }
+        for (int si = 1; si + 1 < st.nsubs; ++si) {
+#define AQC_SS_FROM_REGS false
+#define AQC_SS_RONLY false
+#define AQC_SS_BACK 1
+#include "aqc_sweep_substage.inc"
+#undef AQC_SS_FROM_REGS
+#undef AQC_SS_RONLY
+#undef AQC_SS_BACK
+        }
+        {
+            const int si = st.nsubs - 1;
+#define AQC_SS_FROM_REGS false
+#define AQC_SS_RONLY false
+#define AQC_SS_BACK 2
+#include "aqc_sweep_substage.inc"
+#undef AQC_SS_FROM_REGS
+#undef AQC_SS_RONLY
+#undef AQC_SS_BACK
+        }
+    } else if (!RLAST) {
         for (int si = 0; si < st.nsubs; ++si) {
 #define AQC_SS_FROM_REGS (reg_first && si == 0)
 #define AQC_SS_RONLY false
+#define AQC_SS_BACK 0
 #include "aqc_sweep_substage.inc"
 #undef AQC_SS_FROM_REGS
 #undef AQC_SS_RONLY
+#undef AQC_SS_BACK
         }
     } else {
         if (nmain > 0) {
             const int si = 0;
 #define AQC_SS_FROM_REGS reg_first
 #define AQC_SS_RONLY false
+#define AQC_SS_BACK 0
 #include "aqc_sweep_substage.inc"
 #undef AQC_SS_FROM_REGS
 #undef AQC_SS_RONLY
+#undef AQC_SS_BACK
         }
         for (int si = 1; si < nmain; ++si) {
 #define AQC_SS_FROM_REGS false
 #define AQC_SS_RONLY false
+#define AQC_SS_BACK 0
 #include "aqc_sweep_substage.inc"
 #undef AQC_SS_FROM_REGS
 #undef AQC_SS_RONLY
+#undef AQC_SS_BACK
         }
         if (nmain < st.nsubs) {
             const int si = nmain;
 #define AQC_SS_FROM_REGS false
 #define AQC_SS_RONLY true
+#define AQC_SS_BACK 0
 #include "aqc_sweep_substage.inc"
 #undef AQC_SS_FROM_REGS
 #undef AQC_SS_RONLY
+#undef AQC_SS_BACK
         }
     }
     AQC_STAMP(kStampSlots - 2);
@@ -558,18 +598,18 @@
     }
     AQC_STAMP(kStampSlots - 4);
 }
-template <int K, bool LIST = false, bool SKIPW = false, bool RLAST = false>
+template <int K, bool LIST = false, bool SKIPW = false, bool RLAST = false, bool BACK = false>
 __global__ __launch_bounds__(SweepShape<K>::kWaves * 64, K >= 12 ? 1 : 2) void sweep_mfma_kernel(const Stage3Args a) {
-    sweep_mfma_body<K, LIST, SKIPW, RLAST>(a, (int)blockIdx.x, (int)gridDim.x);
-}
-template <int K, bool RLAST_A, bool RLAST_B>
+    sweep_mfma_body<K, LIST, SKIPW, RLAST, BACK>(a, (int)blockIdx.x, (int)gridDim.x);
+}
+template <int K, bool RLAST_A, bool RLAST_B, bool BACK_A = false>
 __global__ __launch_bounds__(SweepShape<K>::kWaves * 64, K >= 12 ? 1 : 2) void sweep_pair_kernel(const Stage3Args a, const Stage3Args b, const int grid_a) {
     if (K >= 12) {
-        sweep_mfma_body<K, true, false, RLAST_A>(a, (int)blockIdx.x, (int)gridDim.x);
+        sweep_mfma_body<K, true, false, RLAST_A, BACK_A>(a, (int)blockIdx.x, (int)gridDim.x);
         __syncthreads();
         sweep_mfma_body<K, true, false, RLAST_B>(b, (int)blockIdx.x, (int)gridDim.x);
     } else if ((int)blockIdx.x < grid_a) {
-        sweep_mfma_body<K, true, false, RLAST_A>(a, (int)blockIdx.x, grid_a);
+        sweep_mfma_body<K, true, false, RLAST_A, BACK_A>(a, (int)blockIdx.x, grid_a);
     } else {
         sweep_mfma_body<K, true, false, RLAST_B>(b, (int)blockIdx.x - grid_a, (int)gridDim.x - grid_a);
     }
@@ -998,13 +1038,14 @@
 using Stage3Kernel = void (*)(Stage3Args);
 using Pair3Kernel = void (*)(Stage3Args, Stage3Args, int);
 template <int K> static Stage3Kernel apply_variant(bool list) { return list ? apply_mfma_kernel<K, true> : apply_mfma_kernel<K, false>; }
-template <int K> static Stage3Kernel sweep_variant(bool list, bool skipw, bool rlast) {
+template <int K> static Stage3Kernel sweep_variant(bool list, bool skipw, bool rlast, bool back = false) {
+    if (back) return backwalk_tile(K) ? sweep_mfma_kernel<K, true, false, false, backwalk_tile(K)> : nullptr;
     if (list) return rlast ? sweep_mfma_kernel<K, true, false, true> : sweep_mfma_kernel<K, true, false, false>;
     if (skipw) return sweep_mfma_kernel<K, false, true, false>;
     return rlast ? sweep_mfma_kernel<K, false, false, true> : sweep_mfma_kernel<K, false, false, false>;
 }
 template <int K> static Pair3Kernel apply_pair_variant() { return apply_pair_kernel<K>; }
-template <int K> static Pair3Kernel sweep_pair_variant(bool rlast_a) { return rlast_a ? sweep_pair_kernel<K, true, false> : sweep_pair_kernel<K, false, false>; }
+template <int K> static Pair3Kernel sweep_pair_variant(bool rlast_a, bool back_a = false) { return back_a ? (backwalk_tile(K) ? sweep_pair_kernel<K, false, false, backwalk_tile(K)> : nullptr) : rlast_a ? sweep_pair_kernel<K, true, false> : sweep_pair_kernel<K, false, false>; }
 
 template <typename F>
 static hipError_t big_lds(F kernel) {
@@ -1018,6 +1059,8 @@
             hipError_t e = big_lds(apply_pair_variant<K>());
             for (int f = 0; f < 2 && e == hipSuccess; ++f) e = big_lds(apply_variant<K>(f));
             for (int f = 0; f < 2 && e == hipSuccess; ++f) e = big_lds(sweep_pair_variant<K>(f));
+            if (backwalk_tile(K) && e == hipSuccess) e = big_lds(sweep_pair_variant<K>(false, true));
+            if (backwalk_tile(K) && e == hipSuccess) e = big_lds(sweep_variant<K>(true, false, false, true));
             for (int f = 0; f < 8 && e == hipSuccess; ++f) e = big_lds(sweep_variant<K>(f & 1, f & 2, f & 4));
             return e;
         });
@@ -1082,6 +1125,7 @@
     const int chunk = sweep3_chunk(ntiles, batch, k, sweep_grid);
     return chunk > 0 ? std::min(ntiles, (ntiles + chunk - 1) / chunk + 1) : ntiles;
 }
+static bool backwalk_launchable(int k, const Stage3Args& a) { return backwalk_tile(k) && a.items && !a.supp && !a.r_only_last && a.stage.nsubs >= 2; }
 hipError_t launch_sweep3(int k, hipStream_t s, const Stage3Args& a, const Switches& sw) {
     const bool list = a.items != nullptr;
     if (!stage3_launchable(k, a, false, true)) return hipErrorInvalidValue;
@@ -1090,15 +1134,17 @@
     const dim3 grid((unsigned)(k >= 12 ? (list ? std::min<long>(nwork, persistent_sweep_grid(sw.sweep_grid)) : (nwork + a.chunk - 1) / a.chunk) : nwork));
     const bool skipw = !list && a.supp != nullptr;
     const bool rlast = !skipw && a.r_only_last != 0;
-    return with_tile_size(k, [&](auto kk) { return launch3(sweep_variant<decltype(kk)::value>(list, skipw, rlast), grid, k, true, s, a); });
+    const bool back = a.backwalk != 0;
+    if (back && !backwalk_launchable(k, a)) return hipErrorInvalidValue;
+    return with_tile_size(k, [&](auto kk) { return launch3(sweep_variant<decltype(kk)::value>(list, skipw, rlast, back), grid, k, true, s, a); });
 }
 
 hipError_t launch_sweep3_pair(int k, hipStream_t s, const Stage3Args& a, const Stage3Args& b, const Switches& sw) {
     if (!stage3_launchable(k, a, true, true) || !stage3_launchable(k, b, true, true)) return hipErrorInvalidValue;
-    if (a.nparts < 1 || b.nparts < 1 || a.supp || b.supp || b.r_only_last) return hipErrorInvalidValue;
+    if (a.nparts < 1 || b.nparts < 1 || a.supp || b.supp || b.r_only_last || b.backwalk || (a.backwalk && !backwalk_launchable(k, a))) return hipErrorInvalidValue;
     const long longer = std::max(a.max_items, b.max_items);
     const dim3 grid((unsigned)(k >= 12 ? std::min<long>(longer, persistent_sweep_grid(sw.sweep_grid)) : (long)a.max_items + b.max_items));
-    return with_tile_size(k, [&](auto kk) { return launch3(sweep_pair_variant<decltype(kk)::value>(a.r_only_last != 0), grid, k, true, s, a, b, a.max_items); });
+    return with_tile_size(k, [&](auto kk) { return launch3(sweep_pair_variant<decltype(kk)::value>(a.r_only_last != 0, a.backwalk != 0), grid, k, true, s, a, b, a.max_items); });
 }
 
 __device__ __forceinline__ int tile_of_elem(const DevStage& st, long long e) {
diff --git a/aqc_research_amd/csrc/aqc_launch.h b/aqc_research_amd/csrc/aqc_launch.h
--- a/aqc_research_amd/csrc/aqc_launch.h
+++ b/aqc_research_amd/csrc/aqc_launch.h
@@ -68,6 +68,7 @@
     int chunk, nparts;
     int store_out;
     int r_only_last;
+    int backwalk;
     const long long* supp;
     const TileItem* items;
     const int* nitems;
diff --git a/aqc_research_amd/csrc/aqc_sweep_substage.inc b/aqc_research_amd/csrc/aqc_sweep_substage.inc
--- a/aqc_research_amd/csrc/aqc_sweep_substage.inc
+++ b/aqc_research_amd/csrc/aqc_sweep_substage.inc
@@ -1,5 +1,7 @@
 {
         constexpr bool kROnly = AQC_SS_RONLY;
+        constexpr int kBack = AQC_SS_BACK;
+        cplx* const rps = rpart + (size_t)(BACK ? backwalk_r_slot(a.nsubs_total, st.sub_begin + si) : si) * a.nparts * 256;
         const bool from_regs = AQC_SS_FROM_REGS;
         unsigned nzmask = ~0u, kneed = 15u;
         if (SKIPW) {
@@ -16,7 +18,7 @@
                 if (si == (1 + c < st.nsubs ? 1 + c : st.nsubs - 1)) prefetch(c);
         }
         if (kPersist && !seg_first)
-            asm volatile("s_nop 4\n\tglobal_load_dwordx4 %0, %1, %2 sc0 sc1" : "=a"(racc) : "v"(e16), "s"(uniform_ptr(rpart + (size_t)si * a.nparts * 256)) : "memory");
+            asm volatile("s_nop 4\n\tglobal_load_dwordx4 %0, %1, %2 sc0 sc1" : "=a"(racc) : "v"(e16), "s"(uniform_ptr(rps)) : "memory");
         double4_t t1 = {0.0, 0.0, 0.0, 0.0}, t2 = t1, t3 = t1;
         if (!kEarly) {
             sub_addr(ad, cur, lds_base);
@@ -182,6 +184,89 @@
                 }
                 __builtin_amdgcn_sched_barrier(0);
             }
+        } else if (kBack != 0) {
+            constexpr bool kBoth = kBack == 1;
+            cplx rw[4], rz[4];
+#pragma unroll
+            for (int r = 0; r < 4; ++r) { rw[r] = lds_get(ad.a2 ^ ad.k2[0][r]); rz[r] = lds_get(a2z ^ ad.k2[0][r]); }
+            Acc3 aw, az;
+#pragma unroll
+            for (int j = 0; j <= TS::kGpw; ++j) {
+                if (j + 1 < TS::kGpw) {
+#pragma unroll
+                    for (int s = 0; s < 4; ++s) {
+                        if (kBoth) vw[(j + 1) & 1][s] = lds_get(ad.a1 ^ ad.k1[j + 1][s]);
+                        vz[(j + 1) & 1][s] = lds_get(a1z ^ ad.k1[j + 1][s]);
+                    }
+                }
+                __builtin_amdgcn_sched_barrier(0);
+                double sw[4], sz[4], zs2[4], wd2[4];
+                cplx ow[4], oz[4];
+                if (j < TS::kGpw) {
+#pragma unroll
+                    for (int s = 0; s < 4; ++s) {
+                        if (kBoth) sw[s] = vw[j & 1][s].x + vw[j & 1][s].y;
+                        sz[s] = vz[j & 1][s].x + vz[j & 1][s].y;
+                        zs2[s] = rz[s].x + rz[s].y; wd2[s] = rw[s].x - rw[s].y;
+                    }
+                }
+                if (j > 0) {
+                    if (kBoth) u_combine(aw, ow);
+                    u_combine(az, oz);
+                }
+                if (j < TS::kGpw) {
+#pragma unroll
+                    for (int s = 0; s < 4; ++s) {
+                        if (kBoth) asm volatile("" : "+v"(sw[s]));
+                        asm volatile("" : "+v"(sz[s])); asm volatile("" : "+v"(zs2[s])); asm volatile("" : "+v"(wd2[s]));
+                    }
+                }
+                unsigned wa[4], za[4];
+                if (j > 0) {
+#pragma unroll
+                    for (int r = 0; r < 4; ++r) {
+                        if (kBoth) { wa[r] = ad.a2 ^ ad.k2[j - 1][r]; asm volatile("" : "+v"(wa[r])); }
+                        za[r] = a2z ^ ad.k2[j - 1][r]; asm volatile("" : "+v"(za[r]));
+                    }
+                }
+                __builtin_amdgcn_sched_barrier(0);
+                if (j < TS::kGpw) {
+#pragma unroll
+                    for (int r = 0; r < 4; ++r) {
+                        t1 = mfma(rz[r].x, rw[r].x, t1);
+                        t2 = mfma(rz[r].y, rw[r].y, t2);
+                        t3 = mfma(zs2[r], wd2[r], t3);
+                    }
+                    if (j + 1 < TS::kGpw) {
+#pragma unroll
+                        for (int r = 0; r < 4; ++r) { rw[r] = lds_get(ad.a2 ^ ad.k2[j + 1][r]); rz[r] = lds_get(a2z ^ ad.k2[j + 1][r]); }
+                    }
+                    az.k1 = double4_t{0.0, 0.0, 0.0, 0.0}; az.k2 = az.k1; az.k3 = az.k1; aw.k1 = az.k1; aw.k2 = az.k1; aw.k3 = az.k1;
+#pragma unroll
+                    for (int s = 0; s < 4; ++s) {
+                        if (kBoth) {
+                            aw.k1 = mfma(sw[s], cur.u0[s], aw.k1);
+                            aw.k2 = mfma(vw[j & 1][s].x, cur.u1[s], aw.k2);
+                            aw.k3 = mfma(vw[j & 1][s].y, cur.u2[s], aw.k3);
+                        }
+                        az.k1 = mfma(sz[s], cur.u0[s], az.k1);
+                        az.k2 = mfma(vz[j & 1][s].x, cur.u1[s], az.k2);
+                        az.k3 = mfma(vz[j & 1][s].y, cur.u2[s], az.k3);
+                    }
+                }
+                if (j > 0) {
+#pragma unroll
+                    for (int r = 0; r < 4; ++r) { if (kBoth) lds_put(wa[r], ow[r]); lds_put(za[r], oz[r]); }
+                    if (j < TS::kGpw) {
+#pragma unroll
+                        for (int i = 0; i < (kBoth ? 8 : 4); ++i) {
+                            __builtin_amdgcn_sched_group_barrier(0x008, kSweepSpread, 0);
+                            __builtin_amdgcn_sched_group_barrier(0x200, 1, 0);
+                        }
+                    }
+                }
+                __builtin_amdgcn_sched_barrier(0);
+            }
         } else {
             group_loop();
         }
@@ -235,7 +320,7 @@
                 asm volatile("s_waitcnt vmcnt(0)" : "+a"(racc) : : "memory");
                 re += racc.x; im += racc.y;
             }
-            rpart[(size_t)si * a.nparts * 256 + threadIdx.x] = make_double2(re, im);
+            rps[threadIdx.x] = make_double2(re, im);
             if (!kDouble) __syncthreads();
         } else {
             for (int e = threadIdx.x; e < 256; e += TS::kWaves * 64) {
@@ -245,7 +330,7 @@
                 double re = p[0].x, im = p[0].y;
 #pragma unroll
                 for (int w = 1; w < kSlots; ++w) { re += p[w].x; im += p[w].y; }
-                rpart[(size_t)si * a.nparts * 256 + e] = make_double2(re, im);
+                rps[e] = make_double2(re, im);
             }
             if (!kDouble) __syncthreads();
             if (go_on) cur = nxt;
diff --git a/aqc_research_amd/csrc/aqc_ws.h b/aqc_research_amd/csrc/aqc_ws.h
--- a/aqc_research_amd/csrc/aqc_ws.h
+++ b/aqc_research_amd/csrc/aqc_ws.h
@@ -16,6 +16,7 @@
 #include <vector>
 
 #include "../../include/aqc_hip.h"
+#include "aqc_backwalk.h"
 #include "aqc_devbuf.h"
 #include "aqc_device.h"
 #include "aqc_launch.h"
@@ -320,6 +321,8 @@
 bool list_launches_allowed(const aqc_ws* ws);
 bool sweep_route_projected(const aqc_ws* ws, bool sparse);
 bool projected_pairs(const aqc_ws* ws);
+bool backwalk_keeps_vdag_stage(const aqc_ws* ws);
+bool projected_backwalk(const aqc_ws* ws);
 Stage3Args virtual_stage3_args(aqc_ws* ws, const DevPlan& v, size_t s);
 Stage3Args projected_sweep_stage(aqc_ws* ws, size_t s);
 int run_projected_stages(aqc_ws* ws);
diff --git a/aqc_research_amd/csrc/aqc_ws_project.cpp b/aqc_research_amd/csrc/aqc_ws_project.cpp
--- a/aqc_research_amd/csrc/aqc_ws_project.cpp
+++ b/aqc_research_amd/csrc/aqc_ws_project.cpp
@@ -214,11 +214,21 @@
     return a;
 }
 
-bool projected_pairs(const aqc_ws* ws) {
+static bool plan_has_pairs(const aqc_ws* ws) {
     const ProjRoute& pr = ws->proj;
-    return pr.ok && ws->sw.projected_pairs && !ws->capturing && pr.vsw.h_stages.size() == 1 && pr.vinv.h_stages.size() == 1 &&
-           ws->sweep.k == pr.kv && ws->inv.k == pr.kv;
-}
+    return pr.ok && pr.vsw.h_stages.size() == 1 && pr.vinv.h_stages.size() == 1 && ws->sweep.k == pr.kv && ws->inv.k == pr.kv;
+}
+bool projected_pairs(const aqc_ws* ws) { return plan_has_pairs(ws) && ws->sw.projected_pairs && !ws->capturing; }
+
+bool projected_backwalk(const aqc_ws* ws) {
+    const DevPlan& p = ws->sweep;
+    const DevPlan& iv = ws->inv;
+    return ws->proj.ok && ws->inv_mirrored && p.v3 && iv.v3 && ws->sw.r_only_last && iv.k == p.k && backwalk_tile(p.k) &&
+           iv.h_subs3.size() == p.h_subs3.size() && !iv.h_stages.empty() && p.h_stages[0].nsubs >= 2 &&
+           iv.h_stages.back().nsubs == p.h_stages[0].nsubs && iv.h_stages.back().sub_begin + iv.h_stages.back().nsubs == (int)iv.h_subs3.size();
+}
+
+bool backwalk_keeps_vdag_stage(const aqc_ws* ws) { return projected_backwalk(ws) && plan_has_pairs(ws) && ws->sw.projected_pairs == 0; }
 
 RgradSecond projected_rgrad_plan(aqc_ws* ws) {
     ProjRoute& pr = ws->proj;
@@ -298,6 +308,7 @@
     const VirtualRun y0{pr.vinv, pr.vy, pr.vy};
     const ProjArgs a = proj_args(ws);
     const bool pairs = projected_pairs(ws);
+    const bool back = projected_backwalk(ws);
 
     if (!pairs && enqueue_couple(ws, p.k, &psi, nullptr)) return 1;
     if (ensure_pattern(ws, a)) return 1;
@@ -324,8 +335,8 @@
         ProfScope ps(ws, AQC_K_PROJECT);
         HIP_OK(launch_project(q, ws->stream));
     }
-    if (!pairs && enqueue_couple(ws, iv.k, nullptr, &y0)) return 1;
-    if (enqueue_couple(ws, iv.k, &last, pairs ? &y0 : nullptr)) return 1;
+    if ((!pairs || back) && enqueue_couple(ws, iv.k, nullptr, &y0)) return 1;
+    if ((!back || backwalk_keeps_vdag_stage(ws)) && enqueue_couple(ws, iv.k, &last, pairs && !back ? &y0 : nullptr)) return 1;
     vdag_projected_state_after(ws, x_buf);
     return 0;
 }
diff --git a/aqc_research_amd/csrc/aqc_ws_sweep.cpp b/aqc_research_amd/csrc/aqc_ws_sweep.cpp
--- a/aqc_research_amd/csrc/aqc_ws_sweep.cpp
+++ b/aqc_research_amd/csrc/aqc_ws_sweep.cpp
@@ -390,6 +390,9 @@
     if (r.vdag_kind == EvalRoute::kRestricted) return run_vdag_restricted(ws, r.x_buf, r.support_in_gather_set);
     return run_apply(ws, true, AQC_BUF_Y, AQC_BUF_Z);
 }
+static bool gather_follows_sweep(const aqc_ws* ws, const EvalRoute& r) {
+    return r.vdag && r.grads && r.vdag_kind == EvalRoute::kProjected && projected_backwalk(ws);
+}
 int enqueue_gather(aqc_ws* ws, const EvalRoute& r) {
     return r.vdag_kind == EvalRoute::kProjected ? proj_fix_amplitudes(ws, r.x_buf) : aqc_ws_gather_launch(ws, AQC_BUF_Z);
 }
@@ -462,9 +465,14 @@
     const bool projected = sweep_route_projected(ws, sparse);
     if (ensure_umat(ws, p, projected ? kURoute : kUAll)) return 1;
     int r_only_sub = skipw || projected ? -1 : sweep_r_only_sub(ws);
-    const bool first_stage_r_only = projected && ws->proj_y0_ready && ws->sw.r_only_last && p.h_stages[0].nsubs >= 2 &&
+    const bool backwalk = projected && ws->proj_y0_ready && projected_backwalk(ws);
+    const bool first_stage_r_only = !backwalk && projected && ws->proj_y0_ready && ws->sw.r_only_last && p.h_stages[0].nsubs >= 2 &&
                                     p.h_stages[0].nsubs <= ws->sw.r_only_max_subs;
     if (first_stage_r_only) r_only_sub = p.h_stages[0].sub_begin + p.h_stages[0].nsubs - 1;
+    if (backwalk) {
+        if (ensure_umat(ws, ws->inv, kURoute)) return 1;
+        r_only_sub = backwalk_conj_sub(nsubs, ws->inv.h_stages.back().sub_begin);
+    }
     bool pair_virtual = projected && ws->proj_y0_ready && projected_pairs(ws);
 #ifdef AQC_TUNING
     if (ws->sw.stamps) pair_virtual = false;
@@ -477,8 +485,15 @@
         if (ensure_sweep_items(ws, x_buf)) return 1;
     }
     for (size_t s = 0; s < (projected ? 1 : m); ++s) {
-        Stage3Args a = stage3_args(ws, p, s);
-        if (sparse) {
+        Stage3Args a = backwalk ? stage3_args(ws, ws->inv, ws->inv.h_stages.size() - 1) : stage3_args(ws, p, s);
+        if (backwalk) {
+            a.in0 = ws->bufs[AQC_BUF_W];
+            a.in1 = ws->bufs[AQC_BUF_ZW];
+            a.out1 = ws->bufs[AQC_BUF_Z];
+            a.store_out = backwalk_keeps_vdag_stage(ws) ? 0 : 2;
+            a.backwalk = 1;
+            stage3_first_list(ws, a);
+        } else if (sparse) {
             double2* w2 = m >= 3 ? ws->w2 : nullptr;
             double2* z2 = m >= 3 ? ws->zw2 : nullptr;
             a.in0 = s == 0 ? ws->bufs[x_buf] : (s == 1 ? ws->bufs[AQC_BUF_W] : w2);
@@ -496,8 +511,9 @@
             a.store_out = s + 1 < m ? 3 : 0;
         }
         if (skipw && !a.items) a.supp = ws->d_combo_prev[x_buf];
-        if (s + 1 == m && r_only_sub >= 0) a.r_only_last = 1;
-        stage3_sweep_fields(a, p, nparts, chunk);
+        if (s + 1 == m && r_only_sub >= 0 && !backwalk) a.r_only_last = 1;
+        stage3_sweep_fields(a, backwalk ? ws->inv : p, nparts, chunk);
+        if (backwalk) a.rpart = p.d_rpart;
 #ifdef AQC_TUNING
         const size_t nwg = (size_t)p.ntiles * ws->batch;
         a.debug = (int)ws->sw.debug_skip;
@@ -515,6 +531,7 @@
         if (stamps_sweep(ws, a, s, nwg)) return 1;
 #endif
     }
+    if (backwalk && route.gather && !route.gather_rides && proj_fix_amplitudes(ws, x_buf)) return 1;
     if (projected && !pair_virtual && run_projected_stages(ws)) return 1;
     sweep_state_after(ws, sparse);
     ProfScope ps(ws, AQC_K_FINALIZE);
@@ -613,7 +630,7 @@
     route.x_buf = x_buf; route.vdag = route.grads = true; route.gather = ws->gather_count > 0;
     if (eval_route(ws, route)) return 1;
     if (enqueue_vdag(ws, route)) return 1;
-    if (route.gather && enqueue_gather(ws, route)) return 1;
+    if (route.gather && !gather_follows_sweep(ws, route) && enqueue_gather(ws, route)) return 1;
     return grad_from_impl(ws, route, block_from, block_to, front_layer);
 }
 
@@ -652,7 +669,8 @@
             ws->theta_host = direct ? pin_th : nullptr;
         }
         if (route.vdag && enqueue_vdag(ws, route)) return 1;
-        if (route.gather && !route.gather_rides) {
+        const bool gather_alone = route.gather && !route.gather_rides, gather_late = gather_follows_sweep(ws, route);
+        if (gather_alone && !gather_late) {
             if (enqueue_gather(ws, route)) return 1;
             if (!zero_copy) HIP_OK(hipMemcpyAsync(pin_sm, ws->d_small, sizeof(double2) * nsm, hipMemcpyDeviceToHost, ws->stream));
         }
@@ -660,6 +678,8 @@
             if (grad_from_impl(ws, route, block_from, block_to, front_layer)) return 1;
             if (!zero_copy) HIP_OK(hipMemcpyAsync(pin_gr, ws->d_grads, sizeof(double2) * nth, hipMemcpyDeviceToHost, ws->stream));
         }
+        if (gather_alone && gather_late && !zero_copy)
+            HIP_OK(hipMemcpyAsync(pin_sm, ws->d_small, sizeof(double2) * nsm, hipMemcpyDeviceToHost, ws->stream));
         ws->theta_host = nullptr;
         return 0;
     };
```

Measured after the change: 1.229 million evals/s (median of 6 runs). 4.1% higher.
